# emilemathieu/RiemannHamiltonianMonteCarlo

Hardware: AMD Instinct MI355X
Metric: leapfrog-steps/sec (whole node) (higher is better)
Workload: dtype f64 (the two O(M D^2) contractions as exact int8-sliced integer GEMMs)

## Files before the change

### riemannhamiltonianmontecarlo_amd/csrc/kernels.hip.h

```cpp
#pragma once
#include <hip/hip_runtime.h>
#include <stdint.h>

typedef double d4 __attribute__((ext_vector_type(4)));

#define RM_LD 66
#define RM_PI2 6.283185307179586476925286766559
#define RM_PK_DOUBLES (2688 + 64)
template <bool PK>
__device__ __forceinline__ int rm_row(int i) {
  if (!PK) return i * RM_LD;
  const int I = i >> 4;
  return (128 * I + 160) * I + (i & 15) * (16 * I + 18);
}
template <bool PK>
__device__ __forceinline__ int rm_len(int i) { return PK ? 16 * ((i >> 4) + 1) : 64; }

struct DevData {
  const double* Xr;
  const double* Xt;
  const double* t;
  int M, Mp, D, DP, nblk;
  double inv_alpha;
  double log_prior_const;
// ... 1082 lines not shown
        for (int I = kb + 1; I < NB; ++I) op[I] = A[rm_row<PK>(16 * I + ii) + c0 + k0 + kk];
#pragma unroll
        for (int I = kb + 1; I < NB; ++I)
#pragma unroll
          for (int J = kb + 1; J <= I; ++J) acc[I][J] = __builtin_amdgcn_mfma_f64_16x16x4f64(op[I], op[J], acc[I][J], 0, 0, 0);
      }
#pragma unroll
      for (int I = kb + 1; I < NB; ++I)
#pragma unroll
        for (int J = kb + 1; J <= I; ++J)
#pragma unroll
          for (int r = 0; r < 4; ++r) A[rm_row<PK>(16 * I + kk + 4 * r) + 16 * J + ii] -= acc[I][J][r];
      __builtin_amdgcn_wave_barrier();
    }
  }
  if (lane >= D) rdiag = 1.0;
  return bad;
}
template <bool PK = false>
__device__ __forceinline__ double cholsolve_lds(const double* L, int D, int lane, double b, double rdiag) {
  const double* rowp = L + rm_row<PK>(lane);
  int k = 0;
  for (; k + 4 <= D; k += 4) {
    const double2 l01 = lds2(rowp + k), l23 = lds2(rowp + k + 2);
    const double lk[4] = {l01.x, l01.y, l23.x, l23.y};
#pragma unroll
    for (int q = 0; q < 4; ++q) {
      const double yk = rdlane(b, k + q) * rdlane(rdiag, k + q);
      if (lane == k + q) b = yk;
      else if (lane > k + q) b = fma(-lk[q], yk, b);
    }
  }
  for (; k < D; ++k) {
    const double yk = rdlane(b, k) * rdlane(rdiag, k);
    if (lane == k) b = yk;
    else if (lane > k) b = fma(-rowp[k], yk, b);
  }
  k = D - 1;
  for (; k >= 3; k -= 4) {
    const double lk[4] = {L[rm_row<PK>(k) + lane], L[rm_row<PK>(k - 1) + lane], L[rm_row<PK>(k - 2) + lane], L[rm_row<PK>(k - 3) + lane]};
#pragma unroll
    for (int q = 0; q < 4; ++q) {
      const double xk = rdlane(b, k - q) * rdlane(rdiag, k - q);
      if (lane == k - q) b = xk;
      else if (lane < k - q) b = fma(-lk[q], xk, b);
    }
  }
  for (; k >= 0; --k) {
    const double xk = rdlane(b, k) * rdlane(rdiag, k);
    if (lane == k) b = xk;
    else if (lane < k) b = fma(-L[rm_row<PK>(k) + lane], xk, b);
  }
  return b;
}

template <bool PK = false>
__device__ __forceinline__ void load_mat_lds(double* A, const double* __restrict__ G, int D, int DP, int lane) {
  const int l = lane < D ? lane : 0;
  int i = 0;
  for (; i + 16 <= D; i += 16) {
    double v[16];
    const bool in = lane < rm_len<PK>(i);
    if (in) {
#pragma unroll
      for (int q = 0; q < 16; ++q) v[q] = G[(i + q) * DP + l];
#pragma unroll
      for (int q = 0; q < 16; ++q) A[rm_row<PK>(i + q) + lane] = v[q];
    }
  }
  for (; i + 8 <= D; i += 8) {
    double v[8];
    if (lane < rm_len<PK>(i)) {
#pragma unroll
      for (int q = 0; q < 8; ++q) v[q] = G[(i + q) * DP + l];
#pragma unroll
      for (int q = 0; q < 8; ++q) A[rm_row<PK>(i + q) + lane] = v[q];
    }
  }
  for (; i < D; ++i)
    if (lane < rm_len<PK>(i)) A[rm_row<PK>(i) + lane] = G[i * DP + l];
  __builtin_amdgcn_wave_barrier();
}

__global__ __launch_bounds__(64) void k_pos_first(int D, int DP, Chains ch, double eps, int upd_nsplit = 0) {
  __shared__ double A[64];
  const int c = blockIdx.x, lane = threadIdx.x;
  if (c == 0 && lane == 0 && ch.stale_list) *ch.stale_count = 0;
  if (ch.phase[c] != 1) return;
  const double* __restrict__ Gi = ch.trj.Ginv + (size_t)c * DP * DP;
  const bool in = lane < D;
  double g[16];
#pragma unroll
  for (int q = 0; q < 16; ++q) g[q] = (in && q < D) ? Gi[q * DP + lane] : 0.0;
  double pb = in ? ch.p[(size_t)c * DP + lane] : 0.0;
  if (upd_nsplit > 0 && in) {
    const size_t o = (size_t)c * DP + lane;
    double q = 0.0;
    for (int s0 = 0; s0 < upd_nsplit; s0 += 16) {
      double t[16];
#pragma unroll
      for (int k = 0; k < 16; ++k) t[k] = (s0 + k < upd_nsplit) ? ch.qpart[((size_t)(s0 + k) * ch.n + c) * DP + lane] : 0.0;
#pragma unroll
      for (int k = 0; k < 16; ++k)
        if (s0 + k < upd_nsplit) q += t[k];
    }
    pb = pb + (ch.tau[c] * eps * 0.5) * (ch.trj.grad[o] - 0.5 * ch.trj.tr[o] + 0.5 * q);
    ch.p[o] = pb;
  }
  double u0 = 0.0;
  A[lane] = pb;
  __builtin_amdgcn_wave_barrier();
  for (int j0 = 0; j0 < D; j0 += 16) {
    double gn[16];
#pragma unroll
    for (int q = 0; q < 16; ++q) gn[q] = (in && j0 + 16 + q < D) ? Gi[(j0 + 16 + q) * DP + lane] : 0.0;
#pragma unroll
    for (int q = 0; q < 16; ++q)
      if (in && j0 + q < D) u0 = fma(g[q], A[j0 + q], u0);
#pragma unroll
    for (int q = 0; q < 16; ++q) g[q] = gn[q];
  }
  if (lane < D) {
    ch.u0[(size_t)c * DP + lane] = u0;
    ch.wq[(size_t)c * DP + lane] = ch.trj.w[(size_t)c * DP + lane] + ch.tau[c] * eps * u0;
  }
}

template <int NB>
__global__ __launch_bounds__(64) void k_factor_solve(int D, int DP, Chains ch, double eps, int last = -1) {
  __shared__ __attribute__((aligned(16))) double A[RM_PK_DOUBLES];
  const int c = blockIdx.x, lane = threadIdx.x;
  if (c == 0 && lane == 0 && ch.i8_dmax) *ch.i8_dmax = 0ull;
  if (ch.phase[c] != 1) return;
  if (lane == 0 && ch.i8_vbad) ch.i8_vbad[c] = 0;
  load_mat_lds<true>(A, ch.Gq + (size_t)c * DP * DP, D, DP, lane);
  double rdiag;
  const int bad = chol_lds_blk<NB, true>(A, D, lane, rdiag);
  const double pb = (lane < D) ? ch.p[(size_t)c * DP + lane] : 0.0;
  const double u = cholsolve_lds<true>(A, D, lane, pb, rdiag);
  double wn = 0.0;
  if (lane < D) wn = ch.trj.w[(size_t)c * DP + lane] + ch.tau[c] * (eps * 0.5) * (ch.u0[(size_t)c * DP + lane] + u);
  int st = bad ? 1 : 0;
  if (last >= 0) {
    const double nw = sqrt(wave_sum(wn * wn));
    if (last && nw > 10.0) { wn /= nw * 3.0; st |= 8; }
    if (lane < D) ch.trj.w[(size_t)c * DP + lane] = wn;
  }
  if (lane < D) ch.wq[(size_t)c * DP + lane] = wn;
  if (st && lane == 0) ch.status[c] |= st;
}

#define RM_DMAX 256
#define RM_DCH 4

__global__ __launch_bounds__(64) void k_pos_final(int D, int DP, Chains ch, int guards) {
  const int c = blockIdx.x, lane = threadIdx.x;
  if (ch.phase[c] != 1) return;
  const size_t o = (size_t)c * DP;
  double ss = 0.0;
  for (int d = lane; d < D; d += 64) { const double w = ch.wq[o + d]; ss = fma(w, w, ss); }
  const double nw = sqrt(wave_sum(ss));
  const bool fire = guards && nw > 10.0;
  for (int d = lane; d < D; d += 64) {
    double w = ch.wq[o + d];
    if (fire) w /= nw * 3.0;
    ch.trj.w[o + d] = w;
    ch.wq[o + d] = w;
  }
  if (fire && lane == 0) ch.status[c] |= 8;
}

template <int NB, bool PK = false>
__device__ __forceinline__ void spd_inverse_lds(double* A, int D, int lane, double rdiag) {
  constexpr int DPc = 16 * NB;
  {
    const bool act = lane < DPc;
    const int row = act ? lane : DPc - 1;
    double* rowp = A + rm_row<PK>(row);
    const int rlen = min(DPc, rm_len<PK>(row));
    const int il = row & 15, cb0 = row & ~15;
    if (act) {
      rowp[row] = rdiag;
      for (int m = row + 1; m < rlen; ++m) rowp[m] = 0.0;
    }
    __builtin_amdgcn_wave_barrier();
    for (int jl = 14; jl >= 0; --jl) {
      double s0 = 0.0, s1 = 0.0;
#pragma unroll
      for (int ml = 1; ml < 16; ++ml) {
        const double t = (ml > jl) ? rowp[cb0 + ml] * A[rm_row<PK>(cb0 + ml) + cb0 + jl] : 0.0;
        if (ml & 1) s0 += t; else s1 += t;
      }
      const double rj = A[rm_row<PK>(cb0 + jl) + cb0 + jl];
      __builtin_amdgcn_wave_barrier();
      if (act && il > jl) rowp[cb0 + jl] = -(s0 + s1) * rj;
      __builtin_amdgcn_wave_barrier();
    }
    const int kk = lane >> 4, ii = lane & 15;
#pragma unroll
    for (int J = 0; J + 1 < NB; ++J) {
#pragma unroll
      for (int I = J + 1; I < NB; ++I) {
        d4 T = (d4){0.0, 0.0, 0.0, 0.0};
#pragma unroll
        for (int K = J; K < I; ++K)
#pragma unroll
          for (int k0 = 0; k0 < 16; k0 += 4)
            T = __builtin_amdgcn_mfma_f64_16x16x4f64(A[rm_row<PK>(16 * I + ii) + 16 * K + k0 + kk], A[rm_row<PK>(16 * K + k0 + kk) + 16 * J + ii], T, 0, 0,
                                                     0);
        d4 R = (d4){0.0, 0.0, 0.0, 0.0};
#pragma unroll
        for (int r = 0; r < 4; ++r) R = __builtin_amdgcn_mfma_f64_16x16x4f64(A[rm_row<PK>(16 * I + ii) + 16 * I + 4 * r + kk], T[r], R, 0, 0, 0);
        __builtin_amdgcn_wave_barrier();
#pragma unroll
        for (int r = 0; r < 4; ++r) A[rm_row<PK>(16 * I + kk + 4 * r) + 16 * J + ii] = -R[r];
        __builtin_amdgcn_wave_barrier();
      }
    }
    if (D < DPc) {
      if (lane >= D && lane < DPc)
        for (int m = 0; m < rlen; ++m) rowp[m] = 0.0;
      __builtin_amdgcn_wave_barrier();
    }
  }
  constexpr int NT = NB * (NB + 1) / 2;
  d4 acc[NT];
#pragma unroll
  for (int q = 0; q < NT; ++q) acc[q] = (d4){0.0, 0.0, 0.0, 0.0};
  {
    const int kk = lane >> 4, ii = lane & 15;
    for (int m0 = 0; m0 < DPc; m0 += 4) {
      double op[NB];
#pragma unroll
      for (int I = 0; I < NB; ++I) op[I] = A[rm_row<PK>(m0 + kk) + 16 * I + ii];
      int q = 0;
#pragma unroll
      for (int I = 0; I < NB; ++I)
#pragma unroll
        for (int J = 0; J <= I; ++J) {
          if (m0 + 3 >= 16 * I) acc[q] = __builtin_amdgcn_mfma_f64_16x16x4f64(op[I], op[J], acc[q], 0, 0, 0);
          ++q;
        }
    }
  }
  __builtin_amdgcn_wave_barrier();
  {
    int q = 0;
#pragma unroll
    for (int I = 0; I < NB; ++I)
#pragma unroll
      for (int J = 0; J <= I; ++J) {
#pragma unroll
        for (int r = 0; r < 4; ++r) A[rm_row<PK>(16 * I + (lane >> 4) + 4 * r) + 16 * J + (lane & 15)] = acc[q][r];
        ++q;
      }
  }
  __builtin_amdgcn_wave_barrier();
}

template <int NB>
__global__ __launch_bounds__(64) void k_factor_full(DevData dd, Chains ch, int nsplit) {
  __shared__ __attribute__((aligned(16))) double A[RM_PK_DOUBLES];
  constexpr int DPc = 16 * NB;
  const int D = dd.D, DP = dd.DP;
  const int c = blockIdx.x, lane = threadIdx.x;
  if (c == 0 && lane == 0 && ch.i8_dmax) *ch.i8_dmax = 0ull;
  if (ch.phase[c] != 1) return;
  if (lane == 0 && ch.i8_vbad) ch.i8_vbad[c] = 0;
  load_mat_lds<true>(A, ch.Gq + (size_t)c * DP * DP, D, DP, lane);
  double rdiag;
  const int bad = chol_lds_blk<NB, true>(A, D, lane, rdiag);
  const double hld = -wave_sum((lane < D) ? log(rdiag) : 0.0);
  double* __restrict__ Lg = ch.trj.L + (size_t)c * DP * DP;
  for (int i = 0; i < D; ++i)
    if (lane <= i) Lg[i * DP + lane] = A[rm_row<true>(i) + lane];
  __builtin_amdgcn_wave_barrier();
  spd_inverse_lds<NB, true>(A, D, lane, rdiag);
  double* __restrict__ Gi = ch.trj.Ginv + (size_t)c * DP * DP;
  const double pl = (lane < D) ? ch.p[(size_t)c * DP + lane] : 0.0;
  double u = 0.0;
  for (int i = 0; i < D; ++i) {
    const double gi = (lane <= i) ? A[rm_row<true>(i) + lane] : A[rm_row<true>(min(lane, DPc - 1)) + i];
    if (lane < D) Gi[i * DP + lane] = gi;
    u = fma((lane < D) ? gi : 0.0, rdlane(pl, i), u);
  }
  if (lane < D) ch.uq[(size_t)c * DP + lane] = u;
  double part = 0.0;
  for (int b = lane; b < nsplit; b += 64) part += ch.ljl_part[(size_t)c * nsplit + b];
  const double wl = (lane < D) ? ch.trj.w[(size_t)c * DP + lane] : 0.0;
  if (lane < D) {
    double g = 0.0;
    for (int sp = 0; sp < nsplit; ++sp) g += ch.gpart[((size_t)sp * ch.n + c) * DP + lane];
    ch.trj.grad[(size_t)c * DP + lane] = g - wl * dd.inv_alpha;
  }
  part += (lane < D) ? (dd.log_prior_const - wl * wl * 0.5 * dd.inv_alpha) : 0.0;
  const double ljl = wave_sum(part);
  if (lane == 0) {
    ch.trj.hld[c] = hld;
    ch.trj.ljl[c] = ljl;
    if (bad) ch.status[c] |= 1;
  }
}

__global__ __launch_bounds__(64) void k_ginv_matvec(int D, int DP, Chains ch, const double* __restrict__ src) {
  const int c = blockIdx.x, lane = threadIdx.x;
  if (ch.phase[c] != 1) return;
  const double* __restrict__ Gi = ch.trj.Ginv + (size_t)c * DP * DP;
  if (D <= 64) {
    const bool in = lane < D;
    const double sv = in ? src[(size_t)c * DP + lane] : 0.0;
    double u0 = 0.0;
    for (int j0 = 0; j0 < D; j0 += 16) {
      double g[16];
#pragma unroll
      for (int q = 0; q < 16; ++q) g[q] = (in && j0 + q < D) ? Gi[(j0 + q) * DP + lane] : 0.0;
#pragma unroll
      for (int q = 0; q < 16; ++q)
        if (in && j0 + q < D) u0 = fma(g[q], rdlane(sv, j0 + q), u0);
    }
    if (in) ch.uq[(size_t)c * DP + lane] = u0;
    return;
  }
  double u[RM_DCH] = {0.0, 0.0, 0.0, 0.0};
  for (int j = 0; j < D; ++j) {
    const double sj = src[(size_t)c * DP + j];
#pragma unroll
    for (int k = 0; k < RM_DCH; ++k) {
      const int d = lane + 64 * k;
      if (d < D) u[k] = fma(Gi[j * DP + d], sj, u[k]);
    }
  }
#pragma unroll
  for (int k = 0; k < RM_DCH; ++k)
    if (lane + 64 * k < D) ch.uq[(size_t)c * DP + lane + 64 * k] = u[k];
}

__global__ __launch_bounds__(64) void k_mom_update(int D, int DP, Chains ch, double eps, int final, int nsplit) {
  const int c = blockIdx.x, lane = threadIdx.x;
  if (ch.phase[c] != 1) return;
  const double h = ch.tau[c] * eps * 0.5;
  for (int d = lane; d < D; d += 64) {
    const size_t o = (size_t)c * DP + d;
    double q = 0.0;
    for (int s = 0; s < nsplit; ++s) q += ch.qpart[((size_t)s * ch.n + c) * DP + d];
    const double pm = ch.p[o] + h * (ch.trj.grad[o] - 0.5 * ch.trj.tr[o] + 0.5 * q);
    if (final) ch.p[o] = pm;
    else ch.PM[o] = pm;
  }
}

__global__ __launch_bounds__(64) void k_mom_update_matvec(int D, int DP, Chains ch, double eps, int nsplit) {
  const int c = blockIdx.x, lane = threadIdx.x;
  if (ch.phase[c] != 1) return;
  const size_t o = (size_t)c * DP + lane;
  const double* __restrict__ Gi = ch.trj.Ginv + (size_t)c * DP * DP;
  const bool in = lane < D;
  double g[16];
#pragma unroll
  for (int q = 0; q < 16; ++q) g[q] = (in && q < D) ? Gi[q * DP + lane] : 0.0;
  double pm = 0.0;
  if (in) {
    double q = 0.0;
    for (int s0 = 0; s0 < nsplit; s0 += 16) {
      double t[16];
#pragma unroll
      for (int k = 0; k < 16; ++k) t[k] = (s0 + k < nsplit) ? ch.qpart[((size_t)(s0 + k) * ch.n + c) * DP + lane] : 0.0;
#pragma unroll
      for (int k = 0; k < 16; ++k)
        if (s0 + k < nsplit) q += t[k];
    }
    pm = ch.p[o] + (ch.tau[c] * eps * 0.5) * (ch.trj.grad[o] - 0.5 * ch.trj.tr[o] + 0.5 * q);
    ch.PM[o] = pm;
  }
  double u = 0.0;
  for (int j0 = 0; j0 < D; j0 += 16) {
    double gn[16];
#pragma unroll
    for (int q = 0; q < 16; ++q) gn[q] = (in && j0 + 16 + q < D) ? Gi[(j0 + 16 + q) * DP + lane] : 0.0;
#pragma unroll
    for (int q = 0; q < 16; ++q)
      if (j0 + q < D) u = fma(g[q], rdlane(pm, j0 + q), u);
#pragma unroll
    for (int q = 0; q < 16; ++q) g[q] = gn[q];
  }
  if (in) ch.uq[o] = u;
}

__global__ __launch_bounds__(64) void k_mom_final(int D, int DP, Chains ch, double eps, int advance, int nsplit, const double* __restrict__ trpart = nullptr) {
  const int c = blockIdx.x, lane = threadIdx.x;
  if (ch.phase[c] != 1) return;
  const double h = ch.tau[c] * eps * 0.5;
  int nonfinite = 0;
  for (int d = lane; d < D; d += 64) {
    const size_t o = (size_t)c * DP + d;
    if (trpart) {
      double s = 0.0;
      for (int sp = 0; sp < nsplit; ++sp) s += trpart[((size_t)sp * ch.n + c) * DP + d];
      ch.trj.tr[o] = s;
    }
    double q = 0.0;
    for (int s = 0; s < nsplit; ++s) q += ch.qpart[((size_t)s * ch.n + c) * DP + d];
    ch.last[o] = q;
    const double pn = advance ? ch.p[o] + h * (ch.trj.grad[o] - 0.5 * ch.trj.tr[o] + 0.5 * q) : ch.p[o];
    if (advance) ch.p[o] = pn;
    nonfinite |= !(isfinite(pn) && isfinite(ch.trj.w[o]));
  }
  const unsigned long long any = __ballot(nonfinite);
  if (lane == 0) {
    if (any) ch.status[c] |= 2;
    if (advance) {
      ch.steps_left[c] -= 1;
      ch.steps_done[c] += 1;
    }
  }
}

struct IterParams {
  unsigned flags;
  int L;
  unsigned long long seed;
  long long chain_offset;
  long long iter_limit;
  long long burn_in;
  long long S;
  double* samples;
  const double *z_in, *ulen_in, *gdir_in, *uacc_in;
  int* done_count;
  const int* orig;
  int lower_L;
};

__device__ __forceinline__ void copy_rec(const Rec& dst, const Rec& src, int c, int D, int DP, int lane, bool lowerL = false) {
  const size_t o = (size_t)c * DP;
  for (int d = lane; d < D; d += 64) {
    dst.w[o + d] = src.w[o + d];
    dst.grad[o + d] = src.grad[o + d];
    dst.tr[o + d] = src.tr[o + d];
  }
  const size_t m = (size_t)c * DP * DP;
  for (int d = lane; d < D; d += 64) {
    int i = 0;
    for (; i + 16 <= D; i += 16) {
      double a[16], b[16];
#pragma unroll
      for (int q = 0; q < 16; ++q) { a[q] = lowerL && d > i + 15 ? 0.0 : src.L[m + (i + q) * DP + d]; b[q] = src.Ginv[m + (i + q) * DP + d]; }
#pragma unroll
      for (int q = 0; q < 16; ++q) {
        if (!(lowerL && d > i + 15)) dst.L[m + (i + q) * DP + d] = a[q];
        dst.Ginv[m + (i + q) * DP + d] = b[q];
      }
    }
    for (; i + 8 <= D; i += 8) {
      double a[8], b[8];
#pragma unroll
      for (int q = 0; q < 8; ++q) { a[q] = lowerL && d > i + 7 ? 0.0 : src.L[m + (i + q) * DP + d]; b[q] = src.Ginv[m + (i + q) * DP + d]; }
#pragma unroll
      for (int q = 0; q < 8; ++q) {
        if (!(lowerL && d > i + 7)) dst.L[m + (i + q) * DP + d] = a[q];
        dst.Ginv[m + (i + q) * DP + d] = b[q];
      }
    }
    for (; i < D; ++i) {
      if (!(lowerL && d > i)) dst.L[m + i * DP + d] = src.L[m + i * DP + d];
      dst.Ginv[m + i * DP + d] = src.Ginv[m + i * DP + d];
    }
  }
  if (lane == 0) {
    dst.ljl[c] = src.ljl[c];
    dst.hld[c] = src.hld[c];
  }
}

__device__ __forceinline__ double half_quadform(const double* __restrict__ Gi, int D, int DP, int lane, const double* ps) {
  if (D <= 64) {
    const bool in = lane < D;
    double y = 0.0;
    for (int j0 = 0; j0 < D; j0 += 16) {
      double g[16];
#pragma unroll
      for (int q = 0; q < 16; ++q) g[q] = (in && j0 + q < D) ? Gi[(size_t)(j0 + q) * DP + lane] : 0.0;
#pragma unroll
      for (int q = 0; q < 16; ++q)
        if (in && j0 + q < D) y = fma(g[q], ps[j0 + q], y);
    }
    return 0.5 * wave_sum(in ? fma(y, ps[lane], 0.0) : 0.0);
  }
  double y[RM_DCH] = {0.0, 0.0, 0.0, 0.0};
  for (int j = 0; j < D; ++j) {
    const double pj = ps[j];
#pragma unroll
    for (int k = 0; k < RM_DCH; ++k) {
      const int d = lane + 64 * k;
      if (d < D) y[k] = fma(Gi[j * DP + d], pj, y[k]);
    }
  }
  double s = 0.0;
#pragma unroll
  for (int k = 0; k < RM_DCH; ++k)
    if (lane + 64 * k < D) s = fma(y[k], ps[lane + 64 * k], s);
  return 0.5 * wave_sum(s);
}

__device__ __forceinline__ void draw_normals(const IterParams& ip, int c, long long it, int D, int lane, double* zs, long long oc = -1) {
  const long long id = oc >= 0 ? oc : c;
  for (int d = lane; d < D; d += 64) {
    if (ip.z_in) {
      zs[d] = ip.z_in[(size_t)c * D + d];
    } else {
      double U0, U1;
      rng_block(ip.seed, (unsigned long long)(ip.chain_offset + id), (uint32_t)it, (uint32_t)(d >> 1), U0, U1);
      const double R = sqrt(-2.0 * log(U0));
      double sn, cs;
      sincos(RM_PI2 * U1, &sn, &cs);
      zs[d] = (d & 1) ? R * sn : R * cs;
    }
  }
  __builtin_amdgcn_wave_barrier();
}

__device__ __forceinline__ void iter_begin_dev(int D, int DP, const Chains& ch, const IterParams& ip, int c, int lane, double* zs, double* ps) {
  if (ch.phase[c] != 0) return;
  const long long it = ch.iter[c];
  if (it >= ip.iter_limit) return;
  if (!ch.cstale || ch.cstale[c]) copy_rec(ch.trj, ch.cur, c, D, DP, lane, ip.lower_L != 0);
  const long long oc = ip.orig ? ip.orig[c] : c;
  draw_normals(ip, c, it, D, lane, zs, oc);
  double u_len, g_dir;
  if (ip.z_in) {
    u_len = ip.ulen_in[c];
    g_dir = ip.gdir_in[c];
  } else {
    const unsigned long long gid = (unsigned long long)(ip.chain_offset + oc);
    double U0, U1, Ua;
    rng_block(ip.seed, gid, (uint32_t)it, 0x40000000u, u_len, Ua);
    rng_block(ip.seed, gid, (uint32_t)it, 0x40000001u, U0, U1);
    g_dir = sqrt(-2.0 * log(U0)) * cos(RM_PI2 * U1);
  }
  const double* __restrict__ Lc = ch.cur.L + (size_t)c * DP * DP;
  double p[RM_DCH] = {0.0, 0.0, 0.0, 0.0};
  if (D <= 64) {
    const int d = lane;
    double acc = 0.0;
    for (int j0 = 0; j0 < D; j0 += 16) {
      double l[16];
      if (ip.flags & 1u) {
#pragma unroll
        for (int q = 0; q < 16; ++q) l[q] = (j0 + q < D && d <= j0 + q) ? Lc[(size_t)(j0 + q) * DP + d] : 0.0;
#pragma unroll
        for (int q = 0; q < 16; ++q)
          if (j0 + q < D && d <= j0 + q) acc = fma(l[q], zs[j0 + q], acc);
      } else {
#pragma unroll
        for (int q = 0; q < 16; ++q) l[q] = (d < D && j0 + q <= d) ? Lc[(size_t)d * DP + j0 + q] : 0.0;
#pragma unroll
        for (int q = 0; q < 16; ++q)
          if (d < D && j0 + q <= d) acc = fma(l[q], zs[j0 + q], acc);
      }
    }
    p[0] = acc;
  } else if (ip.flags & 1u) {
    for (int i = 0; i < D; ++i) {
      const double zi = zs[i];
#pragma unroll
      for (int k = 0; k < RM_DCH; ++k) {
        const int d = lane + 64 * k;
        if (d <= i) p[k] = fma(Lc[i * DP + d], zi, p[k]);
      }
    }
  } else {
    for (int j = 0; j < D; ++j) {
      const double zj = zs[j];
#pragma unroll
      for (int k = 0; k < RM_DCH; ++k) {
        const int d = lane + 64 * k;
        if (d >= j && d < D) p[k] = fma(Lc[d * DP + j], zj, p[k]);
      }
    }
  }
  int st = 0;
  if (ip.flags & 2u) {
    double ss = 0.0;
#pragma unroll
    for (int k = 0; k < RM_DCH; ++k) ss = fma(p[k], p[k], ss);
    const double np_ = sqrt(wave_sum(ss));
    if (np_ > 100.0) {
#pragma unroll
      for (int k = 0; k < RM_DCH; ++k) p[k] /= np_ * 25.0;
      st = 4;
    }
  }
#pragma unroll
  for (int k = 0; k < RM_DCH; ++k) {
    const int d = lane + 64 * k;
    if (d < D) {
      ps[d] = p[k];
      ch.p[(size_t)c * DP + d] = p[k];
      ch.p0[(size_t)c * DP + d] = p[k];
    }
  }
  __builtin_amdgcn_wave_barrier();
  const double quad = half_quadform(ch.cur.Ginv + (size_t)c * DP * DP, D, DP, lane, ps);
  if (lane == 0) {
    const int ns = (int)ceil(u_len * (double)ip.L);
    ch.steps_left[c] = ns;
    ch.nsteps_last[c] = ns;
    ch.tau[c] = (g_dir > 0.5) ? 1.0 : -1.0;
    ch.Hcur[c] = -ch.cur.ljl[c] + ch.cur.hld[c] + quad;
    ch.status[c] = st;
    ch.phase[c] = (ns > 0) ? 1 : 2;
  }
}

__global__ __launch_bounds__(64) void k_iter_begin(int D, int DP, Chains ch, IterParams ip) {
  __shared__ double zs[RM_DMAX];
  __shared__ double ps[RM_DMAX];
  iter_begin_dev(D, DP, ch, ip, blockIdx.x, threadIdx.x, zs, ps);
}

__device__ __forceinline__ void iter_end_dev(int D, int DP, const Chains& ch, const IterParams& ip, int c, int lane, double* ps) {
  const int ph = ch.phase[c];
  if (!(ph == 2 || (ph == 1 && ch.steps_left[c] == 0))) return;
  const long long it = ch.iter[c];
  const long long oc = ip.orig ? ip.orig[c] : c;
  for (int d = lane; d < D; d += 64) ps[d] = ch.p[(size_t)c * DP + d];
  __builtin_amdgcn_wave_barrier();
  const double quad = half_quadform(ch.trj.Ginv + (size_t)c * DP * DP, D, DP, lane, ps);
  const double Hp = -ch.trj.ljl[c] + ch.trj.hld[c] + quad;
  const double ratio = -Hp + ch.Hcur[c];
  double u_acc;
  if (ip.z_in) {
    u_acc = ip.uacc_in[c];
  } else {
    double U0;
    rng_block(ip.seed, (unsigned long long)(ip.chain_offset + oc), (uint32_t)it, 0x40000000u, U0, u_acc);
  }
  const bool accept = (ratio > 0.0) || (ratio > log(u_acc));
  if (accept) copy_rec(ch.cur, ch.trj, c, D, DP, lane, ip.lower_L != 0);
  __builtin_amdgcn_wave_barrier();
  if (ip.samples && it >= ip.burn_in && it - ip.burn_in < ip.S)
    for (int d = lane; d < D; d += 64)
      ip.samples[((size_t)oc * ip.S + (size_t)(it - ip.burn_in)) * D + d] = ch.cur.w[(size_t)c * DP + d];
  if (lane == 0) {
    ch.Hprop[c] = Hp;
    if (accept) ch.accepted[c] += 1;
    else if (ch.cstale) {
      ch.cstale[c] = 1;
      if (ch.stale_list) ch.stale_list[atomicAdd(ch.stale_count, 1)] = c;
    }
    ch.iter[c] = it + 1;
    ch.phase[c] = 0;
    if (it + 1 == ip.iter_limit && ip.done_count) atomicAdd(ip.done_count, 1);
  }
}

__global__ __launch_bounds__(64) void k_iter_end(int D, int DP, Chains ch, IterParams ip) {
  __shared__ double ps[RM_DMAX];
  iter_end_dev(D, DP, ch, ip, blockIdx.x, threadIdx.x, ps);
}

__global__ __launch_bounds__(64) void k_commit_all(int D, int DP, Chains ch) {
  copy_rec(ch.cur, ch.trj, blockIdx.x, D, DP, threadIdx.x);
}

__device__ __forceinline__ void hmc_finish_eval(const DevData& dd, const Chains& ch, int c, int lane, int nsplit) {
  const int D = dd.D, DP = dd.DP;
  double part = 0.0;
  for (int d = lane; d < D; d += 64) {
    const double wl = ch.trj.w[(size_t)c * DP + d];
    double g = 0.0;
    for (int sp = 0; sp < nsplit; ++sp) g += ch.gpart[((size_t)sp * ch.n + c) * DP + d];
    ch.trj.grad[(size_t)c * DP + d] = g - wl * dd.inv_alpha;
    part += dd.log_prior_const - wl * wl * 0.5 * dd.inv_alpha;
  }
  for (int b = lane; b < nsplit; b += 64) part += ch.ljl_part[(size_t)c * nsplit + b];
  const double ljl = wave_sum(part);
  if (lane == 0) ch.trj.ljl[c] = ljl;
}
__device__ __forceinline__ void hmc_copy(const Rec& dst, const Rec& src, int c, int D, int DP, int lane) {
  for (int d = lane; d < D; d += 64) {
    dst.w[(size_t)c * DP + d] = src.w[(size_t)c * DP + d];
    dst.grad[(size_t)c * DP + d] = src.grad[(size_t)c * DP + d];
  }
  if (lane == 0) dst.ljl[c] = src.ljl[c];
}
__global__ __launch_bounds__(64) void k_hmc_init(DevData dd, Chains ch, int nsplit) {
  const int c = blockIdx.x, lane = threadIdx.x;
  hmc_finish_eval(dd, ch, c, lane, nsplit);
  __syncthreads();
  hmc_copy(ch.cur, ch.trj, c, dd.D, dd.DP, lane);
}
__global__ __launch_bounds__(64) void k_hmc_begin(int D, int DP, Chains ch, IterParams ip) {
  __shared__ double zs[RM_DMAX];
  const int c = blockIdx.x, lane = threadIdx.x;
  if (ch.phase[c] != 0) return;
  const long long it = ch.iter[c];
  if (it >= ip.iter_limit) return;
  hmc_copy(ch.trj, ch.cur, c, D, DP, lane);
  draw_normals(ip, c, it, D, lane, zs);
  double u_len;
  if (ip.z_in) {
    u_len = ip.ulen_in[c];
  } else {
    double Ua;
    rng_block(ip.seed, (unsigned long long)(ip.chain_offset + c), (uint32_t)it, 0x40000000u, u_len, Ua);
  }
  double kin = 0.0;
  for (int d = lane; d < D; d += 64) {
    const double z = zs[d];
    kin = fma(z, z, kin);
    ch.p[(size_t)c * DP + d] = z;
  }
  kin = 0.5 * wave_sum(kin);
  if (lane == 0) {
    const int ns = (int)ceil(u_len * (double)ip.L);
    ch.steps_left[c] = ns;
    ch.nsteps_last[c] = ns;
    ch.Hcur[c] = -ch.cur.ljl[c] + kin;
    ch.status[c] = 0;
    ch.phase[c] = (ns > 0) ? 1 : 2;
  }
}
__global__ __launch_bounds__(64) void k_hmc_pre(int D, int DP, Chains ch, double eps) {
  const int c = blockIdx.x, lane = threadIdx.x;
  if (ch.phase[c] != 1) return;
  int isnan_ = 0;
  for (int d = lane; d < D; d += 64) {
    const size_t o = (size_t)c * DP + d;
    const double p = ch.p[o] + eps * 0.5 * ch.trj.grad[o];
    ch.p[o] = p;
    isnan_ |= (p != p);
  }
  const unsigned long long nan = __ballot(isnan_);
  if (!nan)
    for (int d = lane; d < D; d += 64) ch.trj.w[(size_t)c * DP + d] += eps * ch.p[(size_t)c * DP + d];
  if (nan && lane == 0) { ch.status[c] |= 2; ch.steps_left[c] = 1; }
}
__global__ __launch_bounds__(64) void k_hmc_post(DevData dd, Chains ch, double eps, int nsplit) {
  const int c = blockIdx.x, lane = threadIdx.x;
  if (ch.phase[c] != 1) return;
  hmc_finish_eval(dd, ch, c, lane, nsplit);
  __syncthreads();
  if (!(ch.status[c] & 2))
    for (int d = lane; d < dd.D; d += 64) ch.p[(size_t)c * dd.DP + d] += eps * 0.5 * ch.trj.grad[(size_t)c * dd.DP + d];
  if (lane == 0) { ch.steps_left[c] -= 1; ch.steps_done[c] += 1; }
}
__global__ __launch_bounds__(64) void k_hmc_end(int D, int DP, Chains ch, IterParams ip) {
  const int c = blockIdx.x, lane = threadIdx.x;
  const int ph = ch.phase[c];
  if (!(ph == 2 || (ph == 1 && ch.steps_left[c] == 0))) return;
  const long long it = ch.iter[c];
  double kin = 0.0;
  for (int d = lane; d < D; d += 64) { const double pl = ch.p[(size_t)c * DP + d]; kin = fma(pl, pl, kin); }
  const double Hp = -ch.trj.ljl[c] + 0.5 * wave_sum(kin);
  const double ratio = -Hp + ch.Hcur[c];
  double u_acc;
  if (ip.z_in) {
    u_acc = ip.uacc_in[c];
  } else {
    double U0;
    rng_block(ip.seed, (unsigned long long)(ip.chain_offset + c), (uint32_t)it, 0x40000000u, U0, u_acc);
  }
  const bool accept = (ratio > 0.0) || (ratio > log(u_acc));
  if (accept) hmc_copy(ch.cur, ch.trj, c, D, DP, lane);
  __syncthreads();
  if (ip.samples && it >= ip.burn_in && it - ip.burn_in < ip.S)
    for (int d = lane; d < D; d += 64)
      ip.samples[((size_t)c * ip.S + (size_t)(it - ip.burn_in)) * D + d] = ch.cur.w[(size_t)c * DP + d];
  if (lane == 0) {
    ch.Hprop[c] = Hp;
    if (accept) ch.accepted[c] += 1;
    ch.iter[c] = it + 1;
    ch.phase[c] = 0;
    if (it + 1 == ip.iter_limit && ip.done_count) atomicAdd(ip.done_count, 1);
  }
}

template <int NB>
__global__ __launch_bounds__(256) void k_trvec(DevData dd, int n_chains, int nsplit, const double* __restrict__ R, double* __restrict__ trpart,
                                               const d4* __restrict__ ctile = nullptr) {
  constexpr int DP = 16 * NB;
  const int lane = threadIdx.x & 63;
  const int c0 = (blockIdx.x * 4 + (threadIdx.x >> 6)) * 16;
  if (c0 >= n_chains) return;
  const int split = blockIdx.y;
  const int rr = lane >> 4, ci = lane & 15;
  const int cj = min(c0 + ci, n_chains - 1);
  const int nb32 = dd.Mp / 32;
  const int per = (nb32 + nsplit - 1) / nsplit;
  const int B0 = split * per, B1 = min(nb32, B0 + per);
  const double* __restrict__ xr_p = dd.Xr + (size_t)(8 * rr) * DP + NB * ci;
  const double* __restrict__ rp = R + (size_t)cj * dd.Mp + 8 * rr;
  d4 T[NB];
#pragma unroll
  for (int I = 0; I < NB; ++I) T[I] = (d4){0.0, 0.0, 0.0, 0.0};
  for (int B = B0; B < B1; ++B) {
    const int n0 = 32 * B;
    d4 r0 = *(const d4*)(rp + n0), r1 = *(const d4*)(rp + n0 + 4);
    if (ctile) {
      const d4 cA = ctile[((size_t)(c0 >> 4) * (dd.Mp / 16) + 2 * B) * 64 + lane], cB = ctile[((size_t)(c0 >> 4) * (dd.Mp / 16) + 2 * B + 1) * 64 + lane];
      r0 *= (d4){cA[0], cB[0], cA[1], cB[1]};
      r1 *= (d4){cA[2], cB[2], cA[3], cB[3]};
    }
#pragma unroll
    for (int k = 0; k < 8; ++k) {
      double xb[NB];
#pragma unroll
      for (int I = 0; I < NB; ++I) xb[I] = xr_p[(size_t)(n0 + k) * DP + I];
      const double rv = k < 4 ? r0[k & 3] : r1[k & 3];
#pragma unroll
      for (int I = 0; I < NB; ++I) T[I] = __builtin_amdgcn_mfma_f64_16x16x4f64(xb[I], rv, T[I], 0, 0, 0);
    }
  }
  if (c0 + ci < n_chains) {
    double* __restrict__ out = trpart + ((size_t)split * n_chains + c0 + ci) * DP;
#pragma unroll
    for (int I = 0; I < NB; ++I)
#pragma unroll
      for (int r = 0; r < 4; ++r) {
        const int d = NB * (rr + 4 * r) + I;
        if (d < dd.D) out[d] = T[I][r];
      }
  }
}

__global__ __launch_bounds__(64) void k_mmala_begin(int D, int DP, Chains ch, IterParams ip, double eps, int full) {
  __shared__ double zs[RM_DMAX];
  __shared__ double ts[RM_DMAX];
  const int c = blockIdx.x, lane = threadIdx.x;
  const long long it = ch.iter[c];
  if (it >= ip.iter_limit) { if (lane == 0) ch.phase[c] = 0; return; }
  draw_normals(ip, c, it, D, lane, zs);
  const double* __restrict__ Lc = ch.cur.L + (size_t)c * DP * DP;
  const double* __restrict__ Gi = ch.cur.Ginv + (size_t)c * DP * DP;
  double zz = 0.0;
  for (int d = lane; d < D; d += 64) {
    double s = 0.0;
    for (int j = 0; j <= d; ++j) s = fma(Lc[(size_t)d * DP + j], zs[j], s);
    const double dv = ch.cur.grad[(size_t)c * DP + d] - (full ? ch.cur.tr[(size_t)c * DP + d] : 0.0);
    ts[d] = sqrt(eps) * s + 0.5 * eps * dv;
    zz = fma(zs[d], zs[d], zz);
  }
  zz = wave_sum(zz);
  __syncthreads();
  double u[RM_DCH] = {0.0, 0.0, 0.0, 0.0};
  for (int j = 0; j < D; ++j) {
    const double tj = ts[j];
#pragma unroll
    for (int k = 0; k < RM_DCH; ++k) {
      const int d = lane + 64 * k;
      if (d < D) u[k] = fma(Gi[(size_t)j * DP + d], tj, u[k]);
    }
  }
#pragma unroll
  for (int k = 0; k < RM_DCH; ++k) {
    const int d = lane + 64 * k;
    if (d < D) ch.trj.w[(size_t)c * DP + d] = ch.cur.w[(size_t)c * DP + d] + u[k];
  }
  if (lane == 0) {
    ch.Hcur[c] = ch.cur.ljl[c] + ch.cur.hld[c] - 0.5 * zz;
    ch.status[c] = 0;
    ch.phase[c] = 1;
  }
}
__global__ __launch_bounds__(64) void k_mmala_end(int D, int DP, Chains ch, IterParams ip, double eps, int full) {
  __shared__ double ds[RM_DMAX];
  const int c = blockIdx.x, lane = threadIdx.x;
  if (ch.phase[c] != 1) return;
  const long long it = ch.iter[c];
  const double* __restrict__ Lp = ch.trj.L + (size_t)c * DP * DP;
  const double* __restrict__ Gi = ch.trj.Ginv + (size_t)c * DP * DP;
  double u[RM_DCH] = {0.0, 0.0, 0.0, 0.0};
  for (int j = 0; j < D; ++j) {
    const double gj = ch.trj.grad[(size_t)c * DP + j] - (full ? ch.trj.tr[(size_t)c * DP + j] : 0.0);
#pragma unroll
    for (int k = 0; k < RM_DCH; ++k) {
      const int d = lane + 64 * k;
      if (d < D) u[k] = fma(Gi[(size_t)j * DP + d], gj, u[k]);
    }
  }
#pragma unroll
  for (int k = 0; k < RM_DCH; ++k) {
    const int d = lane + 64 * k;
    if (d < D) ds[d] = ch.trj.w[(size_t)c * DP + d] + 0.5 * eps * u[k] - ch.cur.w[(size_t)c * DP + d];
  }
  __syncthreads();
  double yy = 0.0;
  for (int j = lane; j < D; j += 64) {
    double s = 0.0;
    for (int i = j; i < D; ++i) s = fma(Lp[(size_t)i * DP + j], ds[i], s);
    yy = fma(s, s, yy);
  }
  yy = wave_sum(yy);
  const double q_rev = ch.trj.hld[c] - yy / (2.0 * eps);
  const double ratio = ch.trj.ljl[c] + q_rev - ch.Hcur[c];
  double u_acc;
  if (ip.z_in) {
    u_acc = ip.uacc_in[c];
  } else {
    double U0;
    rng_block(ip.seed, (unsigned long long)(ip.chain_offset + c), (uint32_t)it, 0x40000000u, U0, u_acc);
  }
  const bool accept = (ratio > 0.0) || (ratio > log(u_acc));
  __syncthreads();
  if (accept) copy_rec(ch.cur, ch.trj, c, D, DP, lane);
  __syncthreads();
  if (ip.samples && it >= ip.burn_in && it - ip.burn_in < ip.S)
    for (int d = lane; d < D; d += 64)
      ip.samples[((size_t)c * ip.S + (size_t)(it - ip.burn_in)) * D + d] = ch.cur.w[(size_t)c * DP + d];
  if (lane == 0) {
    ch.Hprop[c] = ratio;
    if (accept) ch.accepted[c] += 1;
    ch.iter[c] = it + 1;
    ch.phase[c] = 0;
  }
}

__global__ __launch_bounds__(64) void k_ess(const double* __restrict__ samples, long long S, int P, double* __restrict__ ess_out,
                                            double* __restrict__ mean_out, double* __restrict__ var_out, long long nfft) {
  extern __shared__ __attribute__((aligned(16))) double ess_x[];
  const long long idx = blockIdx.x;
  const long long c = idx / P;
  const int d = (int)(idx % P);
  const int lane = threadIdx.x;
  const double* __restrict__ x = samples + (size_t)c * S * P + d;
  double m = 0.0;
  for (long long s = lane; s < S; s += 64) m += x[(size_t)s * P];
  m = wave_sum(m) / (double)S;
  double c0 = 0.0;
  for (long long s = lane; s < S; s += 64) {
    const double v = x[(size_t)s * P] - m;
    ess_x[s] = v;
    c0 = fma(v, v, c0);
  }
  c0 = wave_sum(c0);
  __syncthreads();
  double prev = INFINITY, sum = 0.0;
  const long long half = S / 2;
  for (long long j = 0; j < half; ++j) {
    const long long l0 = 2 * j, l1 = 2 * j + 1;
    double a = 0.0, b = 0.0;
    for (long long s = lane; s + l0 < S; s += 64) a = fma(ess_x[s], ess_x[s + l0], a);
    for (long long s = lane; s + l1 < S; s += 64) b = fma(ess_x[s], ess_x[s + l1], b);
    if (nfft > 0) {
      const long long w0 = nfft - l0, w1 = nfft - l1;
      if (l0 > 0) for (long long s = lane; s + w0 < S; s += 64) a = fma(ess_x[s], ess_x[s + w0], a);
      for (long long s = lane; s + w1 < S; s += 64) b = fma(ess_x[s], ess_x[s + w1], b);
    }
    double g = wave_sum(a + b) / c0;
    if (g > prev) g = prev;
    if (!(g > 0.0)) break;
    sum += g;
    prev = g;
  }
  double mono = -1.0 + 2.0 * sum;
  if (mono < 1.0) mono = 1.0;
  if (lane == 0) {
    if (ess_out) ess_out[idx] = (c0 > 0.0) ? (double)S / mono : NAN;
    if (mean_out) mean_out[idx] = m;
    if (var_out) var_out[idx] = c0 / (double)S;
  }
}

__global__ void k_fill_int(int* p, int v, size_t n) {
  size_t i = blockIdx.x * (size_t)blockDim.x + threadIdx.x;
  if (i < n) p[i] = v;
}
__global__ void k_fill_ll(long long* p, long long v, size_t n) {
  size_t i = blockIdx.x * (size_t)blockDim.x + threadIdx.x;
  if (i < n) p[i] = v;
}
__global__ void k_min_iter(const long long* __restrict__ iter, size_t n, unsigned long long* __restrict__ out) {
  size_t i = blockIdx.x * (size_t)blockDim.x + threadIdx.x;
  unsigned long long m = i < n ? (unsigned long long)iter[i] : ~0ull;
  for (int o = 32; o > 0; o >>= 1) {
    const unsigned long long x = __shfl_xor(m, o);
    m = x < m ? x : m;
  }
  if ((threadIdx.x & 63) == 0) atomicMin(out, m);
}
__global__ void k_traj_steps(unsigned long long seed, long long chain_offset, int L, long long it0, long long it1, size_t n,
                             long long* __restrict__ T) {
  size_t c = blockIdx.x * (size_t)blockDim.x + threadIdx.x;
  if (c >= n) return;
  long long t = 0;
  for (long long it = it0; it < it1; ++it) {
    double u_len, ua;
    rng_block(seed, (unsigned long long)(chain_offset + (long long)c), (uint32_t)it, 0x40000000u, u_len, ua);
    t += (long long)ceil(u_len * (double)L);
  }
  T[c] = t;
}
__global__ void k_scatter_ll(long long* __restrict__ dst, const long long* __restrict__ src, const int* __restrict__ orig, size_t n) {
  size_t i = blockIdx.x * (size_t)blockDim.x + threadIdx.x;
  if (i < n) dst[orig[i]] = src[i];
}
__global__ void k_sub_ll(long long* __restrict__ a, const long long* __restrict__ b, size_t n) {
  size_t i = blockIdx.x * (size_t)blockDim.x + threadIdx.x;
  if (i < n) a[i] = b[i] - a[i];
}
__global__ void k_set_leapfrog(int n, const int* __restrict__ nsteps, const int* __restrict__ dir, Chains ch) {
  int c = blockIdx.x * blockDim.x + threadIdx.x;
  if (c >= n) return;
  ch.steps_left[c] = nsteps[c];
  ch.tau[c] = (double)dir[c];
  ch.phase[c] = nsteps[c] > 0 ? 1 : 3;
}
__global__ void k_park_finished(int n, Chains ch) {
  int c = blockIdx.x * blockDim.x + threadIdx.x;
  if (c >= n) return;
  if (ch.phase[c] == 1 && ch.steps_left[c] <= 0) ch.phase[c] = 3;
}
```

### riemannhamiltonianmontecarlo_amd/csrc/rmhmc_hip.hip

```cpp
#include "../../include/rmhmc.h"
#include "../../include/rmhmc_amh.h"
#include "../../include/rmhmc_iwls.h"
#include "../../include/rmhmc_gibbs.h"
#include "kernels.hip.h"
#include "fused_small.hip.h"
#include "large_d.hip.h"
#include "metric_i8.hip.h"
#include "medium_step.hip.h"
#include "amh.hip.h"
#include "iwls.hip.h"
#include "gibbs.hip.h"

#include <algorithm>
#include <chrono>
#include <cmath>
#include <cstdio>
#include <cstdlib>
#include <cstring>
#include <map>
#include <string>
#include <vector>

namespace {

thread_local char g_err[512] = "";
constexpr int MAX_LDS = 160 * 1024;

struct EvPair { hipEvent_t a, b; };

struct Group {
  Chains ch{};
  int n = 0;
  int nsplit = 1;
  int8_t* Vs = nullptr;
  int8_t* Qs = nullptr;
  double* qscale = nullptr;
  double *Gpart = nullptr, *Rpart = nullptr;
  int* Tq = nullptr;
  int tail_pieces = 1;
  int ksplit_a = 1, ksplit_l = 1;
  int fsplit = 1;
  int* vbad = nullptr;
  int* vexp = nullptr;
  int* vexp_d = nullptr; int* rebase = nullptr; unsigned long long* dmax = nullptr;
  unsigned long long* dcount = nullptr;
  double* Gbase = nullptr;
  d4* ctile = nullptr;
  int nCp = 0;
};

struct Options {
  int64_t graph = 1, sorted = 1, inflight = 32, cdyn = 1, crestore = 1, i8_force_rebase = 0;
  int64_t ccache = 1, medium = 1, fused = 1, hmc_traj_maxn = -1, fsplit = 0, nsplit_max = 64, nsplit_waves = -1, i8_tail = -1,
          i8_delta = 1, i8_delta_inner = 1;
};
struct OptionDesc { const char* key; int64_t Options::*slot; bool create_only; int64_t lo, hi; };
const OptionDesc kOptions[] = {
    {"graph", &Options::graph, false, 0, 1},
    {"sorted", &Options::sorted, false, 0, 1},
    {"inflight", &Options::inflight, false, 0, 1 << 20},
    {"cdyn", &Options::cdyn, false, 0, 1},
    {"crestore", &Options::crestore, false, 0, 1},
    {"i8_force_rebase", &Options::i8_force_rebase, false, 0, 1},
    {"ccache", &Options::ccache, true, 0, 1},
    {"medium", &Options::medium, true, 0, 1},
    {"fused", &Options::fused, true, 0, 1},
    {"hmc_traj_maxn", &Options::hmc_traj_maxn, true, -1, (int64_t)1 << 40},
    {"fsplit", &Options::fsplit, true, 0, 64},
    {"nsplit_max", &Options::nsplit_max, true, 1, 1 << 20},
    {"nsplit_waves", &Options::nsplit_waves, true, -1, 1 << 20},
    {"i8_tail", &Options::i8_tail, true, -1, 1},
    {"i8_delta", &Options::i8_delta, true, 0, 1},
    {"i8_delta_inner", &Options::i8_delta_inner, true, 0, 1},
};
const OptionDesc* find_option(const char* key) {
  if (!key) return nullptr;
  for (const OptionDesc& d : kOptions)
    if (!strcmp(d.key, key)) return &d;
  return nullptr;
}

}

struct rmhmc_ctx {
  int device = 0;
  int64_t M = 0, n = 0;
  int D = 0, DP = 0, NB = 0, Mp = 0, nblk = 0;
  uint32_t flags = 0;
  double alpha = 100.0;
  hipStream_t stream = nullptr;
  Options opt{};
  std::vector<hipEvent_t> flow;
  long long flow_steps = 0, flow_ticks = 0;
  int* stale_list_alloc = nullptr;
  DevData dd{};
  Group batch;
  std::vector<void*> allocs;
  bool have_data = false, chains_ready = false;
  int sampler = 0;
  bool big = false;
  int nbk = 1, npairs = 1;
  double *d_Wd = nullptr, *d_hpart = nullptr, *d_Gcopy = nullptr;
  bool want_G = false;
  bool fused = false;
  size_t fused_lds = 0;
  bool medium = false;
  size_t medium_lds = 0;
  bool hmc_traj = false;
  bool i8 = false;
  int i8S = 0, i8_nks = 0, i8_bn = 128, i8_chunk = 1;
  int i8_inner_drop = 1;
  int8_t* d_Zs = nullptr;
  int* d_ze = nullptr;
  int8_t* d_Zt = nullptr;
  int* d_zre = nullptr;
  double *d_cmin = nullptr, *d_cmax = nullptr;
  double* d_zscale = nullptr;
  int i8_nkp = 0, i8_NRp = 0;
  I8Pairs pairs{};
  bool i8_requested = false;
  double i8_bound = 0.0;
  int L = 6, K = 4;
  double eps = 0.5;
  uint64_t seed = 0;
  int64_t chain_offset = 0;
  double *d_z = nullptr, *d_ulen = nullptr, *d_gdir = nullptr, *d_uacc = nullptr;
  int *d_nsteps = nullptr, *d_dir = nullptr, *d_done = nullptr;
  long long* d_steps0 = nullptr;
  unsigned long long* d_miniter = nullptr;
  int* d_orig = nullptr;
  long long* d_T = nullptr;
  bool sorted = false;
  bool counters_sorted = false;
  rmhmc_progress_fn progress_fn = nullptr;
  void* progress_user = nullptr;
  long long progress_first = 0, progress_every = 0, progress_next = 0;
  bool timing = false;
  std::map<std::string, std::vector<EvPair>> events;
  std::vector<EvPair> pool;
  char err[512] = "";
};

namespace {

int fail(rmhmc_ctx* ctx, int code, const std::string& msg) {
  snprintf(ctx ? ctx->err : g_err, 512, "%s", msg.c_str());
  return code;
}

#define HIPCK(call)                                                                                        \
  do {                                                                                                     \
    hipError_t e_ = (call);                                                                                \
    if (e_ != hipSuccess)                                                                                  \
      return fail(ctx, RMHMC_ERR_RUNTIME, std::string(hipGetErrorString(e_)) + " in " #call " (" __FILE__ ":" + std::to_string(__LINE__) + ")"); \
  } while (0)

template <typename T>
int dalloc(rmhmc_ctx* ctx, T** p, size_t count) {
  void* q = nullptr;
  size_t bytes = (count ? count : 1) * sizeof(T);
  HIPCK(hipMalloc(&q, bytes));
  HIPCK(hipMemsetAsync(q, 0, bytes, ctx->stream));
  ctx->allocs.push_back(q);
  *p = (T*)q;
  return RMHMC_OK;
}

struct Timed {
  rmhmc_ctx* ctx;
  hipStream_t st;
  EvPair ev{};
  bool on;
  Timed(rmhmc_ctx* c, const char* name, hipStream_t s) : ctx(c), st(s), on(c->timing) {
    if (!on) return;
    if (!ctx->pool.empty()) { ev = ctx->pool.back(); ctx->pool.pop_back(); }
    else { (void)hipEventCreate(&ev.a); (void)hipEventCreate(&ev.b); }
    (void)hipEventRecord(ev.a, st);
    ctx->events[name].push_back(ev);
  }
  ~Timed() { if (on) (void)hipEventRecord(ev.b, st); }
};

template <typename F>
void launch(rmhmc_ctx* ctx, const char* name, F&& fn) {
  Timed t(ctx, name, ctx->stream);
  fn(ctx->stream);
}

void flow_tick(rmhmc_ctx* ctx, long long steps = 1) {
  const long long w = ctx->opt.inflight;
  if (w <= 0) return;
  ctx->flow_steps += steps;
  const long long stride = std::max<long long>(1, w / 4);
  if (ctx->flow_steps < stride) return;
  ctx->flow_steps = 0;
  if (ctx->flow.empty()) return;
  hipEvent_t e = ctx->flow[ctx->flow_ticks % 4];
  if (ctx->flow_ticks >= 4) (void)hipEventSynchronize(e);
  (void)hipEventRecord(e, ctx->stream);
  ctx->flow_ticks++;
}

#define NB_SWITCH(ctx, ...)                                               \
  switch ((ctx)->NB) {                                                    \
    case 1: { constexpr int NB_ = 1; __VA_ARGS__; } break;                \
    case 2: { constexpr int NB_ = 2; __VA_ARGS__; } break;                \
    case 3: { constexpr int NB_ = 3; __VA_ARGS__; } break;                \
    default: { constexpr int NB_ = 4; __VA_ARGS__; } break;               \
  }

#define I8_SWITCH(ctx, ...) I8_SWITCH_S((ctx)->i8S, __VA_ARGS__)
#define I8_SWITCH_S(sval, ...)                                                     \
  switch (sval) {                                                                  \
    case 4: { constexpr int S_ = 4, WN_ = 4, TN_ = 1; __VA_ARGS__; } break;        \
    case 5: { constexpr int S_ = 5, WN_ = 4, TN_ = 1; __VA_ARGS__; } break;        \
    case 6: { constexpr int S_ = 6, WN_ = 4, TN_ = 1; __VA_ARGS__; } break;        \
    default: { constexpr int S_ = 7, WN_ = 2, TN_ = 1; __VA_ARGS__; } break;       \
  }

static bool use_delta(const rmhmc_ctx* ctx, const Group& g) {
  return ctx->i8 && ctx->opt.i8_delta && (!ctx->big || g.Gbase) && ctx->i8S == 6 && g.ctile && g.ksplit_a <= 1 && ctx->K >= 2 && g.dmax;
}
static bool use_delta_inner(const rmhmc_ctx* ctx, const Group& g, int it) {
  return use_delta(ctx, g) && ctx->opt.i8_delta_inner && ctx->i8_inner_drop && it == 2 && it < ctx->K - 1;
}
template <int MODE>
void launch_rowpass(rmhmc_ctx* ctx, Group& g, const double* w, double* out0, double* out2 = nullptr, bool delta = false) {
  launch(ctx, "rowpass", [&](hipStream_t st) {
    if (ctx->big) {
      dim3 grid((unsigned)((g.n + 15) / 16), g.nsplit);
      hipLaunchKernelGGL((k_rowpass_big<MODE>), grid, dim3(256), 0, st, ctx->dd, g.n, g.nsplit, ctx->nbk, g.ch.phase, w, out0, out2,
                         g.ch.gpart, g.ch.ljl_part, g.ctile);
      return;
    }
    dim3 grid((unsigned)((g.n + 63) / 64), g.nsplit);
    if (ctx->i8 && MODE != RP_G) {
      const VSlice vs{g.Vs, g.vbad, ctx->i8_nks, g.nCp, ctx->i8S, g.vexp, ctx->d_cmin, ctx->d_cmax};
      if (MODE != RP_G && delta) {
        VSlice vd = vs;
        vd.vexp_d = g.vexp_d; vd.rebase = g.rebase; vd.dmax = g.dmax; vd.force_rebase = (int)ctx->opt.i8_force_rebase;
        if (MODE == RP_F) {
          NB_SWITCH(ctx, hipLaunchKernelGGL((k_rowpass<NB_, RP_F, 6, false, true>), grid, dim3(256), 0, st, ctx->dd, g.n, g.nsplit, g.ch.phase, w,
                                            out0, nullptr, g.ch.gpart, g.ch.ljl_part, vd, g.ctile, g.ch.cstale));
        } else {
          NB_SWITCH(ctx, hipLaunchKernelGGL((k_rowpass<NB_, RP_V, 6, true, true>), grid, dim3(256), 0, st, ctx->dd, g.n, g.nsplit, g.ch.phase, w,
                                            out0, out2, g.ch.gpart, g.ch.ljl_part, vd, g.ctile, g.ch.cstale));
        }
      } else if (g.ctile && MODE == RP_F) {
        I8_SWITCH(ctx, NB_SWITCH(ctx, hipLaunchKernelGGL((k_rowpass<NB_, MODE, S_, false>), grid, dim3(256), 0, st, ctx->dd, g.n, g.nsplit, g.ch.phase, w,
                                                        out0, nullptr, g.ch.gpart, g.ch.ljl_part, vs, g.ctile, g.ch.cstale)));
      } else {
        I8_SWITCH(ctx, NB_SWITCH(ctx, hipLaunchKernelGGL((k_rowpass<NB_, MODE, S_>), grid, dim3(256), 0, st, ctx->dd, g.n, g.nsplit, g.ch.phase, w, out0,
                                                        out2, g.ch.gpart, g.ch.ljl_part, vs, g.ctile, g.ch.cstale)));
      }
      return;
    }
    NB_SWITCH(ctx, hipLaunchKernelGGL((k_rowpass<NB_, MODE>), grid, dim3(256), 0, st, ctx->dd, g.n, g.nsplit, g.ch.phase, w, out0,
                                      out2, g.ch.gpart, g.ch.ljl_part, VSlice{}, g.ctile, g.ch.cstale));
  });
}

template <int S, int WN, int TN>
void launch_assemble_i8_t(rmhmc_ctx* ctx, Group& g, const double* v, hipStream_t st, int part, bool delta = false, int seff = 6, int need_lo = 0,
                          int need_hi = 0) {
  const size_t vplane = (size_t)ctx->i8_nks * g.nCp * 32;
  const int8_t* const Vs = g.Vs + (delta ? (size_t)(seff - S) * vplane : 0);
  const I8Delta dl{delta ? g.dmax : nullptr, delta ? g.rebase : nullptr, delta ? std::ldexp(1.0, -8 * (seff - S)) : 1.0, need_lo, need_hi,
                   (delta && ctx->big) ? g.Gbase : nullptr};
  const int* const vexp = delta ? g.vexp_d : g.vexp;
  const int acc0 = delta ? 2 : 0;
  if (part == 0) {
    if (delta) {
      (void)hipMemsetAsync(g.dmax, 0, sizeof(unsigned long long), st);
      hipLaunchKernelGGL((k_vsplit<S, true>), dim3((unsigned)((g.n + 7) / 8)), dim3(256), 0, st, v, ctx->Mp, g.n, g.ch.phase, ctx->i8_nks, g.nCp, g.Vs,
                         g.vbad, ctx->D, ctx->DP, ctx->dd.inv_alpha, g.ch.Gq, g.vexp, VDelta{g.vexp_d, g.rebase, g.dmax, (int)ctx->opt.i8_force_rebase});
      return;
    }
    hipLaunchKernelGGL((k_vsplit<S>), dim3((unsigned)((g.n + 7) / 8)), dim3(256), 0, st, v, ctx->Mp, g.n, g.ch.phase, ctx->i8_nks, g.nCp, g.Vs, g.vbad,
                       ctx->D, ctx->DP, ctx->dd.inv_alpha, g.ch.Gq, g.vexp, VDelta{});
    return;
  }
  const int nCB = g.nCp / I8_BM, nPB = ctx->pairs.NPp / (32 * TN * WN);
  constexpr int lds = i8_lds_bytes<S, WN, TN>();
  const unsigned nblk = (unsigned)(nCB < 8 ? nCB * nPB : (nCB + 7) / 8 * 8 * nPB);
  if (g.ksplit_a > 1) {
    const size_t plane = (size_t)g.n * ctx->DP * ctx->DP;
    hipLaunchKernelGGL((k_assemble_i8<S, WN, TN>), dim3(nblk, (unsigned)g.ksplit_a), dim3(128 * WN), lds, st, g.Vs, ctx->d_Zs, g.nCp, ctx->i8_nks,
                       0, ctx->i8_nks, 0, ctx->pairs, g.n, g.ch.phase, g.vbad, ctx->DP, ctx->dd.inv_alpha, g.Gpart, plane, g.vexp, nPB,
                       I8Delta{nullptr, nullptr, 1.0, 0, 0, nullptr});
    hipLaunchKernelGGL(k_sum_planes, dim3((unsigned)((plane + 255) / 256)), dim3(256), 0, st, g.ch.Gq, g.Gpart, g.ksplit_a, plane, plane);
    return;
  }
  const int nPBfull = ctx->pairs.NP / (32 * TN * WN);
  const bool tail = WN == 4 && g.Tq && nPBfull < nPB && (ctx->opt.i8_tail == 1 || (ctx->opt.i8_tail < 0 && (long long)nCB * nPBfull >= 256));
  const int npb = tail ? nPBfull : nPB;
  const unsigned nblk_main = (unsigned)(nCB < 8 ? nCB * npb : (nCB + 7) / 8 * 8 * npb);
  const int pb32_0 = nPBfull * TN * WN, ntail = (ctx->pairs.NP - pb32_0 * 32 + 31) / 32;
  for (int ks0 = 0; ks0 < ctx->i8_nks; ks0 += ctx->i8_chunk) {
    const int nk = std::min(ctx->i8_chunk, ctx->i8_nks - ks0);
    if (nblk_main)
      hipLaunchKernelGGL((k_assemble_i8<S, WN, TN>), dim3(nblk_main), dim3(128 * WN), lds, st, Vs, ctx->d_Zs, g.nCp,
                         ctx->i8_nks, ks0, nk, (ks0 > 0 ? 1 : 0) | acc0, ctx->pairs, g.n, g.ch.phase, g.vbad, ctx->DP, ctx->dd.inv_alpha, g.ch.Gq, (size_t)0, vexp, npb, dl);
    if (tail) {
      const int pieces = std::max(1, std::min({g.tail_pieces, nk / 8, (int)(256 / std::max(1, nCB * ntail))}));
      hipLaunchKernelGGL((k_assemble_i8_tail<S>), dim3((unsigned)(nCB * ntail), (unsigned)pieces), dim3(128), (i8_lds_bytes<S, 1, 1>()), st, Vs, ctx->d_Zs,
                         g.nCp, ctx->pairs.NPp, ctx->pairs.NP, ctx->i8_nks, ks0, nk, g.n, pb32_0, ntail, g.Tq, dl);
      hipLaunchKernelGGL((k_assemble_i8_tailsum<S>), dim3((unsigned)(((size_t)g.n * 32 * ntail + 255) / 256)), dim3(256), 0, st, g.Tq, pieces, g.nCp, ntail,
                         pb32_0, (ks0 > 0 ? 1 : 0) | acc0, ctx->pairs, g.n, g.ch.phase, g.vbad, ctx->DP, ctx->dd.inv_alpha, g.ch.Gq, vexp, dl);
    }
  }
}
void launch_assemble_i8_delta(rmhmc_ctx* ctx, Group& g, hipStream_t st, int seff) {
  constexpr int WN = 4, TN = 1;
  const size_t vplane = (size_t)ctx->i8_nks * g.nCp * 32;
  const I8Delta dl{g.dmax, g.rebase, 1.0, 0, 0, ctx->big ? g.Gbase : nullptr};
  const int nCB = g.nCp / I8_BM, nPB = ctx->pairs.NPp / (32 * TN * WN);
  constexpr int lds = i8_lds_bytes<6, WN, TN>() > i8_lds_bytes<4, WN, TN>() ? i8_lds_bytes<6, WN, TN>() : i8_lds_bytes<4, WN, TN>();
  static_assert(lds >= (i8_lds_bytes<5, WN, TN>()), "dynamic LDS of the widest instantiation");
  const int nPBfull = ctx->pairs.NP / (32 * TN * WN);
  const bool tail = g.Tq && nPBfull < nPB && (ctx->opt.i8_tail == 1 || (ctx->opt.i8_tail < 0 && (long long)nCB * nPBfull >= 256));
  const int npb = tail ? nPBfull : nPB;
  const unsigned nblk_main = (unsigned)(nCB < 8 ? nCB * npb : (nCB + 7) / 8 * 8 * npb);
  const int pb32_0 = nPBfull * TN * WN, ntail = (ctx->pairs.NP - pb32_0 * 32 + 31) / 32;
  constexpr int lds_t = i8_lds_bytes<6, 1, 1>() > i8_lds_bytes<4, 1, 1>() ? i8_lds_bytes<6, 1, 1>() : i8_lds_bytes<4, 1, 1>();
  static_assert(lds_t >= (i8_lds_bytes<5, 1, 1>()), "dynamic LDS of the widest tail instantiation");
  I8Delta dlc = dl;
  dlc.count = g.dcount;
  for (int ks0 = 0; ks0 < ctx->i8_nks; ks0 += ctx->i8_chunk) {
    const int nk = std::min(ctx->i8_chunk, ctx->i8_nks - ks0);
    if (nblk_main)
      hipLaunchKernelGGL((k_assemble_i8_sel<WN, TN>), dim3(nblk_main), dim3(128 * WN), lds, st, g.Vs, vplane, seff, ctx->d_Zs, g.nCp, ctx->i8_nks, ks0, nk,
                         (ks0 > 0 ? 1 : 0) | 2, ctx->pairs, g.n, g.ch.phase, g.vbad, ctx->DP, ctx->dd.inv_alpha, g.ch.Gq, (size_t)0, g.vexp_d, npb,
                         ks0 == 0 ? dlc : dl);
    if (tail) {
      const int pieces = std::max(1, std::min({g.tail_pieces, nk / 8, (int)(256 / std::max(1, nCB * ntail))}));
      hipLaunchKernelGGL(k_assemble_i8_tail_sel, dim3((unsigned)(nCB * ntail), (unsigned)pieces), dim3(128), lds_t, st, g.Vs, vplane, seff, ctx->d_Zs,
                         g.nCp, ctx->pairs.NPp, ctx->pairs.NP, ctx->i8_nks, ks0, nk, g.n, pb32_0, ntail, g.Tq, (ks0 == 0 && !nblk_main) ? dlc : dl);
      hipLaunchKernelGGL(k_assemble_i8_tailsum_sel, dim3((unsigned)(((size_t)g.n * 32 * ntail + 255) / 256)), dim3(256), 0, st, seff, g.Tq, pieces, g.nCp, ntail,
                         pb32_0, (ks0 > 0 ? 1 : 0) | 2, ctx->pairs, g.n, g.ch.phase, g.vbad, ctx->DP, ctx->dd.inv_alpha, g.ch.Gq, g.vexp_d, dl);
    }
  }
}
template <int S, int WN, int TN>
void launch_leverage_i8_t(rmhmc_ctx* ctx, Group& g, hipStream_t st, int part) {
  if (part == 0) {
    hipLaunchKernelGGL((k_qsplit<S>), dim3((unsigned)g.n), dim3(256), 0, st, g.ch.trj.Ginv, ctx->DP, ctx->pairs, g.ch.phase, ctx->i8_nkp, g.nCp,
                       g.Qs, g.qscale);
    return;
  }
  const int nCB = g.nCp / I8_BM, nRB = ctx->i8_NRp / (32 * TN * WN);
  constexpr int lds = i8_lds_bytes<S, WN, TN>();
  const unsigned nblk = (unsigned)(nCB < 8 ? nCB * nRB : (nCB + 7) / 8 * 8 * nRB);
  if (g.ksplit_l > 1) {
    const size_t plane = (size_t)g.n * ctx->Mp;
    hipLaunchKernelGGL((k_leverage_i8<S, WN, TN>), dim3(nblk, (unsigned)g.ksplit_l), dim3(128 * WN), lds, st, g.Qs, ctx->d_Zt, g.nCp, ctx->i8_NRp,
                       ctx->i8_nkp, 0, ctx->i8_nkp, 0, (ctx->big || g.ctile) ? 0 : 1, g.n, ctx->Mp, g.ch.phase, g.qscale, ctx->d_zscale, g.ch.rv2, g.Rpart, plane);
    hipLaunchKernelGGL(k_sum_planes, dim3((unsigned)((plane + 255) / 256)), dim3(256), 0, st, g.ch.rv0, g.Rpart, g.ksplit_l, plane, plane);
    return;
  }
  for (int kp0 = 0; kp0 < ctx->i8_nkp; kp0 += ctx->i8_chunk) {
    const int nk = std::min(ctx->i8_chunk, ctx->i8_nkp - kp0);
    hipLaunchKernelGGL((k_leverage_i8<S, WN, TN>), dim3(nblk), dim3(128 * WN), lds, st, g.Qs, ctx->d_Zt, g.nCp,
                       ctx->i8_NRp, ctx->i8_nkp, kp0, nk, kp0 > 0 ? 1 : 0, (ctx->big || g.ctile) ? 0 : 1, g.n, ctx->Mp, g.ch.phase, g.qscale, ctx->d_zscale,
                       g.ch.rv2, g.ch.rv0, (size_t)0);
  }
}
void launch_assemble(rmhmc_ctx* ctx, Group& g, const double* v, bool inner = false, bool delta = false, bool keep_base = false) {
  if (ctx->i8 && delta && ctx->big)
    launch(ctx, "vsplit", [&](hipStream_t st) { launch_assemble_i8_t<6, 4, 1>(ctx, g, v, st, 0, true); });
  if (ctx->i8 && delta && inner) {
    launch(ctx, "assemble_i8_inner_delta", [&](hipStream_t st) { launch_assemble_i8_delta(ctx, g, st, 5); });
    return;
  }
  if (ctx->i8 && delta) {
    launch(ctx, "assemble_i8_delta", [&](hipStream_t st) { launch_assemble_i8_delta(ctx, g, st, 6); });
    return;
  }
  if (ctx->i8) {
    if (ctx->big)
      launch(ctx, "vsplit", [&](hipStream_t st) { I8_SWITCH(ctx, (launch_assemble_i8_t<S_, WN_, TN_>(ctx, g, v, st, 0))); });
    const int suse = (inner && ctx->i8_inner_drop && ctx->i8S == 6) ? 5 : ctx->i8S;
    launch(ctx, suse == ctx->i8S ? "assemble_i8" : "assemble_i8_inner", [&](hipStream_t st) {
      I8_SWITCH_S(suse, (launch_assemble_i8_t<S_, WN_, TN_>(ctx, g, v, st, 1)));
      if (keep_base && ctx->big && g.Gbase)
        (void)hipMemcpyAsync(g.Gbase, g.ch.Gq, sizeof(double) * (size_t)g.n * ctx->DP * ctx->DP, hipMemcpyDeviceToDevice, st);
    });
    return;
  }
  launch(ctx, "assemble", [&](hipStream_t st) {
    if (ctx->flags & RMHMC_FLAG_FP32_METRIC) {
      if (ctx->big) {
        hipLaunchKernelGGL((k_assemble_f32<4>), dim3((unsigned)((g.n + 3) / 4), ctx->npairs), dim3(256), 0, st, ctx->dd, g.n, g.ch.phase, v,
                           g.ch.Gq, ctx->nbk);
      } else {
        NB_SWITCH(ctx, hipLaunchKernelGGL((k_assemble_f32<NB_>), dim3((unsigned)((g.n + 3) / 4)), dim3(256), 0, st, ctx->dd, g.n,
                                          g.ch.phase, v, g.ch.Gq, 1));
      }
      return;
    }
    if (ctx->big) {
      hipLaunchKernelGGL(k_assemble_pair<false>, dim3((unsigned)((g.n + 3) / 4), ctx->npairs - ctx->nbk), dim3(256), 0, st, ctx->dd, g.n,
                         g.ch.phase, v, g.ch.Gq);
      hipLaunchKernelGGL(k_assemble_pair<true>, dim3((unsigned)((g.n + 3) / 4), ctx->nbk), dim3(256), 0, st, ctx->dd, g.n, g.ch.phase, v,
                         g.ch.Gq);
      return;
    }
    if (g.fsplit > 1) {
      const size_t plane = (size_t)g.n * ctx->DP * ctx->DP;
      dim3 grid((unsigned)((g.n + 3) / 4), (unsigned)g.fsplit);
      NB_SWITCH(ctx, hipLaunchKernelGGL((k_assemble<NB_>), grid, dim3(256), 0, st, ctx->dd, g.n, g.ch.phase, v, g.Gpart, plane));
      hipLaunchKernelGGL(k_sum_planes, dim3((unsigned)((plane + 255) / 256)), dim3(256), 0, st, g.ch.Gq, g.Gpart, g.fsplit, plane, plane);
      return;
    }
    dim3 grid((unsigned)((g.n + 3) / 4));
    NB_SWITCH(ctx, hipLaunchKernelGGL((k_assemble<NB_>), grid, dim3(256), 0, st, ctx->dd, g.n, g.ch.phase, v, g.ch.Gq, (size_t)0));
  });
}

void launch_mompass(rmhmc_ctx* ctx, Group& g, const double* w, int cmode) {
  launch(ctx, "mompass", [&](hipStream_t st) {
    if (!ctx->opt.ccache) cmode = 0;
    if (ctx->big) {
      dim3 grid((unsigned)((g.n + 15) / 16), g.nsplit);
      switch (cmode) {
        case 1: hipLaunchKernelGGL(k_mompass_big<1>, grid, dim3(256), 0, st, ctx->dd, g.n, g.nsplit, ctx->nbk, w, g.ch.uq, g.ch.qpart, g.ctile); break;
        case 2: hipLaunchKernelGGL(k_mompass_big<2>, grid, dim3(256), 0, st, ctx->dd, g.n, g.nsplit, ctx->nbk, w, g.ch.uq, g.ch.qpart, g.ctile); break;
        default: hipLaunchKernelGGL(k_mompass_big<0>, grid, dim3(256), 0, st, ctx->dd, g.n, g.nsplit, ctx->nbk, w, g.ch.uq, g.ch.qpart, g.ctile); break;
      }
      return;
    }
    dim3 grid((unsigned)((g.n + 63) / 64), g.nsplit);
    switch (cmode) {
      case 1:
        if (ctx->opt.cdyn) { NB_SWITCH(ctx, hipLaunchKernelGGL((k_mompass<NB_, 3>), grid, dim3(256), 0, st, ctx->dd, g.n, g.nsplit, w, g.ch.uq, g.ch.qpart, g.ctile, g.ch.cstale)); }
        else { NB_SWITCH(ctx, hipLaunchKernelGGL((k_mompass<NB_, 1>), grid, dim3(256), 0, st, ctx->dd, g.n, g.nsplit, w, g.ch.uq, g.ch.qpart, g.ctile)); }
        break;
      case 2: NB_SWITCH(ctx, hipLaunchKernelGGL((k_mompass<NB_, 2>), grid, dim3(256), 0, st, ctx->dd, g.n, g.nsplit, w, g.ch.uq, g.ch.qpart, g.ctile)); break;
      default: NB_SWITCH(ctx, hipLaunchKernelGGL((k_mompass<NB_, 0>), grid, dim3(256), 0, st, ctx->dd, g.n, g.nsplit, w, g.ch.uq, g.ch.qpart, g.ctile)); break;
    }
  });
}

static bool fused_trace(const rmhmc_ctx* ctx, const Group& g) { return ctx->i8 && !ctx->big && g.ctile != nullptr && ctx->opt.ccache; }

void launch_leverage(rmhmc_ctx* ctx, Group& g, int part = 0) {
  if (ctx->i8 && part == 2) {
    launch(ctx, "small", [&](hipStream_t st) {
      hipLaunchKernelGGL(k_reduce_tr, dim3((unsigned)g.n), dim3(64), 0, st, ctx->D, ctx->DP, g.ch, g.ch.gpart, g.nsplit);
    });
    return;
  }
  if (ctx->i8) {
    launch(ctx, "qsplit", [&](hipStream_t st) { I8_SWITCH(ctx, (launch_leverage_i8_t<S_, WN_, TN_>(ctx, g, st, 0))); });
    const int suse = (ctx->i8_inner_drop && ctx->i8S == 6) ? 5 : ctx->i8S;
    launch(ctx, "leverage_i8", [&](hipStream_t st) { I8_SWITCH_S(suse, (launch_leverage_i8_t<S_, WN_, TN_>(ctx, g, st, 1))); });
    if (part == 1) return;
    launch(ctx, "trvec", [&](hipStream_t st) {
      if (ctx->big) {
        dim3 grid((unsigned)((g.n + 15) / 16), g.nsplit);
        hipLaunchKernelGGL(k_trace_big, grid, dim3(256), 0, st, ctx->dd, g.n, g.nsplit, ctx->nbk, 1, g.ch.rv2, g.ch.rv0, g.ch.gpart);
        return;
      }
      dim3 grid((unsigned)((g.n + 63) / 64), g.nsplit);
      NB_SWITCH(ctx, hipLaunchKernelGGL((k_trvec<NB_>), grid, dim3(256), 0, st, ctx->dd, g.n, g.nsplit, g.ch.rv0, g.ch.gpart, (const d4*)g.ctile));
    });
    launch(ctx, "small", [&](hipStream_t st) {
      hipLaunchKernelGGL(k_reduce_tr, dim3((unsigned)g.n), dim3(64), 0, st, ctx->D, ctx->DP, g.ch, g.ch.gpart, g.nsplit);
    });
    return;
  }
  if (ctx->big) {
    double* hpart = ctx->d_hpart;
    launch(ctx, "leverage", [&](hipStream_t st) {
      hipLaunchKernelGGL(k_leverage_pair<false>, dim3((unsigned)((g.n + 3) / 4), ctx->npairs - ctx->nbk), dim3(256), 0, st, ctx->dd, g.n,
                         ctx->nbk, g.ch.phase, g.ch.trj.Ginv, hpart);
      hipLaunchKernelGGL(k_leverage_pair<true>, dim3((unsigned)((g.n + 3) / 4), ctx->nbk), dim3(256), 0, st, ctx->dd, g.n, ctx->nbk,
                         g.ch.phase, g.ch.trj.Ginv, hpart);
    });
    launch(ctx, "leverage", [&](hipStream_t st) {
      dim3 grid((unsigned)((g.n + 15) / 16), g.nsplit);
      hipLaunchKernelGGL(k_trace_big, grid, dim3(256), 0, st, ctx->dd, g.n, g.nsplit, ctx->nbk, ctx->npairs, g.ch.rv2, hpart, g.ch.gpart);
    });
    launch(ctx, "small", [&](hipStream_t st) {
      hipLaunchKernelGGL(k_reduce_tr, dim3((unsigned)g.n), dim3(64), 0, st, ctx->D, ctx->DP, g.ch, g.ch.gpart, g.nsplit);
    });
    return;
  }
  const int fs = std::min(g.fsplit, g.nsplit);
  launch(ctx, "leverage", [&](hipStream_t st) {
    dim3 grid((unsigned)((g.n + 3) / 4), (unsigned)fs);
    NB_SWITCH(ctx, hipLaunchKernelGGL((k_leverage<NB_>), grid, dim3(256), 0, st, ctx->dd, g.n, g.ch.phase, g.ch.trj.Ginv, g.ch.rv2,
                                      g.ch.trj.tr, g.ch.gpart));
  });
  if (fs > 1)
    launch(ctx, "small", [&](hipStream_t st) {
      hipLaunchKernelGGL(k_reduce_tr, dim3((unsigned)g.n), dim3(64), 0, st, ctx->D, ctx->DP, g.ch, g.ch.gpart, fs);
    });
}

#define SMALL(ctx, g, name, kern, ...)                                                                     \
  launch(ctx, name, [&](hipStream_t st_) { hipLaunchKernelGGL(kern, dim3((unsigned)(g).n), dim3(64), 0, st_, __VA_ARGS__); })

#define BIG(ctx, g, name, kern, ...)                                                                       \
  launch(ctx, name, [&](hipStream_t st_) { hipLaunchKernelGGL(kern, dim3((unsigned)(g).n), dim3(256), 0, st_, __VA_ARGS__); })

void eval_point_phases(rmhmc_ctx* ctx, Group& g, bool advance, int mode = 0) {
  const bool delta = advance && use_delta(ctx, g);
  launch_rowpass<RP_F>(ctx, g, g.ch.trj.w, g.ch.rv0, g.ch.rv2, delta);
  if (ctx->big) SMALL(ctx, g, "small", k_finish_big, ctx->dd, g.ch, g.nsplit);
  launch_assemble(ctx, g, g.ch.rv0, false, delta);
  if (ctx->big) {
    if (ctx->want_G)
      (void)hipMemcpyAsync(ctx->d_Gcopy, g.ch.Gq, sizeof(double) * (size_t)g.n * ctx->DP * ctx->DP, hipMemcpyDeviceToDevice, ctx->stream);
    BIG(ctx, g, "factor", k_chol_big<1>, ctx->dd, g.ch, ctx->nbk, ctx->d_Wd, ctx->eps);
    BIG(ctx, g, "factor", k_inverse_big, ctx->dd, g.ch, ctx->nbk, ctx->d_Wd);
    SMALL(ctx, g, "small", k_ginv_matvec, ctx->D, ctx->DP, g.ch, g.ch.p);
  } else {
    launch(ctx, "factor", [&](hipStream_t st) {
      NB_SWITCH(ctx, hipLaunchKernelGGL((k_factor_full<NB_>), dim3((unsigned)g.n), dim3(64), 0, st, ctx->dd, g.ch, g.nsplit));
    });
  }
  if (mode == 1) return;
  if (mode == 2) {
    launch_leverage(ctx, g);
    return;
  }
  if (fused_trace(ctx, g)) {
    launch_leverage(ctx, g, 1);
    launch(ctx, "mompass", [&](hipStream_t st) {
      dim3 grid((unsigned)((g.n + 63) / 64), g.nsplit);
      NB_SWITCH(ctx, hipLaunchKernelGGL((k_mompass_trv<NB_>), grid, dim3(256), 0, st, ctx->dd, g.n, g.nsplit, g.ch.uq, g.ch.qpart, g.ctile, g.ch.rv0, g.ch.gpart));
    });
  } else {
    launch_mompass(ctx, g, g.ch.trj.w, 2);
    launch_leverage(ctx, g);
  }
  SMALL(ctx, g, "small", k_mom_final, ctx->D, ctx->DP, g.ch, ctx->eps, advance ? 1 : 0, g.nsplit, fused_trace(ctx, g) ? g.ch.gpart : (const double*)nullptr);
}

template <int NB>
void launch_step_medium_nb(rmhmc_ctx* ctx, Group& g, hipStream_t st, int guards, int eval_only, int fold, const IterParams& ip) {
  const int rpt = (ctx->Mp + 255) / 256;
  const dim3 grid((unsigned)g.n), block(256);
  const size_t lds = ctx->medium_lds;
  switch (rpt * 16 * NB <= 64 ? rpt : 0) {
    case 1: hipLaunchKernelGGL((k_step_medium<NB, 1>), grid, block, lds, st, ctx->dd, g.ch, ctx->eps, ctx->K, guards, eval_only, fold, ip); break;
    case 2: hipLaunchKernelGGL((k_step_medium<NB, 2>), grid, block, lds, st, ctx->dd, g.ch, ctx->eps, ctx->K, guards, eval_only, fold, ip); break;
    case 3: hipLaunchKernelGGL((k_step_medium<NB, (NB == 1 ? 3 : 0)>), grid, block, lds, st, ctx->dd, g.ch, ctx->eps, ctx->K, guards, eval_only, fold, ip); break;
    case 4: hipLaunchKernelGGL((k_step_medium<NB, (NB == 1 ? 4 : 0)>), grid, block, lds, st, ctx->dd, g.ch, ctx->eps, ctx->K, guards, eval_only, fold, ip); break;
    default: hipLaunchKernelGGL((k_step_medium<NB, 0>), grid, block, lds, st, ctx->dd, g.ch, ctx->eps, ctx->K, guards, eval_only, fold, ip); break;
  }
}
void launch_step_medium(rmhmc_ctx* ctx, Group& g, hipStream_t st, int guards, int eval_only, int fold, const IterParams& ip) {
  if (ctx->NB == 1) launch_step_medium_nb<1>(ctx, g, st, guards, eval_only, fold, ip);
  else launch_step_medium_nb<2>(ctx, g, st, guards, eval_only, fold, ip);
}

void step_phases(rmhmc_ctx* ctx, Group& g) {
  const int D = ctx->D, DP = ctx->DP, K = ctx->K;
  const double eps = ctx->eps;
  const int guards = (ctx->flags & RMHMC_FLAG_GUARDS) ? 1 : 0;
  if (ctx->medium) {
    launch(ctx, "medium", [&](hipStream_t st) { launch_step_medium(ctx, g, st, guards, 0, 0, IterParams{}); });
    return;
  }
  if (!ctx->big && ctx->opt.cdyn && g.ctile && g.ch.stale_list)
    launch(ctx, "mompass", [&](hipStream_t st) {
      const int rsplit = std::max(1, std::min(32, ctx->Mp / 32 / 4));
      dim3 grid((unsigned)std::min((g.n + 63) / 64, 8), (unsigned)rsplit);
      NB_SWITCH(ctx, hipLaunchKernelGGL((k_crestore<NB_>), grid, dim3(256), 0, st, ctx->dd, g.n, g.ch.phase, g.ch.trj.w, g.ctile, g.ch.cstale,
                                        g.ch.stale_list, g.ch.stale_count));
    });
  const bool fuse = !ctx->big;
  for (int it = 0; it < K; ++it) {
    if (it == 0 || !fuse) SMALL(ctx, g, "small", k_ginv_matvec, D, DP, g.ch, it == 0 ? g.ch.p : g.ch.PM);
    launch_mompass(ctx, g, g.ch.trj.w, it == 0 ? 1 : 2);
    if (!fuse) SMALL(ctx, g, "small", k_mom_update, D, DP, g.ch, eps, it == K - 1 ? 1 : 0, g.nsplit);
    else if (it < K - 1) SMALL(ctx, g, "small", k_mom_update_matvec, D, DP, g.ch, eps, g.nsplit);
  }
  if (ctx->big) {
    SMALL(ctx, g, "small", k_ginv_matvec, D, DP, g.ch, g.ch.p);
    SMALL(ctx, g, "small", k_pos_first_big, D, DP, g.ch, eps);
  } else {
    SMALL(ctx, g, "factor", k_pos_first, D, DP, g.ch, eps, g.nsplit);
  }
  for (int it = 1; it < K; ++it) {
    launch_rowpass<RP_V>(ctx, g, g.ch.wq, g.ch.rv0, nullptr, use_delta_inner(ctx, g, it));
    const bool base = (it == 1 && use_delta_inner(ctx, g, 2)) || (it == K - 1 && use_delta(ctx, g));
    launch_assemble(ctx, g, g.ch.rv0, it < K - 1, use_delta_inner(ctx, g, it), base);
    if (ctx->big)
      BIG(ctx, g, "factor", k_chol_big<0>, ctx->dd, g.ch, ctx->nbk, ctx->d_Wd, eps);
    else
      launch(ctx, "factor", [&](hipStream_t st) {
        NB_SWITCH(ctx, hipLaunchKernelGGL((k_factor_solve<NB_>), dim3((unsigned)g.n), dim3(64), 0, st, D, DP, g.ch, eps, it == K - 1 ? guards : -1));
      });
  }
  if (ctx->big || K < 2) SMALL(ctx, g, "small", k_pos_final, D, DP, g.ch, guards);
  eval_point_phases(ctx, g, true);
}

struct IterBase {
  long long limit, burn_in, S;
  double* samples;
  bool explicit_rng;
  bool count_done;
};

IterParams iter_params(rmhmc_ctx* ctx, const IterBase& b) {
  IterParams ip{};
  ip.flags = ctx->flags;
  ip.L = ctx->L;
  ip.seed = ctx->seed;
  ip.chain_offset = ctx->chain_offset;
  ip.iter_limit = b.limit;
  ip.burn_in = b.burn_in;
  ip.S = b.S;
  ip.samples = b.samples;
  if (ctx->sorted) ip.orig = ctx->d_orig;
  if (b.explicit_rng) {
    ip.z_in = ctx->d_z; ip.ulen_in = ctx->d_ulen; ip.gdir_in = ctx->d_gdir; ip.uacc_in = ctx->d_uacc;
  }
  ip.done_count = b.count_done ? ctx->d_done : nullptr;
  ip.lower_L = (!ctx->big && !ctx->medium && !ctx->fused && ctx->sampler == 0) ? 1 : 0;
  return ip;
}

void launch_iter_begin(rmhmc_ctx* ctx, Group& g, const IterBase& b) {
  const IterParams ip = iter_params(ctx, b);
  SMALL(ctx, g, "small", k_iter_begin, ctx->D, ctx->DP, g.ch, ip);
}
void launch_iter_end(rmhmc_ctx* ctx, Group& g, const IterBase& b) {
  const IterParams ip = iter_params(ctx, b);
  SMALL(ctx, g, "small", k_iter_end, ctx->D, ctx->DP, g.ch, ip);
}

template <int NB>
void launch_hmc_traj_nb(rmhmc_ctx* ctx, Group& g, int eval_only, hipStream_t st) {
  const int rpt = (ctx->Mp + 255) / 256;
  const dim3 grid((unsigned)g.n), block(256);
  switch (rpt <= 4 ? rpt : 0) {
    case 1: hipLaunchKernelGGL((k_hmc_traj<NB, 1>), grid, block, 0, st, ctx->dd, g.ch, ctx->eps, eval_only); break;
    case 2: hipLaunchKernelGGL((k_hmc_traj<NB, 2>), grid, block, 0, st, ctx->dd, g.ch, ctx->eps, eval_only); break;
    case 3: hipLaunchKernelGGL((k_hmc_traj<NB, 3>), grid, block, 0, st, ctx->dd, g.ch, ctx->eps, eval_only); break;
    case 4: hipLaunchKernelGGL((k_hmc_traj<NB, 4>), grid, block, 0, st, ctx->dd, g.ch, ctx->eps, eval_only); break;
    default: hipLaunchKernelGGL((k_hmc_traj<NB, 0>), grid, block, 0, st, ctx->dd, g.ch, ctx->eps, eval_only); break;
  }
}
void launch_hmc_traj(rmhmc_ctx* ctx, Group& g, int eval_only) {
  launch(ctx, "medium", [&](hipStream_t st) {
    if (ctx->NB == 1) launch_hmc_traj_nb<1>(ctx, g, eval_only, st);
    else launch_hmc_traj_nb<2>(ctx, g, eval_only, st);
  });
}

void launch_hmc_global_step(rmhmc_ctx* ctx, Group& g, const IterBase& b) {
  const double eps = ctx->eps;
  const IterParams ip = iter_params(ctx, b);
  SMALL(ctx, g, "small", k_hmc_begin, ctx->D, ctx->DP, g.ch, ip);
  if (ctx->hmc_traj) {
    launch_hmc_traj(ctx, g, 0);
  } else {
    SMALL(ctx, g, "small", k_hmc_pre, ctx->D, ctx->DP, g.ch, eps);
    launch_rowpass<RP_G>(ctx, g, g.ch.trj.w, nullptr);
    SMALL(ctx, g, "small", k_hmc_post, ctx->dd, g.ch, eps, g.nsplit);
  }
  SMALL(ctx, g, "small", k_hmc_end, ctx->D, ctx->DP, g.ch, ip);
}

void launch_global_step(rmhmc_ctx* ctx, Group& g, const IterBase& b) {
  if (ctx->sampler == 1) { launch_hmc_global_step(ctx, g, b); return; }
  if (ctx->medium) {
    const int guards = (ctx->flags & RMHMC_FLAG_GUARDS) ? 1 : 0;
    const IterParams ip = iter_params(ctx, b);
    launch(ctx, "medium", [&](hipStream_t st) { launch_step_medium(ctx, g, st, guards, 0, 1, ip); });
    return;
  }
  launch_iter_begin(ctx, g, b);
  step_phases(ctx, g);
  launch_iter_end(ctx, g, b);
}

void launch_fused(rmhmc_ctx* ctx, const IterBase& b, long long nsteps) {
  Group& g = ctx->batch;
  while (nsteps > 0) {
    const int chunk = (int)std::min<long long>(nsteps, 4096);
    FusedParams fp{};
    fp.ip = iter_params(ctx, b);
    fp.eps = ctx->eps; fp.K = ctx->K; fp.nsteps = chunk; fp.DPs = ctx->DP; fp.init_eval = 0;
    launch(ctx, "fused", [&](hipStream_t st) {
      hipLaunchKernelGGL(k_fused_small, dim3((unsigned)((g.n + FS_WAVES - 1) / FS_WAVES)), dim3(64 * FS_WAVES), ctx->fused_lds, st,
                         ctx->dd, g.ch, fp);
    });
    nsteps -= chunk;
    if (nsteps > 0) flow_tick(ctx, ctx->opt.inflight);
  }
}

void fill_int(rmhmc_ctx* ctx, int* p, int v, size_t n) {
  hipLaunchKernelGGL(k_fill_int, dim3((unsigned)((n + 255) / 256)), dim3(256), 0, ctx->stream, p, v, n);
}
void fill_ll(rmhmc_ctx* ctx, long long* p, long long v, size_t n) {
  hipLaunchKernelGGL(k_fill_ll, dim3((unsigned)((n + 255) / 256)), dim3(256), 0, ctx->stream, p, v, n);
}

int upload_vec(rmhmc_ctx* ctx, double* dst, const double* src) {
  HIPCK(hipMemcpy2DAsync(dst, ctx->DP * sizeof(double), src, ctx->D * sizeof(double), ctx->D * sizeof(double), ctx->n,
                         hipMemcpyHostToDevice, ctx->stream));
  return RMHMC_OK;
}
int download_vec(rmhmc_ctx* ctx, double* dst, const double* src) {
  HIPCK(hipMemcpy2DAsync(dst, ctx->D * sizeof(double), src, ctx->DP * sizeof(double), ctx->D * sizeof(double), ctx->n,
                         hipMemcpyDeviceToHost, ctx->stream));
  return RMHMC_OK;
}
template <typename T>
int download(rmhmc_ctx* ctx, T* dst, const T* src, size_t count) {
  HIPCK(hipMemcpyAsync(dst, src, count * sizeof(T), hipMemcpyDeviceToHost, ctx->stream));
  return RMHMC_OK;
}
template <typename T>
int upload(rmhmc_ctx* ctx, T* dst, const T* src, size_t count) {
  HIPCK(hipMemcpyAsync(dst, src, count * sizeof(T), hipMemcpyHostToDevice, ctx->stream));
  return RMHMC_OK;
}

int sync(rmhmc_ctx* ctx) {
  HIPCK(hipStreamSynchronize(ctx->stream));
  HIPCK(hipGetLastError());
  return RMHMC_OK;
}

#define RC(x) do { int rc_ = (x); if (rc_ != RMHMC_OK) return rc_; } while (0)
#define NEED_DATA(ctx)                                                              \
  do {                                                                              \
    if (!(ctx)) return fail(nullptr, RMHMC_ERR_INVALID, "null context");            \
    if (!(ctx)->have_data) return fail(ctx, RMHMC_ERR_INVALID, "rmhmc_set_data has not been called"); \
    HIPCK(hipSetDevice((ctx)->device));                                             \
  } while (0)

int eval_at(rmhmc_ctx* ctx, const double* w, const double* p, bool one_launch = false) {
  Group& g = ctx->batch;
  Chains& ch = g.ch;
  RC(upload_vec(ctx, ch.trj.w, w));
  if (p) RC(upload_vec(ctx, ch.p, p));
  else HIPCK(hipMemsetAsync(ch.p, 0, sizeof(double) * ctx->n * ctx->DP, ctx->stream));
  fill_int(ctx, ch.phase, 1, ctx->n);
  fill_int(ctx, ch.status, 0, ctx->n);
  if (one_launch && ctx->medium) {
    launch(ctx, "medium", [&](hipStream_t st) { launch_step_medium(ctx, g, st, 0, 1, 0, IterParams{}); });
    return RMHMC_OK;
  }
  eval_point_phases(ctx, g, false);
  return RMHMC_OK;
}

void apply_runtime_options(rmhmc_ctx* ctx) {
  Group& g = ctx->batch;
  const bool ok = !ctx->big && !ctx->medium && !ctx->fused && g.ctile && ctx->opt.cdyn && ctx->opt.crestore;
  g.ch.stale_list = ok ? ctx->stale_list_alloc : nullptr;
}

}

extern "C" {

const char* rmhmc_version(void) { return "rmhmc-hip 0.1 (gfx950, fp64 MFMA)"; }
const char* rmhmc_last_error(const rmhmc_ctx* ctx) { return ctx ? ctx->err : g_err; }

int rmhmc_create(rmhmc_ctx** out, int32_t device_id, int64_t M, int32_t D, int64_t n_chains, int32_t dtype, uint32_t flags) {
  return rmhmc_create_opts(out, device_id, M, D, n_chains, dtype, flags, nullptr, 0);
}

int rmhmc_create_opts(rmhmc_ctx** out, int32_t device_id, int64_t M, int32_t D, int64_t n_chains, int32_t dtype, uint32_t flags,
                      const rmhmc_option* opts, int32_t n_opts) {
  rmhmc_ctx* ctx = nullptr;
  Options opt{};
  if (n_opts < 0 || (n_opts > 0 && !opts)) return fail(nullptr, RMHMC_ERR_INVALID, "rmhmc_create_opts: bad option array");
  for (int i = 0; i < n_opts; ++i) {
    const OptionDesc* d = find_option(opts[i].key);
    if (!d) return fail(nullptr, RMHMC_ERR_INVALID, std::string("rmhmc_create_opts: unknown option '") + (opts[i].key ? opts[i].key : "(null)") + "'");
    if (opts[i].value < d->lo || opts[i].value > d->hi)
      return fail(nullptr, RMHMC_ERR_INVALID, std::string("rmhmc_create_opts: value out of range for option '") + d->key + "'");
    opt.*(d->slot) = opts[i].value;
  }
  if (!out || M <= 0 || D <= 0 || n_chains <= 0) return fail(nullptr, RMHMC_ERR_INVALID, "rmhmc_create: bad shape");
  if (dtype != RMHMC_F64) return fail(nullptr, RMHMC_ERR_UNSUPPORTED, "rmhmc_create: only float64 is built (the reference is float64)");
  if (D > 256) return fail(nullptr, RMHMC_ERR_UNSUPPORTED, "rmhmc_create: D > 256 is not supported (64 < D <= 256 uses the blocked large-D path)");
  if (flags & RMHMC_FLAG_ORACLE_LITERAL) return fail(nullptr, RMHMC_ERR_UNSUPPORTED, "rmhmc_create: the literal variant exists only in the CPU oracle");
  if (M > (int64_t)1 << 30 || n_chains > (int64_t)1 << 30) return fail(nullptr, RMHMC_ERR_UNSUPPORTED, "rmhmc_create: M or n_chains too large");
  if (D <= 64 && (M + 63) / 64 * 64 * (int64_t)(16 * ((D + 15) / 16)) * 8 >= (int64_t)1 << 32)
    return fail(nullptr, RMHMC_ERR_UNSUPPORTED, "rmhmc_create: the data matrix of the D <= 64 path must stay below 4 GB");
  int ndev = 0;
  if (hipGetDeviceCount(&ndev) != hipSuccess || ndev <= 0)
    return fail(nullptr, RMHMC_ERR_NO_DEVICE, "rmhmc_create: no HIP device available (this library has no CPU fallback)");
  if (device_id < 0 || device_id >= ndev) return fail(nullptr, RMHMC_ERR_NO_DEVICE, "rmhmc_create: device ordinal out of range");
  HIPCK(hipSetDevice(device_id));
  hipDeviceProp_t prop;
  HIPCK(hipGetDeviceProperties(&prop, device_id));
  if (std::string(prop.gcnArchName).find("gfx950") == std::string::npos)
    return fail(nullptr, RMHMC_ERR_NO_DEVICE, std::string("rmhmc_create: kernels are built for gfx950 only, device is ") + prop.gcnArchName);
  ctx = new rmhmc_ctx();
  ctx->device = device_id;
  ctx->M = M; ctx->D = D; ctx->n = n_chains; ctx->flags = flags; ctx->opt = opt;
  ctx->NB = (D + 15) / 16; ctx->DP = 16 * ctx->NB;
  if (D > 64) {
    ctx->big = true;
    ctx->nbk = (D + 63) / 64;
    ctx->npairs = ctx->nbk * (ctx->nbk + 1) / 2;
    ctx->DP = 64 * ctx->nbk;
    ctx->NB = 4;
  }
  ctx->Mp = (int)((M + 63) / 64 * 64); ctx->nblk = ctx->Mp / 64;
  if (flags & RMHMC_FLAG_INT8_INNER_FULL) ctx->i8_inner_drop = 0;
  int rc = RMHMC_OK;
  auto body = [&]() -> int {
    HIPCK(hipStreamCreateWithFlags(&ctx->stream, hipStreamNonBlocking));
    ctx->flow.resize(4);
    for (auto& e : ctx->flow) { e = nullptr; HIPCK(hipEventCreateWithFlags(&e, hipEventDisableTiming)); }
    const size_t n = n_chains, DP = ctx->DP, Mp = ctx->Mp;
    double *Xr, *Xt, *t;
    RC(dalloc(ctx, &Xr, Mp * DP)); RC(dalloc(ctx, &Xt, DP * Mp)); RC(dalloc(ctx, &t, Mp));
    ctx->dd.Xr = Xr; ctx->dd.Xt = Xt; ctx->dd.t = t;
    ctx->dd.M = (int)M; ctx->dd.Mp = ctx->Mp; ctx->dd.D = D; ctx->dd.DP = ctx->DP; ctx->dd.nblk = ctx->nblk;
    Chains& ch = ctx->batch.ch;
    ch.n = (int)n;
    for (Rec* r : {&ch.cur, &ch.trj}) {
      RC(dalloc(ctx, &r->w, n * DP)); RC(dalloc(ctx, &r->grad, n * DP)); RC(dalloc(ctx, &r->tr, n * DP));
      RC(dalloc(ctx, &r->L, n * DP * DP)); RC(dalloc(ctx, &r->Ginv, n * DP * DP));
      RC(dalloc(ctx, &r->ljl, n)); RC(dalloc(ctx, &r->hld, n));
    }
    RC(dalloc(ctx, &ch.p, n * DP)); RC(dalloc(ctx, &ch.p0, n * DP)); RC(dalloc(ctx, &ch.Hcur, n)); RC(dalloc(ctx, &ch.Hprop, n));
    RC(dalloc(ctx, &ch.tau, n)); RC(dalloc(ctx, &ch.steps_left, n)); RC(dalloc(ctx, &ch.phase, n)); RC(dalloc(ctx, &ch.status, n)); RC(dalloc(ctx, &ch.cstale, n));
    RC(dalloc(ctx, &ch.stale_list, n)); RC(dalloc(ctx, &ch.stale_count, (size_t)1));
    ctx->stale_list_alloc = ch.stale_list;
    RC(dalloc(ctx, &ch.nsteps_last, n)); RC(dalloc(ctx, &ch.iter, n)); RC(dalloc(ctx, &ch.accepted, n)); RC(dalloc(ctx, &ch.steps_done, n));
    RC(dalloc(ctx, &ch.wq, n * DP)); RC(dalloc(ctx, &ch.uq, n * DP)); RC(dalloc(ctx, &ch.PM, n * DP)); RC(dalloc(ctx, &ch.u0, n * DP));
    RC(dalloc(ctx, &ch.q, n * DP)); RC(dalloc(ctx, &ch.last, n * DP)); RC(dalloc(ctx, &ch.Gq, n * DP * DP));
    RC(dalloc(ctx, &ch.rv0, n * Mp)); RC(dalloc(ctx, &ch.rv2, n * Mp));
    Group& g = ctx->batch;
    {
      g.n = (int)n_chains;
      const long long cgroups = (g.n + 15) / 16, nb16 = ctx->Mp / 16;
      const long long target = ctx->opt.nsplit_waves > 0 ? ctx->opt.nsplit_waves : (ctx->big ? 6144 : 2048);
      long long ns = (target + cgroups - 1) / cgroups;
      if (ns < 1) ns = 1;
      if (ns > nb16) ns = nb16;
      if (ns > ctx->opt.nsplit_max) ns = ctx->opt.nsplit_max;
      g.nsplit = (int)ns;
      RC(dalloc(ctx, &g.ch.qpart, (size_t)g.nsplit * g.n * DP));
      RC(dalloc(ctx, &g.ch.gpart, (size_t)g.nsplit * g.n * DP));
      RC(dalloc(ctx, &g.ch.ljl_part, (size_t)g.n * g.nsplit));
      if (ctx->opt.ccache) RC(dalloc(ctx, &g.ctile, (size_t)((g.n + 15) / 16) * (ctx->Mp / 16) * 64));
      if (!ctx->big) {
        const long long waves = g.n;
        long long fs = waves >= 1024 ? 1 : std::min<long long>(16, (2048 + waves - 1) / waves);
        fs = std::min<long long>(fs, std::max(1, ctx->Mp / 256));
        if (ctx->opt.fsplit >= 1) fs = ctx->opt.fsplit;
        g.fsplit = (int)fs;
      }
    }
    int i8_slices = (int)((flags >> 12) & 7u);
    if (i8_slices == 0) i8_slices = 6;
    if (i8_slices < 4) i8_slices = 4;
    if (flags & RMHMC_FLAG_INT8_METRIC) {
      const int S = i8_slices;
      ctx->i8_chunk = std::max(1, (int)(2147483647.0 / (S * 16384.0)) / 32);
      ctx->i8 = true;
      ctx->i8_requested = true;
      ctx->i8S = S;
      ctx->i8_bn = S <= 6 ? 128 : 64;
      ctx->i8_nks = (int)((M + 31) / 32);
      const int NP = D * (D + 1) / 2, NPp = (NP + ctx->i8_bn - 1) / ctx->i8_bn * ctx->i8_bn;
      std::vector<short> pa(NPp, 0), pb(NPp, 0);
      for (int a = 0, q = 0; a < D; ++a)
        for (int b = 0; b <= a; ++b, ++q) { pa[q] = (short)a; pb[q] = (short)b; }
      short *d_pa, *d_pb; double* d_scale;
      RC(dalloc(ctx, &d_pa, (size_t)NPp)); RC(dalloc(ctx, &d_pb, (size_t)NPp)); RC(dalloc(ctx, &d_scale, (size_t)NPp));
      RC(dalloc(ctx, &ctx->d_ze, (size_t)NPp));
      HIPCK(hipMemcpyAsync(d_pa, pa.data(), NPp * sizeof(short), hipMemcpyHostToDevice, ctx->stream));
      HIPCK(hipMemcpyAsync(d_pb, pb.data(), NPp * sizeof(short), hipMemcpyHostToDevice, ctx->stream));
      RC(sync(ctx));
      int* d_cexp;
      RC(dalloc(ctx, &d_cexp, (size_t)ctx->DP));
      RC(dalloc(ctx, &ctx->d_cmin, (size_t)ctx->DP)); RC(dalloc(ctx, &ctx->d_cmax, (size_t)ctx->DP));
      ctx->pairs = I8Pairs{d_pa, d_pb, d_scale, NP, NPp, d_cexp};
      RC(dalloc(ctx, &ctx->d_Zs, (size_t)S * ctx->i8_nks * NPp * 32));
      ctx->i8_nkp = (NP + 31) / 32;
      ctx->i8_NRp = (ctx->Mp + ctx->i8_bn - 1) / ctx->i8_bn * ctx->i8_bn;
      RC(dalloc(ctx, &ctx->d_Zt, (size_t)S * ctx->i8_nkp * ctx->i8_NRp * 32));
      RC(dalloc(ctx, &ctx->d_zre, (size_t)ctx->i8_NRp)); RC(dalloc(ctx, &ctx->d_zscale, (size_t)ctx->i8_NRp));
      {
        g.nCp = (g.n + I8_BM - 1) / I8_BM * I8_BM;
        RC(dalloc(ctx, &g.Vs, (size_t)S * ctx->i8_nks * g.nCp * 32));
        RC(dalloc(ctx, &g.vbad, (size_t)g.nCp));
        RC(dalloc(ctx, &g.vexp, (size_t)g.nCp));
        RC(dalloc(ctx, &g.vexp_d, (size_t)g.nCp)); RC(dalloc(ctx, &g.rebase, (size_t)g.nCp)); RC(dalloc(ctx, &g.dmax, (size_t)1));
        RC(dalloc(ctx, &g.dcount, (size_t)6));
        if (!ctx->big) { g.ch.i8_vbad = g.vbad; g.ch.i8_dmax = g.dmax; }
        if (ctx->big && ctx->opt.i8_delta && S == 6) RC(dalloc(ctx, &g.Gbase, (size_t)g.n * ctx->DP * ctx->DP));
        RC(dalloc(ctx, &g.Qs, (size_t)S * ctx->i8_nkp * g.nCp * 32));
        RC(dalloc(ctx, &g.qscale, (size_t)g.nCp));
        auto pieces = [&](long long tiles, int stages) {
          long long k = std::min<long long>(16, 256 / std::max<long long>(1, tiles));
          k = std::min<long long>(k, stages / 8);
          if (k < 2 || stages > ctx->i8_chunk || ctx->big) return 1;
          const int per = (int)((stages + k - 1) / k);
          return (stages + per - 1) / per;
        };
        g.ksplit_a = pieces((long long)(g.nCp / I8_BM) * (NPp / ctx->i8_bn), ctx->i8_nks);
        g.ksplit_l = pieces((long long)(g.nCp / I8_BM) * (ctx->i8_NRp / ctx->i8_bn), ctx->i8_nkp);
        if (g.ksplit_a > 1) RC(dalloc(ctx, &g.Gpart, (size_t)g.ksplit_a * g.n * ctx->DP * ctx->DP));
        if (g.ksplit_a == 1 && ctx->i8_bn == 128 && NP % 128 != 0 && ctx->opt.i8_tail != 0) {
          const int ntail = (NP % 128 + 31) / 32;
          g.tail_pieces = (int)std::max<long long>(1, std::min<long long>(8, 256 / ((long long)(g.nCp / I8_BM) * ntail)));
          RC(dalloc(ctx, &g.Tq, (size_t)g.tail_pieces * S * g.nCp * 32 * ntail));
        }
        if (g.ksplit_l > 1) RC(dalloc(ctx, &g.Rpart, (size_t)g.ksplit_l * g.n * ctx->Mp));
      }
      I8_SWITCH(ctx, {
        constexpr int lds = i8_lds_bytes<S_, WN_, TN_>();
        auto kfn = k_assemble_i8<S_, WN_, TN_>;
        HIPCK(hipFuncSetAttribute((const void*)kfn, hipFuncAttributeMaxDynamicSharedMemorySize, lds));
        auto kfn2 = k_leverage_i8<S_, WN_, TN_>;
        HIPCK(hipFuncSetAttribute((const void*)kfn2, hipFuncAttributeMaxDynamicSharedMemorySize, lds));
        auto kfn3 = k_assemble_i8_tail<S_>;
        HIPCK(hipFuncSetAttribute((const void*)kfn3, hipFuncAttributeMaxDynamicSharedMemorySize, (i8_lds_bytes<S_, 1, 1>())));
      });
      if (S == 6) {
        constexpr int ld = i8_lds_bytes<6, 4, 1>() > i8_lds_bytes<4, 4, 1>() ? i8_lds_bytes<6, 4, 1>() : i8_lds_bytes<4, 4, 1>();
        constexpr int ldt = i8_lds_bytes<6, 1, 1>() > i8_lds_bytes<4, 1, 1>() ? i8_lds_bytes<6, 1, 1>() : i8_lds_bytes<4, 1, 1>();
        HIPCK(hipFuncSetAttribute((const void*)k_assemble_i8_sel<4, 1>, hipFuncAttributeMaxDynamicSharedMemorySize, ld));
        HIPCK(hipFuncSetAttribute((const void*)k_assemble_i8_tail_sel, hipFuncAttributeMaxDynamicSharedMemorySize, ldt));
      }
      if (S == 6)
        for (int sv = S - 2; sv < S; ++sv)
          I8_SWITCH_S(sv, {
            auto kfn = k_assemble_i8<S_, WN_, TN_>;
            HIPCK(hipFuncSetAttribute((const void*)kfn, hipFuncAttributeMaxDynamicSharedMemorySize, (i8_lds_bytes<S_, WN_, TN_>())));
            auto kfn2 = k_leverage_i8<S_, WN_, TN_>;
            HIPCK(hipFuncSetAttribute((const void*)kfn2, hipFuncAttributeMaxDynamicSharedMemorySize, (i8_lds_bytes<S_, WN_, TN_>())));
            auto kfn3 = k_assemble_i8_tail<S_>;
            HIPCK(hipFuncSetAttribute((const void*)kfn3, hipFuncAttributeMaxDynamicSharedMemorySize, (i8_lds_bytes<S_, 1, 1>())));
          });
    }
    {
      const int need = std::max(g.fsplit, g.ksplit_a);
      if (g.fsplit > 1 && (!g.Gpart || g.fsplit > g.ksplit_a)) RC(dalloc(ctx, &g.Gpart, (size_t)need * g.n * ctx->DP * ctx->DP));
    }
    RC(dalloc(ctx, &ctx->d_z, n * (size_t)D)); RC(dalloc(ctx, &ctx->d_ulen, n)); RC(dalloc(ctx, &ctx->d_gdir, n)); RC(dalloc(ctx, &ctx->d_uacc, n));
    if (ctx->big) {
      RC(dalloc(ctx, &ctx->d_Wd, n * (size_t)ctx->nbk * 4096));
      if (!(flags & RMHMC_FLAG_INT8_METRIC)) RC(dalloc(ctx, &ctx->d_hpart, (size_t)ctx->npairs * n * Mp));
    }
    fill_int(ctx, ch.cstale, 1, n);
    RC(dalloc(ctx, &ctx->d_nsteps, n)); RC(dalloc(ctx, &ctx->d_dir, n)); RC(dalloc(ctx, &ctx->d_done, 1)); RC(dalloc(ctx, &ctx->d_steps0, n));
    RC(dalloc(ctx, &ctx->d_miniter, 1));
    RC(dalloc(ctx, &ctx->d_orig, n)); RC(dalloc(ctx, &ctx->d_T, 2 * n));
    {
      const bool on = ctx->opt.medium && !ctx->big && D > FS_D && D <= 32 && ctx->Mp <= MS_MAXMP && n_chains <= 512;
      if (on) {
        const size_t lds = sizeof(double) * (ctx->NB == 1 ? ms_lds_doubles<1>(ctx->Mp) : ms_lds_doubles<2>(ctx->Mp));
        if (ctx->NB == 1) {
          HIPCK(hipFuncSetAttribute((const void*)k_step_medium<1, 0>, hipFuncAttributeMaxDynamicSharedMemorySize, MAX_LDS));
          HIPCK(hipFuncSetAttribute((const void*)k_step_medium<1, 1>, hipFuncAttributeMaxDynamicSharedMemorySize, MAX_LDS));
          HIPCK(hipFuncSetAttribute((const void*)k_step_medium<1, 2>, hipFuncAttributeMaxDynamicSharedMemorySize, MAX_LDS));
          HIPCK(hipFuncSetAttribute((const void*)k_step_medium<1, 3>, hipFuncAttributeMaxDynamicSharedMemorySize, MAX_LDS));
          HIPCK(hipFuncSetAttribute((const void*)k_step_medium<1, 4>, hipFuncAttributeMaxDynamicSharedMemorySize, MAX_LDS));
        } else {
          HIPCK(hipFuncSetAttribute((const void*)k_step_medium<2, 0>, hipFuncAttributeMaxDynamicSharedMemorySize, MAX_LDS));
          HIPCK(hipFuncSetAttribute((const void*)k_step_medium<2, 1>, hipFuncAttributeMaxDynamicSharedMemorySize, MAX_LDS));
          HIPCK(hipFuncSetAttribute((const void*)k_step_medium<2, 2>, hipFuncAttributeMaxDynamicSharedMemorySize, MAX_LDS));
        }
        ctx->medium = true;
        ctx->medium_lds = lds;
      }
    }
    {
      long long maxn = ctx->Mp <= 1024 ? (1ll << 40) : 512;
      if (ctx->opt.hmc_traj_maxn >= 0) maxn = ctx->opt.hmc_traj_maxn;
      ctx->hmc_traj = ctx->opt.medium && !ctx->big && D <= 32 && n_chains <= maxn;
    }
    {
      const size_t lds = ((size_t)(FS_D + 1 + FS_WAVES) * ctx->Mp + (size_t)FS_WAVES * FS_PT) * sizeof(double);
      if (ctx->opt.fused && D <= FS_D && lds <= 160 * 1024) {
        HIPCK(hipFuncSetAttribute((const void*)k_fused_small, hipFuncAttributeMaxDynamicSharedMemorySize, MAX_LDS));
        ctx->fused = true;
        ctx->fused_lds = lds;
      }
    }
    RC(sync(ctx));
    return RMHMC_OK;
  };
  rc = body();
  if (rc != RMHMC_OK) {
    snprintf(g_err, 512, "%s", ctx->err);
    rmhmc_destroy(ctx);
    return rc;
  }
  apply_runtime_options(ctx);
  *out = ctx;
  return RMHMC_OK;
}

void rmhmc_destroy(rmhmc_ctx* ctx) {
  if (!ctx) return;
  (void)hipSetDevice(ctx->device);
  if (ctx->stream) (void)hipStreamSynchronize(ctx->stream);
  for (auto& e : ctx->flow) if (e) (void)hipEventDestroy(e);
  for (auto& kv : ctx->events) for (auto& e : kv.second) { (void)hipEventDestroy(e.a); (void)hipEventDestroy(e.b); }
  for (auto& e : ctx->pool) { (void)hipEventDestroy(e.a); (void)hipEventDestroy(e.b); }
  for (void* p : ctx->allocs) (void)hipFree(p);
  if (ctx->stream) (void)hipStreamDestroy(ctx->stream);
  delete ctx;
}

int rmhmc_set_option(rmhmc_ctx* ctx, const char* key, int64_t value) {
  if (!ctx) return fail(nullptr, RMHMC_ERR_INVALID, "set_option: null context");
  const OptionDesc* d = find_option(key);
  if (!d) return fail(ctx, RMHMC_ERR_INVALID, std::string("set_option: unknown option '") + (key ? key : "(null)") + "'");
  if (d->create_only) return fail(ctx, RMHMC_ERR_INVALID, std::string("set_option: '") + key + "' shapes the context and can only be given to rmhmc_create_opts");
  if (value < d->lo || value > d->hi) return fail(ctx, RMHMC_ERR_INVALID, std::string("set_option: value out of range for '") + key + "'");
  HIPCK(hipSetDevice(ctx->device));
  HIPCK(hipStreamSynchronize(ctx->stream));
  ctx->opt.*(d->slot) = value;
  apply_runtime_options(ctx);
  if (ctx->stale_list_alloc) {
    HIPCK(hipMemsetAsync(ctx->batch.ch.stale_count, 0, sizeof(int), ctx->stream));
    fill_int(ctx, ctx->batch.ch.cstale, 1, ctx->n);
    HIPCK(hipStreamSynchronize(ctx->stream));
  }
  return RMHMC_OK;
}
int rmhmc_get_option(rmhmc_ctx* ctx, const char* key, int64_t* value_out) {
  if (!ctx || !value_out) return fail(ctx, RMHMC_ERR_INVALID, "get_option: null pointer");
  const OptionDesc* d = find_option(key);
  if (!d) return fail(ctx, RMHMC_ERR_INVALID, std::string("get_option: unknown option '") + (key ? key : "(null)") + "'");
  *value_out = ctx->opt.*(d->slot);
  return RMHMC_OK;
}
int rmhmc_options(rmhmc_ctx* ctx, char* buf, size_t len) {
  if (!ctx || !buf || !len) return fail(ctx, RMHMC_ERR_INVALID, "options: bad argument");
  std::string o;
  for (const OptionDesc& d : kOptions) o += (o.empty() ? "" : " ") + std::string(d.key) + "=" + std::to_string(ctx->opt.*(d.slot));
  snprintf(buf, len, "%s", o.c_str());
  return RMHMC_OK;
}

int rmhmc_device_info(rmhmc_ctx* ctx, char* buf, size_t len) {
  if (!ctx || !buf) return fail(ctx, RMHMC_ERR_INVALID, "device_info: bad argument");
  hipDeviceProp_t prop;
  HIPCK(hipGetDeviceProperties(&prop, ctx->device));
  snprintf(buf, len, "%s %s, %d CUs, %.0f MHz, %.1f GiB; M=%lld (padded %d) D=%d (padded %d, %d MFMA tiles) chains=%lld%s",
           prop.name, prop.gcnArchName, prop.multiProcessorCount, prop.clockRate / 1000.0, prop.totalGlobalMem / 1073741824.0,
           (long long)ctx->M, ctx->Mp, ctx->D, ctx->DP, ctx->NB * (ctx->NB + 1) / 2, (long long)ctx->n,
           ctx->fused ? ", fused small-problem path" : ctx->medium ? ", one-launch step" : ctx->big ? ", blocked large-D path" : "");
  if (ctx->i8_requested) {
    const size_t k = strlen(buf);
    snprintf(buf + k, len > k ? len - k : 0, "; int8 metric path %d slices: %s (certificate %.2e%s)", ctx->i8S,
             ctx->i8 ? "active" : "NOT certified for this data, fp64 matrix cores used", ctx->i8_bound,
             ctx->have_data ? "" : ", no data yet");
  }
  {
    const size_t k = strlen(buf);
    if (len > k + 12) {
      snprintf(buf + k, len - k, "; options: ");
      const size_t k2 = strlen(buf);
      (void)rmhmc_options(ctx, buf + k2, len - k2);
    }
  }
  return RMHMC_OK;
}

int rmhmc_set_data(rmhmc_ctx* ctx, const double* X, const double* t, double alpha) {
  if (!ctx || !X || !t || !(alpha > 0)) return fail(ctx, RMHMC_ERR_INVALID, "set_data: bad argument");
  HIPCK(hipSetDevice(ctx->device));
  const size_t M = ctx->M, D = ctx->D, DP = ctx->DP, Mp = ctx->Mp;
  std::vector<double> xr(Mp * DP, 0.0), xt(DP * Mp, 0.0), tt(Mp, 0.0);
  for (size_t n = 0; n < M; ++n) {
    for (size_t d = 0; d < D; ++d) {
      xr[n * DP + d] = X[n * D + d];
      xt[d * Mp + n] = X[n * D + d];
    }
    tt[n] = t[n];
  }
  HIPCK(hipMemcpyAsync((void*)ctx->dd.Xr, xr.data(), xr.size() * 8, hipMemcpyHostToDevice, ctx->stream));
  HIPCK(hipMemcpyAsync((void*)ctx->dd.Xt, xt.data(), xt.size() * 8, hipMemcpyHostToDevice, ctx->stream));
  HIPCK(hipMemcpyAsync((void*)ctx->dd.t, tt.data(), tt.size() * 8, hipMemcpyHostToDevice, ctx->stream));
  if (ctx->i8_requested) {
    std::vector<int> cexp(DP, 0);
    std::vector<double> cmin(DP, 0.0), cmax(DP, 0.0);
    for (size_t d = 0; d < D; ++d) {
      double m = 0.0, lo = INFINITY;
      for (size_t n = 0; n < M; ++n) { const double a = std::fabs(X[n * D + d]); m = std::max(m, a); lo = std::min(lo, a); }
      if (m > 0.0 && m < 1e300) (void)std::frexp(m, &cexp[d]);
      if (m < 1e300) { cmin[d] = lo; cmax[d] = m; }
    }
    HIPCK(hipMemcpyAsync((void*)ctx->pairs.cexp, cexp.data(), sizeof(int) * DP, hipMemcpyHostToDevice, ctx->stream));
    HIPCK(hipMemcpyAsync(ctx->d_cmin, cmin.data(), sizeof(double) * DP, hipMemcpyHostToDevice, ctx->stream));
    HIPCK(hipMemcpyAsync(ctx->d_cmax, cmax.data(), sizeof(double) * DP, hipMemcpyHostToDevice, ctx->stream));
    RC(sync(ctx));
    hipLaunchKernelGGL(k_zmax, dim3((unsigned)ctx->pairs.NPp), dim3(256), 0, ctx->stream, ctx->dd.Xt, (int)M, (int)Mp, ctx->pairs, ctx->d_ze,
                       (double*)ctx->pairs.scale);
    const dim3 grid((unsigned)((ctx->i8_nks * 8 + 255) / 256), (unsigned)ctx->pairs.NPp);
    I8_SWITCH(ctx, hipLaunchKernelGGL((k_zsplit<S_>), grid, dim3(256), 0, ctx->stream, ctx->dd.Xt, (int)M, (int)Mp, ctx->pairs, ctx->d_ze,
                                      ctx->i8_nks, ctx->d_Zs); (void)WN_; (void)TN_);
    hipLaunchKernelGGL(k_zrowmax, dim3((unsigned)((ctx->i8_NRp + 255) / 256)), dim3(256), 0, ctx->stream, ctx->dd.Xr, (int)M, (int)D, (int)DP,
                       ctx->i8_NRp, ctx->pairs.cexp, ctx->d_zre, ctx->d_zscale);
    const dim3 gridt((unsigned)(ctx->i8_NRp / 32), (unsigned)ctx->i8_nkp);
    I8_SWITCH(ctx, hipLaunchKernelGGL((k_ztsplit<S_>), gridt, dim3(256), 0, ctx->stream, ctx->dd.Xr, (int)M, (int)DP, ctx->pairs, ctx->d_zre,
                                      ctx->i8_nkp, ctx->i8_NRp, ctx->d_Zt); (void)WN_; (void)TN_);
    HIPCK(hipGetLastError());
  }
  RC(sync(ctx));
  if (ctx->i8_requested) {
    std::vector<int> ze(ctx->pairs.NP);
    HIPCK(hipMemcpy(ze.data(), ctx->d_ze, sizeof(int) * ze.size(), hipMemcpyDeviceToHost));
    std::vector<double> g0(D, 1.0 / alpha);
    for (size_t n = 0; n < M; ++n)
      for (size_t d = 0; d < D; ++d) g0[d] += 0.25 * X[n * D + d] * X[n * D + d];
    double bound = 0.0;
    for (size_t a = 0, q = 0; a < D; ++a)
      for (size_t b = 0; b <= a; ++b, ++q)
        bound = std::max(bound, std::ldexp((double)ctx->i8S * (double)M, ze[q] - 8 * ctx->i8S) / std::sqrt(g0[a] * g0[b]));
    if (ctx->opt.i8_delta && ctx->i8S == 6) bound *= (2.0 * ctx->i8S - 1.0) / ctx->i8S;
    ctx->i8_bound = bound;
    const bool ok = !(ctx->flags & RMHMC_FLAG_INT8_CERTIFY) || bound <= RMHMC_INT8_CERTIFY_TOL;
    if (!ok && ctx->big && !ctx->d_hpart) RC(dalloc(ctx, &ctx->d_hpart, (size_t)ctx->npairs * ctx->n * Mp));
    ctx->i8 = ok;
    RC(sync(ctx));
  }
  ctx->alpha = alpha;
  ctx->dd.inv_alpha = 1.0 / alpha;
  ctx->dd.log_prior_const = -0.5 * std::log(2.0 * M_PI * alpha);
  ctx->have_data = true;
  ctx->chains_ready = false;
  return RMHMC_OK;
}

int rmhmc_log_posterior(rmhmc_ctx* ctx, const double* w, double* ljl_out) {
  NEED_DATA(ctx);
  if (!w || !ljl_out) return fail(ctx, RMHMC_ERR_INVALID, "log_posterior: null pointer");
  ctx->chains_ready = false;
  RC(eval_at(ctx, w, nullptr));
  RC(download(ctx, ljl_out, ctx->batch.ch.trj.ljl, ctx->n));
  return sync(ctx);
}

int rmhmc_metric(rmhmc_ctx* ctx, const double* w, double* G_out, double* half_logdet_out, double* grad_out) {
  NEED_DATA(ctx);
  if (!w) return fail(ctx, RMHMC_ERR_INVALID, "metric: null pointer");
  ctx->chains_ready = false;
  if (ctx->big && G_out && !ctx->d_Gcopy) RC(dalloc(ctx, &ctx->d_Gcopy, (size_t)ctx->n * ctx->DP * ctx->DP));
  ctx->want_G = ctx->big && G_out;
  int rc_eval = eval_at(ctx, w, nullptr);
  ctx->want_G = false;
  RC(rc_eval);
  if (G_out)
    for (int64_t c = 0; c < ctx->n; ++c)
      HIPCK(hipMemcpy2DAsync(G_out + c * ctx->D * ctx->D, ctx->D * 8, (ctx->big ? ctx->d_Gcopy : ctx->batch.ch.Gq) + c * ctx->DP * ctx->DP, ctx->DP * 8, ctx->D * 8, ctx->D,
                             hipMemcpyDeviceToHost, ctx->stream));
  if (half_logdet_out) RC(download(ctx, half_logdet_out, ctx->batch.ch.trj.hld, ctx->n));
  if (grad_out) RC(download_vec(ctx, grad_out, ctx->batch.ch.trj.grad));
  RC(sync(ctx));
  if (G_out && ctx->i8) {
    const int64_t D = ctx->D;
    for (int64_t c = 0; c < ctx->n; ++c)
      for (int64_t a = 0; a < D; ++a)
        for (int64_t b = a + 1; b < D; ++b) G_out[(c * D + a) * D + b] = G_out[(c * D + b) * D + a];
  }
  return RMHMC_OK;
}

int rmhmc_metric_terms(rmhmc_ctx* ctx, const double* w, const double* p, double* trace_out, double* quad_out) {
  NEED_DATA(ctx);
  if (!w) return fail(ctx, RMHMC_ERR_INVALID, "metric_terms: null pointer");
  ctx->chains_ready = false;
  RC(eval_at(ctx, w, p));
  if (trace_out) RC(download_vec(ctx, trace_out, ctx->batch.ch.trj.tr));
  if (quad_out && p) RC(download_vec(ctx, quad_out, ctx->batch.ch.last));
  return sync(ctx);
}

int rmhmc_leapfrog(rmhmc_ctx* ctx, double* w, double* p, double eps, const int32_t* dir, const int32_t* nsteps, int32_t K,
                   double* half_logdet_out, int32_t* status_out) {
  NEED_DATA(ctx);
  if (!w || !p || !dir || !nsteps || K < 1) return fail(ctx, RMHMC_ERR_INVALID, "leapfrog: null pointer or K < 1");
  ctx->chains_ready = false;
  int maxs = 0;
  for (int64_t c = 0; c < ctx->n; ++c) {
    if (nsteps[c] < 0 || (dir[c] != 1 && dir[c] != -1)) return fail(ctx, RMHMC_ERR_INVALID, "leapfrog: nsteps >= 0 and dir = +-1 required");
    if (nsteps[c] > maxs) maxs = nsteps[c];
  }
  ctx->eps = eps; ctx->K = K;
  RC(upload(ctx, ctx->d_nsteps, nsteps, ctx->n));
  RC(upload(ctx, ctx->d_dir, dir, ctx->n));
  RC(eval_at(ctx, w, p));
  Group& g = ctx->batch;
  launch(ctx, "small", [&](hipStream_t st) {
    hipLaunchKernelGGL(k_set_leapfrog, dim3((unsigned)((g.n + 255) / 256)), dim3(256), 0, st, g.n, ctx->d_nsteps, ctx->d_dir, g.ch);
  });
  for (int s = 0; s < maxs; ++s) {
    step_phases(ctx, g);
    launch(ctx, "small", [&](hipStream_t st) {
      hipLaunchKernelGGL(k_park_finished, dim3((unsigned)((g.n + 255) / 256)), dim3(256), 0, st, g.n, g.ch);
    });
  }
  RC(download_vec(ctx, w, ctx->batch.ch.trj.w));
  RC(download_vec(ctx, p, ctx->batch.ch.p));
  if (half_logdet_out) RC(download(ctx, half_logdet_out, ctx->batch.ch.trj.hld, ctx->n));
  if (status_out) RC(download(ctx, status_out, ctx->batch.ch.status, ctx->n));
  return sync(ctx);
}

static int init_chains(rmhmc_ctx* ctx, const double* theta0_host , bool allow_fused = true, bool allow_medium = true) {
  Group& g = ctx->batch;
  std::vector<double> th;
  if (!theta0_host) {
    th.assign((size_t)ctx->n * ctx->D, 1e-3);
    theta0_host = th.data();
  }
  if (ctx->fused && allow_fused) {
    RC(upload_vec(ctx, g.ch.cur.w, theta0_host));
    FusedParams fp{};
    fp.ip = iter_params(ctx, IterBase{0, 0, 0, nullptr, false, false});
    fp.eps = ctx->eps; fp.K = ctx->K; fp.nsteps = 0; fp.DPs = ctx->DP; fp.init_eval = 1;
    launch(ctx, "fused", [&](hipStream_t st) {
      hipLaunchKernelGGL(k_fused_small, dim3((unsigned)((g.n + FS_WAVES - 1) / FS_WAVES)), dim3(64 * FS_WAVES), ctx->fused_lds, st,
                         ctx->dd, g.ch, fp);
    });
  } else {
    RC(eval_at(ctx, theta0_host, nullptr, allow_medium));
    SMALL(ctx, g, "small", k_commit_all, ctx->D, ctx->DP, g.ch);
  }
  fill_int(ctx, ctx->batch.ch.phase, 0, ctx->n);
  fill_int(ctx, ctx->batch.ch.steps_left, 0, ctx->n);
  fill_int(ctx, ctx->batch.ch.status, 0, ctx->n);
  fill_ll(ctx, ctx->batch.ch.iter, 0, ctx->n);
  fill_ll(ctx, ctx->batch.ch.accepted, 0, ctx->n);
  fill_ll(ctx, ctx->batch.ch.steps_done, 0, ctx->n);
  HIPCK(hipMemsetAsync(ctx->d_done, 0, sizeof(int), ctx->stream));
  return sync(ctx);
}

int rmhmc_transition(rmhmc_ctx* ctx, double* w, const double* z, const double* u_len, const double* g_dir, const double* u_acc,
                     int32_t L, double eps, int32_t K, int32_t* accepted_out, int32_t* nsteps_out, double* H_cur_out,
                     double* H_prop_out, double* w_prop_out, double* p_prop_out, double* half_logdet_prop_out, int32_t* status_out) {
  NEED_DATA(ctx);
  if (!w || !z || !u_len || !g_dir || !u_acc || L < 1 || K < 1) return fail(ctx, RMHMC_ERR_INVALID, "transition: null pointer, L < 1 or K < 1");
  ctx->chains_ready = false;
  ctx->L = L; ctx->eps = eps; ctx->K = K;
  RC(init_chains(ctx, w));
  RC(upload(ctx, ctx->d_z, z, (size_t)ctx->n * ctx->D));
  RC(upload(ctx, ctx->d_ulen, u_len, ctx->n));
  RC(upload(ctx, ctx->d_gdir, g_dir, ctx->n));
  RC(upload(ctx, ctx->d_uacc, u_acc, ctx->n));
  const IterBase ib{1, 0, 0, nullptr, true, false};
  if (ctx->fused) {
    launch_fused(ctx, ib, L);
  } else {
    Group& g = ctx->batch;
    launch_iter_begin(ctx, g, ib);
    launch_iter_end(ctx, g, ib);
    for (int s = 0; s < L; ++s) {
      step_phases(ctx, g);
      launch_iter_end(ctx, g, ib);
    }
  }
  std::vector<long long> acc(ctx->n);
  RC(download_vec(ctx, w, ctx->batch.ch.cur.w));
  RC(download(ctx, acc.data(), ctx->batch.ch.accepted, ctx->n));
  if (nsteps_out) RC(download(ctx, nsteps_out, ctx->batch.ch.nsteps_last, ctx->n));
  if (H_cur_out) RC(download(ctx, H_cur_out, ctx->batch.ch.Hcur, ctx->n));
  if (H_prop_out) RC(download(ctx, H_prop_out, ctx->batch.ch.Hprop, ctx->n));
  if (w_prop_out) RC(download_vec(ctx, w_prop_out, ctx->batch.ch.trj.w));
  if (p_prop_out) RC(download_vec(ctx, p_prop_out, ctx->batch.ch.p));
  if (half_logdet_prop_out) RC(download(ctx, half_logdet_prop_out, ctx->batch.ch.trj.hld, ctx->n));
  if (status_out) RC(download(ctx, status_out, ctx->batch.ch.status, ctx->n));
  RC(sync(ctx));
  if (accepted_out) for (int64_t c = 0; c < ctx->n; ++c) accepted_out[c] = (int32_t)acc[c];
  return RMHMC_OK;
}

struct StepGraph {
  hipGraph_t graph = nullptr;
  hipGraphExec_t exec = nullptr;
  ~StepGraph() {
    if (exec) (void)hipGraphExecDestroy(exec);
    if (graph) (void)hipGraphDestroy(graph);
  }
};
static bool step_graph_usable(const rmhmc_ctx* ctx, long long nsteps) {
  if (ctx->timing || nsteps < 8) return false;
  if (ctx->fused && ctx->sampler == 0) return false;
  if (ctx->medium && ctx->sampler == 0) return false;
  return ctx->opt.graph != 0;
}
static bool build_step_graph(rmhmc_ctx* ctx, const IterBase& ib, StepGraph& sg) {
  if (hipStreamBeginCapture(ctx->stream, hipStreamCaptureModeThreadLocal) != hipSuccess) return false;
  launch_global_step(ctx, ctx->batch, ib);
  if (hipStreamEndCapture(ctx->stream, &sg.graph) != hipSuccess || !sg.graph) { (void)hipGetLastError(); return false; }
  if (hipGraphInstantiate(&sg.exec, sg.graph, nullptr, nullptr, 0) != hipSuccess) { (void)hipGetLastError(); sg.exec = nullptr; return false; }
  return true;
}
static void run_generic_steps(rmhmc_ctx* ctx, const IterBase& ib, long long nsteps, StepGraph* sg) {
  if (sg && sg->exec) {
    for (long long s = 0; s < nsteps; ++s) { (void)hipGraphLaunch(sg->exec, ctx->stream); flow_tick(ctx); }
  } else {
    for (long long s = 0; s < nsteps; ++s) { launch_global_step(ctx, ctx->batch, ib); flow_tick(ctx); }
  }
}

static int poll_progress(rmhmc_ctx* ctx, int* done, long long* min_iter) {
  HIPCK(hipMemsetAsync(ctx->d_miniter, 0xff, sizeof(unsigned long long), ctx->stream));
  hipLaunchKernelGGL(k_min_iter, dim3((unsigned)((ctx->n + 255) / 256)), dim3(256), 0, ctx->stream, ctx->batch.ch.iter, (size_t)ctx->n, ctx->d_miniter);
  unsigned long long mi = 0;
  HIPCK(hipMemcpyAsync(done, ctx->d_done, sizeof(int), hipMemcpyDeviceToHost, ctx->stream));
  HIPCK(hipMemcpyAsync(&mi, ctx->d_miniter, sizeof(mi), hipMemcpyDeviceToHost, ctx->stream));
  RC(sync(ctx));
  *min_iter = (long long)mi;
  return RMHMC_OK;
}

static int report_progress(rmhmc_ctx* ctx, int event, long long iters) {
  std::vector<long long> acc(ctx->n), it(ctx->n);
  RC(download(ctx, acc.data(), ctx->batch.ch.accepted, ctx->n));
  RC(download(ctx, it.data(), ctx->batch.ch.iter, ctx->n));
  RC(sync(ctx));
  long long tot = 0, tit = 0;
  for (long long a : acc) tot += a;
  for (long long a : it) tit += a;
  ctx->progress_fn(event, iters, tot, tit, ctx->progress_user);
  return RMHMC_OK;
}
static bool progress_ticking(const rmhmc_ctx* ctx) { return ctx->progress_fn && ctx->progress_every > 0 && ctx->n > 1; }
static int progress_fire(rmhmc_ctx* ctx, long long min_iter) {
  if (!progress_ticking(ctx)) return RMHMC_OK;
  long long last = -1;
  while (ctx->progress_next <= min_iter) { last = ctx->progress_next; ctx->progress_next += ctx->progress_every; }
  if (last >= 0) RC(report_progress(ctx, RMHMC_EV_PROGRESS, last));
  return RMHMC_OK;
}

static int run_until_done(rmhmc_ctx* ctx, const IterBase& ib, long long min_steps) {
  int done = 0;
  long long s = min_steps, min_iter = 0;
  const long long poll = 4;
  const bool fused = ctx->fused && ctx->sampler == 0;
  const bool ticking = progress_ticking(ctx);
  const long long chunk = ticking ? std::max<long long>(8, ctx->progress_every * (ctx->L + 1) / 2) : min_steps;
  StepGraph sg;
  if (!fused && step_graph_usable(ctx, std::min(min_steps, chunk))) (void)build_step_graph(ctx, ib, sg);
  for (long long left = min_steps; left > 0;) {
    const long long k = std::min(left, chunk);
    if (fused) launch_fused(ctx, ib, k);
    else run_generic_steps(ctx, ib, k, &sg);
    left -= k;
    if (ticking && left > 0) {
      RC(poll_progress(ctx, &done, &min_iter));
      RC(progress_fire(ctx, min_iter));
    }
  }
  for (;;) {
    RC(poll_progress(ctx, &done, &min_iter));
    RC(progress_fire(ctx, min_iter));
    if (done >= ctx->n) break;
    long long next = std::max(poll, ib.limit - min_iter);
    if (ticking) next = std::min(next, chunk);
    if (fused) launch_fused(ctx, ib, next);
    else run_generic_steps(ctx, ib, next, &sg);
    s += next;
    if (s > min_steps * (long long)ctx->L + 1000000) return fail(ctx, RMHMC_ERR_RUNTIME, "sampler did not terminate");
  }
  return RMHMC_OK;
}

static int run_phase(rmhmc_ctx* ctx, const IterBase& ib, long long from, bool at_from = false, bool at_limit = false) {
  if (ctx->progress_fn && ctx->progress_every > 0 && ctx->n == 1) {
    long long m = ctx->progress_first;
    if (from > m) m += ((from - m + ctx->progress_every - 1) / ctx->progress_every) * ctx->progress_every;
    if (m == from) {
      if (at_from) RC(report_progress(ctx, RMHMC_EV_PROGRESS, m));
      m += ctx->progress_every;
    }
    for (; m < ib.limit || (at_limit && m == ib.limit); m += ctx->progress_every) {
      IterBase seg = ib;
      seg.limit = m;
      HIPCK(hipMemsetAsync(ctx->d_done, 0, sizeof(int), ctx->stream));
      RC(run_until_done(ctx, seg, m - from));
      RC(report_progress(ctx, RMHMC_EV_PROGRESS, m));
      from = m;
    }
    HIPCK(hipMemsetAsync(ctx->d_done, 0, sizeof(int), ctx->stream));
  }
  if (ib.limit > from) RC(run_until_done(ctx, ib, ib.limit - from));
  return RMHMC_OK;
}

static void launch_global_step_prefix(rmhmc_ctx* ctx, const IterBase& ib, int na) {
  Group g = ctx->batch;
  g.n = na; g.ch.n = na;
  if (g.nCp) g.nCp = (na + I8_BM - 1) / I8_BM * I8_BM;
  launch_global_step(ctx, g, ib);
}

static int run_sorted_phase(rmhmc_ctx* ctx, const IterBase& ib, const std::vector<long long>& T ) {
  const int n = (int)ctx->n;
  const long long Tmin = T[n - 1], Tmax = T[0];
  const bool ticking = progress_ticking(ctx);
  const long long chunk = ticking ? std::max<long long>(8, ctx->progress_every * (ctx->L + 1) / 2) : Tmax + 1;
  int done = 0;
  long long mi = 0;
  {
    StepGraph sg;
    if (step_graph_usable(ctx, std::min(Tmin, chunk))) (void)build_step_graph(ctx, ib, sg);
    for (long long left = Tmin; left > 0;) {
      const long long k = std::min(left, chunk);
      run_generic_steps(ctx, ib, k, &sg);
      left -= k;
      if (ticking) { RC(poll_progress(ctx, &done, &mi)); RC(progress_fire(ctx, mi)); }
    }
    HIPCK(hipStreamSynchronize(ctx->stream));
  }
  int na = n;
  for (long long s = Tmin; s < Tmax; ++s) {
    while (na > 0 && T[na - 1] <= s) --na;
    const int nar = std::min(n, (na + 127) / 128 * 128);
    if (nar == n) launch_global_step(ctx, ctx->batch, ib);
    else launch_global_step_prefix(ctx, ib, nar);
    flow_tick(ctx);
    if (ticking && (s - Tmin) % chunk == chunk - 1) { RC(poll_progress(ctx, &done, &mi)); RC(progress_fire(ctx, mi)); }
  }
  RC(poll_progress(ctx, &done, &mi));
  RC(progress_fire(ctx, mi));
  if (done < n) RC(run_until_done(ctx, ib, 1));
  return RMHMC_OK;
}

static int sample_core(rmhmc_ctx* ctx, int64_t n_iter, int64_t burn_in, const double* theta0, double* d_samples, double* seconds_out) {
  const long long S = n_iter - burn_in;
  const int n = (int)ctx->n;
  std::vector<long long> T;
  std::vector<double> th_perm;
  bool sorted = ctx->sampler == 0 && !ctx->fused && n >= 2 && n_iter > burn_in + 1;
  ctx->progress_next = ctx->progress_first;
  sorted = sorted && ctx->opt.sorted;
  if (sorted) {
    hipLaunchKernelGGL(k_traj_steps, dim3((unsigned)((n + 255) / 256)), dim3(256), 0, ctx->stream, (unsigned long long)ctx->seed,
                       (long long)ctx->chain_offset, ctx->L, (long long)burn_in + 1, (long long)n_iter, (size_t)n, ctx->d_T);
    std::vector<long long> t0(n);
    RC(download(ctx, t0.data(), ctx->d_T, (size_t)n));
    RC(sync(ctx));
    std::vector<int> orig(n);
    for (int i = 0; i < n; ++i) orig[i] = i;
    std::stable_sort(orig.begin(), orig.end(), [&](int a, int b) { return t0[a] > t0[b]; });
    T.resize(n);
    for (int i = 0; i < n; ++i) T[i] = t0[orig[i]];
    RC(upload(ctx, ctx->d_orig, orig.data(), (size_t)n));
    RC(sync(ctx));
    th_perm.resize((size_t)n * ctx->D);
    for (int i = 0; i < n; ++i)
      for (int d = 0; d < ctx->D; ++d) th_perm[(size_t)i * ctx->D + d] = theta0 ? theta0[(size_t)orig[i] * ctx->D + d] : 1e-3;
    theta0 = th_perm.data();
  }
  ctx->sorted = sorted;
  int rc = [&]() -> int {
    RC(init_chains(ctx, theta0));
    const IterBase ipA{burn_in + 1, burn_in, S, d_samples, false, true};
    RC(run_phase(ctx, ipA, 0));
    HIPCK(hipMemcpyAsync(ctx->d_steps0, ctx->batch.ch.steps_done, sizeof(long long) * ctx->n, hipMemcpyDeviceToDevice, ctx->stream));
    HIPCK(hipMemsetAsync(ctx->d_done, 0, sizeof(int), ctx->stream));
    RC(sync(ctx));
    if (ctx->progress_fn) RC(report_progress(ctx, RMHMC_EV_BURNIN_DONE, burn_in + 1));
    const auto t0 = std::chrono::steady_clock::now();
    if (n_iter > burn_in + 1) {
      const IterBase ipB{n_iter, burn_in, S, d_samples, false, true};
      if (sorted) RC(run_sorted_phase(ctx, ipB, T));
      else RC(run_phase(ctx, ipB, burn_in + 1, true));
    }
    RC(sync(ctx));
    if (seconds_out) *seconds_out = std::chrono::duration<double>(std::chrono::steady_clock::now() - t0).count();
    hipLaunchKernelGGL(k_sub_ll, dim3((unsigned)((ctx->n + 255) / 256)), dim3(256), 0, ctx->stream, ctx->d_steps0, ctx->batch.ch.steps_done, (size_t)ctx->n);
    if (sorted) {
      const dim3 grid((unsigned)((n + 255) / 256));
      hipLaunchKernelGGL(k_scatter_ll, grid, dim3(256), 0, ctx->stream, ctx->d_T, ctx->batch.ch.accepted, ctx->d_orig, (size_t)n);
      hipLaunchKernelGGL(k_scatter_ll, grid, dim3(256), 0, ctx->stream, ctx->d_T + n, ctx->d_steps0, ctx->d_orig, (size_t)n);
    }
    return RMHMC_OK;
  }();
  ctx->sorted = false;
  ctx->counters_sorted = sorted && rc == RMHMC_OK;
  return rc;
}
static int sample_counters(rmhmc_ctx* ctx, int64_t* accept_out, int64_t* steps_out, hipMemcpyKind kind) {
  static_assert(sizeof(long long) == sizeof(int64_t), "int64");
  const long long* acc = ctx->counters_sorted ? ctx->d_T : ctx->batch.ch.accepted;
  const long long* stp = ctx->counters_sorted ? ctx->d_T + ctx->n : ctx->d_steps0;
  if (accept_out) HIPCK(hipMemcpyAsync(accept_out, acc, sizeof(int64_t) * ctx->n, kind, ctx->stream));
  if (steps_out) HIPCK(hipMemcpyAsync(steps_out, stp, sizeof(int64_t) * ctx->n, kind, ctx->stream));
  return RMHMC_OK;
}

static int sample_impl(rmhmc_ctx* ctx, int64_t n_iter, int64_t burn_in, int32_t L, double eps, int32_t K, uint64_t seed, int64_t chain_offset,
                       const double* theta0, double* samples_out, int64_t* accept_out, int64_t* steps_out, double* seconds_out, bool dev) {
  NEED_DATA(ctx);
  if (!samples_out || burn_in < 0 || burn_in >= n_iter || L < 1 || K < 1)
    return fail(ctx, RMHMC_ERR_INVALID, "sample: need samples_out, 0 <= burn_in < n_iter, L >= 1, K >= 1");
  ctx->chains_ready = false;
  ctx->L = L; ctx->eps = eps; ctx->K = K; ctx->seed = seed; ctx->chain_offset = chain_offset;
  const size_t count = (size_t)ctx->n * (n_iter - burn_in) * ctx->D;
  double* d_samples = dev ? samples_out : nullptr;
  if (!dev) HIPCK(hipMalloc((void**)&d_samples, sizeof(double) * count));
  int rc = [&]() -> int {
    RC(sample_core(ctx, n_iter, burn_in, theta0, d_samples, seconds_out));
    if (!dev) HIPCK(hipMemcpyAsync(samples_out, d_samples, sizeof(double) * count, hipMemcpyDeviceToHost, ctx->stream));
    RC(sample_counters(ctx, accept_out, steps_out, dev ? hipMemcpyDeviceToDevice : hipMemcpyDeviceToHost));
    return sync(ctx);
  }();
  if (!dev && d_samples) (void)hipFree(d_samples);
  return rc;
}

int rmhmc_sample(rmhmc_ctx* ctx, int64_t n_iter, int64_t burn_in, int32_t L, double eps, int32_t K, uint64_t seed,
                 int64_t chain_offset, const double* theta0, double* samples_out, int64_t* accept_out, int64_t* steps_out,
                 double* seconds_out) {
  return sample_impl(ctx, n_iter, burn_in, L, eps, K, seed, chain_offset, theta0, samples_out, accept_out, steps_out, seconds_out, false);
}
int rmhmc_sample_dev(rmhmc_ctx* ctx, int64_t n_iter, int64_t burn_in, int32_t L, double eps, int32_t K, uint64_t seed,
                     int64_t chain_offset, const double* theta0, double* samples_dev, int64_t* accept_dev, int64_t* steps_dev,
                     double* seconds_out) {
  return sample_impl(ctx, n_iter, burn_in, L, eps, K, seed, chain_offset, theta0, samples_dev, accept_dev, steps_dev, seconds_out, true);
}

static int launch_ess(rmhmc_ctx* ctx, const double* d_samples, long long nblocks, long long S, int P, double* d_ess, double* d_mean, double* d_var) {
  if (S < 2 || S > 20000) return fail(ctx, RMHMC_ERR_UNSUPPORTED, "ess: 2 <= S <= 20000 samples per chain (the centred series is held in LDS)");
  HIPCK(hipFuncSetAttribute((const void*)k_ess, hipFuncAttributeMaxDynamicSharedMemorySize, MAX_LDS));
  long long nfft = 0;
  if (ctx->flags & RMHMC_FLAG_ESS_WRAP) { nfft = 1; while (nfft < S) nfft *= 2; nfft += 1; }
  hipLaunchKernelGGL(k_ess, dim3((unsigned)(nblocks * P)), dim3(64), (size_t)S * sizeof(double), ctx->stream, d_samples, S, P, d_ess, d_mean, d_var, nfft);
  return RMHMC_OK;
}

int rmhmc_ess(rmhmc_ctx* ctx, const double* samples, int64_t n, int64_t S, int32_t P, double* ess_out) {
  if (!ctx || !samples || !ess_out || n < 1 || P < 1 || n * (int64_t)P > 0x7fffffffLL) return fail(ctx, RMHMC_ERR_INVALID, "ess: bad argument");
  HIPCK(hipSetDevice(ctx->device));
  double *d_s = nullptr, *d_e = nullptr;
  HIPCK(hipMalloc((void**)&d_s, sizeof(double) * (size_t)n * S * P));
  int rc = [&]() -> int {
    HIPCK(hipMalloc((void**)&d_e, sizeof(double) * (size_t)n * P));
    HIPCK(hipMemcpyAsync(d_s, samples, sizeof(double) * (size_t)n * S * P, hipMemcpyHostToDevice, ctx->stream));
    RC(launch_ess(ctx, d_s, n, S, P, d_e, nullptr, nullptr));
    HIPCK(hipMemcpyAsync(ess_out, d_e, sizeof(double) * (size_t)n * P, hipMemcpyDeviceToHost, ctx->stream));
    return sync(ctx);
  }();
  (void)hipFree(d_s);
  if (d_e) (void)hipFree(d_e);
  return rc;
}

static int sample_stats_impl(rmhmc_ctx* ctx, int64_t n_iter, int64_t burn_in, int32_t L, double eps, int32_t K, uint64_t seed,
                             int64_t chain_offset, const double* theta0, double* mean_out, double* var_out, double* ess_out,
                             int64_t* accept_out, int64_t* steps_out, double* seconds_out, bool dev) {
  NEED_DATA(ctx);
  if (burn_in < 0 || burn_in >= n_iter || L < 1 || K < 1)
    return fail(ctx, RMHMC_ERR_INVALID, "sample_stats: need 0 <= burn_in < n_iter, L >= 1, K >= 1");
  ctx->chains_ready = false;
  ctx->L = L; ctx->eps = eps; ctx->K = K; ctx->seed = seed; ctx->chain_offset = chain_offset;
  const long long S = n_iter - burn_in;
  double* d_samples = nullptr;
  double* d_out = nullptr;
  HIPCK(hipMalloc((void**)&d_samples, sizeof(double) * (size_t)ctx->n * S * ctx->D));
  int rc = [&]() -> int {
    RC(sample_core(ctx, n_iter, burn_in, theta0, d_samples, seconds_out));
    const size_t nd = (size_t)ctx->n * ctx->D;
    HIPCK(hipMalloc((void**)&d_out, sizeof(double) * 3 * nd));
    RC(launch_ess(ctx, d_samples, ctx->n, S, ctx->D, d_out, d_out + nd, d_out + 2 * nd));
    const hipMemcpyKind kind = dev ? hipMemcpyDeviceToDevice : hipMemcpyDeviceToHost;
    if (ess_out) HIPCK(hipMemcpyAsync(ess_out, d_out, sizeof(double) * nd, kind, ctx->stream));
    if (mean_out) HIPCK(hipMemcpyAsync(mean_out, d_out + nd, sizeof(double) * nd, kind, ctx->stream));
    if (var_out) HIPCK(hipMemcpyAsync(var_out, d_out + 2 * nd, sizeof(double) * nd, kind, ctx->stream));
    RC(sample_counters(ctx, accept_out, steps_out, kind));
    return sync(ctx);
  }();
  if (d_samples) (void)hipFree(d_samples);
  if (d_out) (void)hipFree(d_out);
  return rc;
}
int rmhmc_sample_stats(rmhmc_ctx* ctx, int64_t n_iter, int64_t burn_in, int32_t L, double eps, int32_t K, uint64_t seed,
                       int64_t chain_offset, const double* theta0, double* mean_out, double* var_out, double* ess_out,
                       int64_t* accept_out, int64_t* steps_out, double* seconds_out) {
  return sample_stats_impl(ctx, n_iter, burn_in, L, eps, K, seed, chain_offset, theta0, mean_out, var_out, ess_out, accept_out, steps_out,
                           seconds_out, false);
}
int rmhmc_sample_stats_dev(rmhmc_ctx* ctx, int64_t n_iter, int64_t burn_in, int32_t L, double eps, int32_t K, uint64_t seed,
                           int64_t chain_offset, const double* theta0, double* mean_dev, double* var_dev, double* ess_dev,
                           int64_t* accept_dev, int64_t* steps_dev, double* seconds_out) {
  return sample_stats_impl(ctx, n_iter, burn_in, L, eps, K, seed, chain_offset, theta0, mean_dev, var_dev, ess_dev, accept_dev, steps_dev,
                           seconds_out, true);
}

static int hmc_init_chains(rmhmc_ctx* ctx, const double* theta0_host ) {
  std::vector<double> th;
  if (!theta0_host) { th.assign((size_t)ctx->n * ctx->D, 0.0); theta0_host = th.data(); }
  RC(upload_vec(ctx, ctx->batch.ch.trj.w, theta0_host));
  fill_int(ctx, ctx->batch.ch.phase, 1, ctx->n);
  Group& g = ctx->batch;
  if (ctx->hmc_traj) {
    launch_hmc_traj(ctx, g, 1);
  } else {
    launch_rowpass<RP_G>(ctx, g, g.ch.trj.w, nullptr);
    SMALL(ctx, g, "small", k_hmc_init, ctx->dd, g.ch, g.nsplit);
  }
  fill_int(ctx, ctx->batch.ch.phase, 0, ctx->n);
  fill_int(ctx, ctx->batch.ch.steps_left, 0, ctx->n);
  fill_int(ctx, ctx->batch.ch.status, 0, ctx->n);
  fill_ll(ctx, ctx->batch.ch.iter, 0, ctx->n);
  fill_ll(ctx, ctx->batch.ch.accepted, 0, ctx->n);
  fill_ll(ctx, ctx->batch.ch.steps_done, 0, ctx->n);
  HIPCK(hipMemsetAsync(ctx->d_done, 0, sizeof(int), ctx->stream));
  return sync(ctx);
}

int rmhmc_hmc_transition(rmhmc_ctx* ctx, double* w, const double* z, const double* u_len, const double* u_acc, int32_t L, double eps,
                         int32_t* accepted_out, int32_t* nsteps_out, double* H_cur_out, double* H_prop_out, double* w_prop_out,
                         double* p_prop_out) {
  NEED_DATA(ctx);
  if (!w || !z || !u_len || !u_acc || L < 1) return fail(ctx, RMHMC_ERR_INVALID, "hmc_transition: null pointer or L < 1");
  ctx->chains_ready = false;
  ctx->L = L; ctx->eps = eps; ctx->sampler = 1;
  int rc = [&]() -> int {
    RC(hmc_init_chains(ctx, w));
    RC(upload(ctx, ctx->d_z, z, (size_t)ctx->n * ctx->D));
    RC(upload(ctx, ctx->d_ulen, u_len, ctx->n));
    RC(upload(ctx, ctx->d_uacc, u_acc, ctx->n));
    const IterBase ib{1, 0, 0, nullptr, true, false};
    for (int s = 0; s < L; ++s) launch_hmc_global_step(ctx, ctx->batch, ib);
    std::vector<long long> acc(ctx->n);
    RC(download_vec(ctx, w, ctx->batch.ch.cur.w));
    RC(download(ctx, acc.data(), ctx->batch.ch.accepted, ctx->n));
    if (nsteps_out) RC(download(ctx, nsteps_out, ctx->batch.ch.nsteps_last, ctx->n));
    if (H_cur_out) RC(download(ctx, H_cur_out, ctx->batch.ch.Hcur, ctx->n));
    if (H_prop_out) RC(download(ctx, H_prop_out, ctx->batch.ch.Hprop, ctx->n));
    if (w_prop_out) RC(download_vec(ctx, w_prop_out, ctx->batch.ch.trj.w));
    if (p_prop_out) RC(download_vec(ctx, p_prop_out, ctx->batch.ch.p));
    RC(sync(ctx));
    if (accepted_out) for (int64_t c = 0; c < ctx->n; ++c) accepted_out[c] = (int32_t)acc[c];
    return RMHMC_OK;
  }();
  ctx->sampler = 0;
  return rc;
}

int rmhmc_hmc_sample(rmhmc_ctx* ctx, int64_t n_iter, int64_t burn_in, int32_t L, double eps, uint64_t seed, int64_t chain_offset,
                     const double* theta0, double* samples_out, int64_t* accept_out, int64_t* steps_out, double* seconds_out) {
  NEED_DATA(ctx);
  if (!samples_out || burn_in < 0 || burn_in >= n_iter || L < 1)
    return fail(ctx, RMHMC_ERR_INVALID, "hmc_sample: need samples_out, 0 <= burn_in < n_iter, L >= 1");
  ctx->chains_ready = false;
  ctx->L = L; ctx->eps = eps; ctx->seed = seed; ctx->chain_offset = chain_offset;
  const long long S = n_iter - burn_in;
  double* d_samples = nullptr;
  HIPCK(hipMalloc((void**)&d_samples, sizeof(double) * (size_t)ctx->n * S * ctx->D));
  ctx->sampler = 1;
  ctx->progress_next = ctx->progress_first;
  int rc = [&]() -> int {
    RC(hmc_init_chains(ctx, theta0));
    const IterBase ipA{burn_in + 1, burn_in, S, d_samples, false, true};
    RC(run_phase(ctx, ipA, 0, false, true));
    HIPCK(hipMemcpyAsync(ctx->d_steps0, ctx->batch.ch.steps_done, sizeof(long long) * ctx->n, hipMemcpyDeviceToDevice, ctx->stream));
    HIPCK(hipMemsetAsync(ctx->d_done, 0, sizeof(int), ctx->stream));
    RC(sync(ctx));
    if (ctx->progress_fn) RC(report_progress(ctx, RMHMC_EV_BURNIN_DONE, burn_in + 1));
    const auto t0 = std::chrono::steady_clock::now();
    if (n_iter > burn_in + 1) {
      const rmhmc_progress_fn fn = ctx->progress_fn;
      ctx->progress_fn = nullptr;
      const IterBase ipB{n_iter, burn_in, S, d_samples, false, true};
      const int rcB = run_phase(ctx, ipB, burn_in + 1);
      ctx->progress_fn = fn;
      RC(rcB);
    }
    RC(sync(ctx));
    if (seconds_out) *seconds_out = std::chrono::duration<double>(std::chrono::steady_clock::now() - t0).count();
    HIPCK(hipMemcpyAsync(samples_out, d_samples, sizeof(double) * (size_t)ctx->n * S * ctx->D, hipMemcpyDeviceToHost, ctx->stream));
    std::vector<long long> a(ctx->n), s1(ctx->n), s0(ctx->n);
    RC(download(ctx, a.data(), ctx->batch.ch.accepted, ctx->n));
    RC(download(ctx, s1.data(), ctx->batch.ch.steps_done, ctx->n));
    RC(download(ctx, s0.data(), ctx->d_steps0, ctx->n));
    RC(sync(ctx));
    for (int64_t c = 0; c < ctx->n; ++c) {
      if (accept_out) accept_out[c] = a[c];
      if (steps_out) steps_out[c] = s1[c] - s0[c];
    }
    return RMHMC_OK;
  }();
  (void)hipFree(d_samples);
  ctx->sampler = 0;
  return rc;
}

static void launch_mmala_step(rmhmc_ctx* ctx, Group& g, const IterBase& b) {
  const double eps = ctx->eps;
  const int full = (ctx->flags & RMHMC_FLAG_MMALA_FULL) ? 1 : 0;
  const IterParams ip = iter_params(ctx, b);
  SMALL(ctx, g, "small", k_mmala_begin, ctx->D, ctx->DP, g.ch, ip, eps, full);
  eval_point_phases(ctx, g, false, full ? 2 : 1);
  SMALL(ctx, g, "small", k_mmala_end, ctx->D, ctx->DP, g.ch, ip, eps, full);
}
static int mmala_init(rmhmc_ctx* ctx, const double* theta0_host, bool allow_medium = true) {
  std::vector<double> th;
  if (!theta0_host) { th.assign((size_t)ctx->n * ctx->D, 0.0); theta0_host = th.data(); }
  return init_chains(ctx, theta0_host, false, allow_medium);
}

int rmhmc_mmala_transition(rmhmc_ctx* ctx, double* w, const double* z, const double* u_acc, double eps, int32_t* accepted_out,
                           double* ratio_out, double* w_prop_out) {
  NEED_DATA(ctx);
  if (!w || !z || !u_acc || !(eps > 0)) return fail(ctx, RMHMC_ERR_INVALID, "mmala_transition: null pointer or eps <= 0");
  ctx->chains_ready = false;
  ctx->eps = eps;
  RC(mmala_init(ctx, w));
  RC(upload(ctx, ctx->d_z, z, (size_t)ctx->n * ctx->D));
  RC(upload(ctx, ctx->d_uacc, u_acc, ctx->n));
  const IterBase ib{1, 0, 0, nullptr, true, false};
  launch_mmala_step(ctx, ctx->batch, ib);
  std::vector<long long> acc(ctx->n);
  RC(download_vec(ctx, w, ctx->batch.ch.cur.w));
  RC(download(ctx, acc.data(), ctx->batch.ch.accepted, ctx->n));
  if (ratio_out) RC(download(ctx, ratio_out, ctx->batch.ch.Hprop, ctx->n));
  if (w_prop_out) RC(download_vec(ctx, w_prop_out, ctx->batch.ch.trj.w));
  RC(sync(ctx));
  if (accepted_out) for (int64_t c = 0; c < ctx->n; ++c) accepted_out[c] = (int32_t)acc[c];
  return RMHMC_OK;
}

int rmhmc_mmala_sample(rmhmc_ctx* ctx, int64_t n_iter, int64_t burn_in, double eps, uint64_t seed, int64_t chain_offset,
                       const double* theta0, double* samples_out, int64_t* accept_out, double* seconds_out) {
  NEED_DATA(ctx);
  if (!samples_out || burn_in < 0 || burn_in >= n_iter || !(eps > 0))
    return fail(ctx, RMHMC_ERR_INVALID, "mmala_sample: need samples_out, 0 <= burn_in < n_iter, eps > 0");
  ctx->chains_ready = false;
  ctx->eps = eps; ctx->seed = seed; ctx->chain_offset = chain_offset;
  const long long S = n_iter - burn_in;
  double* d_samples = nullptr;
  HIPCK(hipMalloc((void**)&d_samples, sizeof(double) * (size_t)ctx->n * S * ctx->D));
  int rc = [&]() -> int {
    RC(mmala_init(ctx, theta0));
    const IterBase ib{n_iter, burn_in, S, d_samples, false, false};
    for (int64_t it = 0; it <= burn_in; ++it) { launch_mmala_step(ctx, ctx->batch, ib); flow_tick(ctx); }
    RC(sync(ctx));
    const auto t0 = std::chrono::steady_clock::now();
    for (int64_t it = burn_in + 1; it < n_iter; ++it) { launch_mmala_step(ctx, ctx->batch, ib); flow_tick(ctx); }
    RC(sync(ctx));
    if (seconds_out) *seconds_out = std::chrono::duration<double>(std::chrono::steady_clock::now() - t0).count();
    HIPCK(hipMemcpyAsync(samples_out, d_samples, sizeof(double) * (size_t)ctx->n * S * ctx->D, hipMemcpyDeviceToHost, ctx->stream));
    if (accept_out) {
      static_assert(sizeof(long long) == sizeof(int64_t), "int64");
      RC(download(ctx, (long long*)accept_out, ctx->batch.ch.accepted, ctx->n));
    }
    return sync(ctx);
  }();
  (void)hipFree(d_samples);
  return rc;
}

int rmhmc_chains_init(rmhmc_ctx* ctx, const double* theta0, uint64_t seed, int64_t chain_offset, int32_t L, double eps, int32_t K) {
  NEED_DATA(ctx);
  if (L < 1 || K < 1) return fail(ctx, RMHMC_ERR_INVALID, "chains_init: L >= 1 and K >= 1 required");
  ctx->L = L; ctx->eps = eps; ctx->K = K; ctx->seed = seed; ctx->chain_offset = chain_offset;
  RC(init_chains(ctx, theta0));
  if (ctx->batch.dcount) HIPCK(hipMemsetAsync(ctx->batch.dcount, 0, 6 * sizeof(unsigned long long), ctx->stream));
  ctx->chains_ready = true;
  return RMHMC_OK;
}

int rmhmc_chains_run(rmhmc_ctx* ctx, int64_t n_steps) {
  NEED_DATA(ctx);
  if (!ctx->chains_ready) return fail(ctx, RMHMC_ERR_INVALID, "chains_run: rmhmc_chains_init has not been called");
  const IterBase ib{(long long)1 << 62, 0, 0, nullptr, false, false};
  {
    Timed t(ctx, "total", ctx->stream);
    if (ctx->fused) {
      launch_fused(ctx, ib, n_steps);
    } else {
      StepGraph sg;
      if (step_graph_usable(ctx, n_steps)) (void)build_step_graph(ctx, ib, sg);
      run_generic_steps(ctx, ib, n_steps, &sg);
      HIPCK(hipStreamSynchronize(ctx->stream));
    }
  }
  return sync(ctx);
}

static int chains_state_impl(rmhmc_ctx* ctx, double* w_out, int64_t* iters_out, int64_t* accept_out, bool dev) {
  NEED_DATA(ctx);
  if (!ctx->chains_ready) return fail(ctx, RMHMC_ERR_INVALID, "chains_state: rmhmc_chains_init has not been called");
  const hipMemcpyKind kind = dev ? hipMemcpyDeviceToDevice : hipMemcpyDeviceToHost;
  if (w_out)
    HIPCK(hipMemcpy2DAsync(w_out, ctx->D * sizeof(double), ctx->batch.ch.cur.w, ctx->DP * sizeof(double), ctx->D * sizeof(double), ctx->n, kind, ctx->stream));
  static_assert(sizeof(long long) == sizeof(int64_t), "int64");
  if (iters_out) HIPCK(hipMemcpyAsync(iters_out, ctx->batch.ch.iter, sizeof(int64_t) * ctx->n, kind, ctx->stream));
  if (accept_out) HIPCK(hipMemcpyAsync(accept_out, ctx->batch.ch.accepted, sizeof(int64_t) * ctx->n, kind, ctx->stream));
  return sync(ctx);
}
int rmhmc_chains_state(rmhmc_ctx* ctx, double* w_out, int64_t* iters_out, int64_t* accept_out) {
  return chains_state_impl(ctx, w_out, iters_out, accept_out, false);
}
int rmhmc_chains_state_dev(rmhmc_ctx* ctx, double* w_dev, int64_t* iters_dev, int64_t* accept_dev) {
  return chains_state_impl(ctx, w_dev, iters_dev, accept_dev, true);
}

int rmhmc_chains_restore(rmhmc_ctx* ctx, const int64_t* iters, const int64_t* accepted) {
  NEED_DATA(ctx);
  if (!ctx->chains_ready || !iters || !accepted) return fail(ctx, RMHMC_ERR_INVALID, "chains_restore: call rmhmc_chains_init first");
  for (int64_t c = 0; c < ctx->n; ++c)
    if (iters[c] < 0 || accepted[c] < 0) return fail(ctx, RMHMC_ERR_INVALID, "chains_restore: negative counter");
  RC(upload(ctx, ctx->batch.ch.iter, (const long long*)iters, ctx->n));
  RC(upload(ctx, ctx->batch.ch.accepted, (const long long*)accepted, ctx->n));
  return sync(ctx);
}

int rmhmc_set_progress(rmhmc_ctx* ctx, rmhmc_progress_fn fn, int64_t first, int64_t every, void* user) {
  if (!ctx || (fn && (first < 1 || every < 1))) return fail(ctx, RMHMC_ERR_INVALID, "set_progress: first >= 1 and every >= 1 required");
  ctx->progress_fn = fn; ctx->progress_first = first; ctx->progress_every = every; ctx->progress_user = user;
  return RMHMC_OK;
}

int rmhmc_int8_certificate(rmhmc_ctx* ctx, double* bound_out, int32_t* active_out) {
  if (!ctx) return fail(nullptr, RMHMC_ERR_INVALID, "int8_certificate: null context");
  if (bound_out) *bound_out = ctx->i8_bound;
  if (active_out) *active_out = (ctx->i8_requested && ctx->i8) ? 1 : 0;
  return RMHMC_OK;
}

int rmhmc_kernel_time(rmhmc_ctx* ctx, const char* which, double* seconds_out, int64_t* launches_out) {
  if (!ctx || !which) return fail(ctx, RMHMC_ERR_INVALID, "kernel_time: bad argument");
  HIPCK(hipSetDevice(ctx->device));
  const std::string w(which);
  if (seconds_out) *seconds_out = 0.0;
  if (launches_out) *launches_out = 0;
  if (w == "enable") { ctx->timing = true; return RMHMC_OK; }
  if (w == "disable") { ctx->timing = false; return RMHMC_OK; }
  if (w == "reset") {
    RC(sync(ctx));
    for (auto& kv : ctx->events) { for (auto& e : kv.second) ctx->pool.push_back(e); kv.second.clear(); }
    return RMHMC_OK;
  }
  RC(sync(ctx));
  if (w.rfind("i8_delta_", 0) == 0) {
    static const char* const names[5] = {"i8_delta_end_s4", "i8_delta_end_s5", "i8_delta_end_s6", "i8_delta_inner_s4", "i8_delta_inner_s5"};
    const int slot = (int)(std::find_if(names, names + 5, [&](const char* s) { return w == s; }) - names);
    if (slot == 5) return fail(ctx, RMHMC_ERR_INVALID, "kernel_time: unknown delta counter " + w);
    if (ctx->batch.dcount) {
      unsigned long long h = 0;
      HIPCK(hipMemcpy(&h, ctx->batch.dcount + slot, sizeof(h), hipMemcpyDeviceToHost));
      if (launches_out) *launches_out = (int64_t)h;
    }
    return RMHMC_OK;
  }
  auto it = ctx->events.find(w);
  if (it == ctx->events.end()) return RMHMC_OK;
  double ms = 0.0;
  for (auto& e : it->second) {
    float m = 0.f;
    HIPCK(hipEventElapsedTime(&m, e.a, e.b));
    ms += m;
  }
  if (seconds_out) *seconds_out = ms * 1e-3;
  if (launches_out) *launches_out = (int64_t)it->second.size();
  return RMHMC_OK;
}

}

namespace {

void amh_shape(const rmhmc_ctx* ctx, int* nt, int* rows) {
  const long long M = ctx->M;
  const int NT = (M <= 64 * 16 && ctx->n >= 1024) ? 64 : 256;
  *nt = NT;
  *rows = M > AMH_MAX_ONCHIP_ROWS ? 0 : (int)((M + NT - 1) / NT);
}

int amh_run(rmhmc_ctx* ctx, AmhParams p, const double* theta0, double* seconds_out) {
  const size_t n = ctx->n, D = ctx->D, DP = ctx->DP;
  Chains& ch = ctx->batch.ch;
  std::vector<double> h((size_t)n * D, 0.0);
  RC(upload_vec(ctx, ch.cur.w, theta0 ? theta0 : h.data()));
  std::fill(h.begin(), h.end(), 1.0);
  RC(upload_vec(ctx, ch.PM, h.data()));
  HIPCK(hipMemsetAsync(ch.u0, 0, sizeof(double) * n * DP, ctx->stream));
  fill_ll(ctx, ch.accepted, 0, n);
  p.w = ch.cur.w; p.sd = ch.PM; p.accw = ch.u0; p.ljl = ch.cur.ljl; p.accepted = ch.accepted; p.fa = ch.rv0; p.fb = ch.rv2;
  int NT = 256, R = 0;
  amh_shape(ctx, &NT, &R);
  const bool sampling = p.z_in == nullptr;
  const long long N = p.n_iter, B = p.burn_in;
  auto t0 = std::chrono::steady_clock::now();
  for (long long start = 0; start < N;) {
    long long end = std::min(N, start + 1000);
    if (start <= B) {
      end = std::min(end, B + 1);
      const long long rep = (start + 999) / 1000 * 1000;
      if (rep < B) end = std::min(end, rep + 1);
    }
    const long long per_iter = (long long)n * (long long)D * ctx->M;
    const long long step = std::max(1LL, AMH_LAUNCH_ROWS / std::max(1LL, per_iter));
    for (long long a = start; a < end; a += step) {
      p.it0 = a; p.it1 = std::min(end, a + step); p.carry = a > start ? 1 : 0;
      AMH_SWITCH(NT, R, hipLaunchKernelGGL((k_amh<NT_, R_>), dim3((unsigned)n), dim3(NT_), 0, ctx->stream, ctx->dd, p));
      HIPCK(hipGetLastError());
    }
    const long long last = end - 1;
    if (sampling && last <= B) {
      RC(sync(ctx));
      if (ctx->progress_fn && last % 1000 == 0 && last < B) ctx->progress_fn(RMHMC_EV_PROGRESS, last, 0, 0, ctx->progress_user);
      if (last == B) {
        if (ctx->progress_fn) ctx->progress_fn(RMHMC_EV_BURNIN_DONE, B, 0, 0, ctx->progress_user);
        t0 = std::chrono::steady_clock::now();
      }
    }
    start = end;
  }
  RC(sync(ctx));
  if (seconds_out) *seconds_out = std::chrono::duration<double>(std::chrono::steady_clock::now() - t0).count();
  return RMHMC_OK;
}

bool amh_iters_ok(int64_t n_iter, int64_t burn_in) { return burn_in >= 0 && burn_in < n_iter && n_iter <= (int64_t)0xffffffffLL; }

}

extern "C" {

int rmhmc_amh_sample(rmhmc_ctx* ctx, int64_t n_iter, int64_t burn_in, uint64_t seed, int64_t chain_offset, const double* theta0,
                     double* samples_out, int64_t* accepted_out, double* sd_out, double* seconds_out) {
  NEED_DATA(ctx);
  if (!samples_out || !amh_iters_ok(n_iter, burn_in) || chain_offset < 0)
    return fail(ctx, RMHMC_ERR_INVALID, "amh_sample: need samples_out, 0 <= burn_in < n_iter < 2^32, chain_offset >= 0");
  ctx->chains_ready = false;
  const size_t n = ctx->n, D = ctx->D, S = (size_t)(n_iter - burn_in);
  double* d_samples = nullptr;
  HIPCK(hipMalloc((void**)&d_samples, sizeof(double) * n * S * D));
  int rc = [&]() -> int {
    AmhParams p{};
    p.samples = d_samples; p.seed = seed; p.chain_offset = chain_offset; p.n_iter = n_iter; p.burn_in = burn_in;
    RC(amh_run(ctx, p, theta0, seconds_out));
    HIPCK(hipMemcpyAsync(samples_out, d_samples, sizeof(double) * n * S * D, hipMemcpyDeviceToHost, ctx->stream));
    std::vector<long long> a(n);
    RC(download(ctx, a.data(), ctx->batch.ch.accepted, n));
    if (sd_out) RC(download_vec(ctx, sd_out, ctx->batch.ch.PM));
    RC(sync(ctx));
    if (accepted_out) for (size_t c = 0; c < n; ++c) accepted_out[c] = a[c];
    return RMHMC_OK;
  }();
  (void)hipFree(d_samples);
  return rc;
}

int rmhmc_amh_replay(rmhmc_ctx* ctx, int64_t n_iter, int64_t burn_in, const double* z, const double* u, const double* theta0,
                     double* w_out, double* ljl_out, double* sd_out, int8_t* decisions_out) {
  NEED_DATA(ctx);
  if (!z || !u || !w_out || !ljl_out || !decisions_out || !amh_iters_ok(n_iter, burn_in))
    return fail(ctx, RMHMC_ERR_INVALID, "amh_replay: need z, u, w_out, ljl_out, decisions_out and 0 <= burn_in < n_iter < 2^32");
  ctx->chains_ready = false;
  const size_t n = ctx->n, D = ctx->D, T = (size_t)n_iter, vec = n * T * D;
  double *d_z = nullptr, *d_u = nullptr, *d_w = nullptr, *d_l = nullptr;
  int8_t* d_dec = nullptr;
  int rc = [&]() -> int {
    HIPCK(hipMalloc((void**)&d_z, sizeof(double) * vec)); HIPCK(hipMalloc((void**)&d_u, sizeof(double) * vec));
    HIPCK(hipMalloc((void**)&d_w, sizeof(double) * vec)); HIPCK(hipMalloc((void**)&d_l, sizeof(double) * n * T));
    HIPCK(hipMalloc((void**)&d_dec, vec));
    RC(upload(ctx, d_z, z, vec)); RC(upload(ctx, d_u, u, vec));
    AmhParams p{};
    p.z_in = d_z; p.u_in = d_u; p.w_out = d_w; p.ljl_out = d_l; p.dec_out = d_dec; p.n_iter = n_iter; p.burn_in = burn_in;
    RC(amh_run(ctx, p, theta0, nullptr));
    RC(download(ctx, w_out, d_w, vec)); RC(download(ctx, ljl_out, d_l, n * T)); RC(download(ctx, decisions_out, d_dec, vec));
    if (sd_out) RC(download_vec(ctx, sd_out, ctx->batch.ch.PM));
    return sync(ctx);
  }();
  for (void* q : {(void*)d_z, (void*)d_u, (void*)d_w, (void*)d_l, (void*)d_dec}) if (q) (void)hipFree(q);
  return rc;
}

}

namespace {

const char* const kIwlsDMsg = "iwls: D > 64 is not supported (64 < D <= 256 needs a blocked factorisation of G^-1 + 1e-6 I)";

struct IwlsState {
  double* lq = nullptr;
  int* sat = nullptr;
  long long* nsat = nullptr;
  double* mcur = nullptr;
};

int iwls_alloc(rmhmc_ctx* ctx, IwlsState& s, IwlsParams& p, int32_t compat) {
  const size_t n = ctx->n;
  HIPCK(hipMalloc((void**)&s.lq, sizeof(double) * 2 * n));
  HIPCK(hipMalloc((void**)&s.sat, sizeof(int) * n));
  HIPCK(hipMalloc((void**)&s.nsat, sizeof(long long) * n));
  HIPCK(hipMalloc((void**)&s.mcur, sizeof(double) * n * ctx->DP));
  HIPCK(hipMemsetAsync(s.lq, 0, sizeof(double) * 2 * n, ctx->stream));
  HIPCK(hipMemsetAsync(s.nsat, 0, sizeof(long long) * n, ctx->stream));
  p.compat = compat ? 1 : 0;
  p.lq_cur = s.lq; p.lq_trj = s.lq + n; p.sat = s.sat; p.nsat = s.nsat; p.mcur = s.mcur;
  return RMHMC_OK;
}
void iwls_free(IwlsState& s) {
  for (void* q : {(void*)s.lq, (void*)s.sat, (void*)s.nsat, (void*)s.mcur}) if (q) (void)hipFree(q);
}

void launch_iwls_ljit(rmhmc_ctx* ctx, Group& g, const double* Ginv, double* out) {
  launch(ctx, "iwls", [&](hipStream_t st) {
    NB_SWITCH(ctx, hipLaunchKernelGGL((k_iwls_ljit<NB_>), dim3((unsigned)g.n), dim3(64), 0, st, ctx->D, ctx->DP, Ginv, out));
  });
}

void launch_iwls_iter(rmhmc_ctx* ctx, Group& g, const IwlsParams& p) {
  SMALL(ctx, g, "iwls", k_iwls_begin, ctx->D, ctx->DP, g.ch, p);
  eval_point_phases(ctx, g, false, 1);
  if (p.compat) {
    launch_iwls_ljit(ctx, g, g.ch.trj.Ginv, p.lq_trj);
    launch(ctx, "iwls_sat", [&](hipStream_t st) {
      const dim3 grid((unsigned)((ctx->M + IWLS_SAT_ROWS - 1) / IWLS_SAT_ROWS), (unsigned)((g.n + IWLS_SAT_CH - 1) / IWLS_SAT_CH));
      hipLaunchKernelGGL(k_iwls_sat, grid, dim3(IWLS_SAT_ROWS), 0, st, ctx->dd, g.n, (const double*)g.ch.trj.w, p.sat);
    });
  }
  SMALL(ctx, g, "iwls", k_iwls_end, ctx->D, ctx->DP, g.ch, p);
}

int iwls_run(rmhmc_ctx* ctx, IwlsParams p, long long n_iter, bool sampling, const double* theta0, double* seconds_out) {
  Group& g = ctx->batch;
  RC(mmala_init(ctx, theta0, false));
  if (p.compat) launch_iwls_ljit(ctx, g, g.ch.cur.Ginv, p.lq_cur);
  std::vector<long long> acc;
  auto t0 = std::chrono::steady_clock::now();
  for (long long i = 0; i < n_iter; ++i) {
    if (sampling && (i % 1000 == 0 || i == p.burn_in)) {
      if (ctx->progress_fn) {
        acc.resize(ctx->n);
        RC(download(ctx, acc.data(), ctx->batch.ch.accepted, ctx->n));
        RC(sync(ctx));
        long long a = 0;
        for (long long x : acc) a += x;
        if (i % 1000 == 0) ctx->progress_fn(RMHMC_EV_PROGRESS, i, a, i * ctx->n, ctx->progress_user);
        if (i == p.burn_in) ctx->progress_fn(RMHMC_EV_BURNIN_DONE, i, a, i * ctx->n, ctx->progress_user);
      }
      if (i == p.burn_in) {
        RC(sync(ctx));
        t0 = std::chrono::steady_clock::now();
      }
    }
    p.it = i;
    launch_iwls_iter(ctx, g, p);
    HIPCK(hipGetLastError());
    flow_tick(ctx);
  }
  RC(sync(ctx));
  if (seconds_out) *seconds_out = std::chrono::duration<double>(std::chrono::steady_clock::now() - t0).count();
  return RMHMC_OK;
}

}

extern "C" {

int rmhmc_iwls_sample(rmhmc_ctx* ctx, int64_t n_iter, int64_t burn_in, int32_t compat, uint64_t seed, int64_t chain_offset,
                      const double* theta0, double* samples_out, int64_t* accepted_out, int64_t* saturated_out, double* seconds_out) {
  NEED_DATA(ctx);
  if (!samples_out || !amh_iters_ok(n_iter, burn_in) || chain_offset < 0)
    return fail(ctx, RMHMC_ERR_INVALID, "iwls_sample: need samples_out, 0 <= burn_in < n_iter < 2^32, chain_offset >= 0");
  if (ctx->D > 64) return fail(ctx, RMHMC_ERR_UNSUPPORTED, kIwlsDMsg);
  ctx->chains_ready = false;
  const size_t n = ctx->n, D = ctx->D, S = (size_t)(n_iter - burn_in);
  double* d_samples = nullptr;
  IwlsState s;
  int rc = [&]() -> int {
    HIPCK(hipMalloc((void**)&d_samples, sizeof(double) * n * S * D));
    IwlsParams p{};
    RC(iwls_alloc(ctx, s, p, compat));
    p.seed = seed; p.chain_offset = chain_offset; p.burn_in = burn_in; p.S = (long long)S; p.samples = d_samples; p.T = n_iter;
    RC(iwls_run(ctx, p, n_iter, true, theta0, seconds_out));
    HIPCK(hipMemcpyAsync(samples_out, d_samples, sizeof(double) * n * S * D, hipMemcpyDeviceToHost, ctx->stream));
    std::vector<long long> a(n), b(n);
    RC(download(ctx, a.data(), ctx->batch.ch.accepted, n));
    RC(download(ctx, b.data(), s.nsat, n));
    RC(sync(ctx));
    for (size_t c = 0; c < n; ++c) {
      if (accepted_out) accepted_out[c] = a[c];
      if (saturated_out) saturated_out[c] = b[c];
    }
    return RMHMC_OK;
  }();
  if (d_samples) (void)hipFree(d_samples);
  iwls_free(s);
  return rc;
}

int rmhmc_iwls_replay(rmhmc_ctx* ctx, int64_t n_iter, int32_t compat, const double* w_prop, const double* u, const double* theta0,
                      double* w_out, double* mean_out, double* ljl_out, double* ratio_out, int8_t* decisions_out) {
  NEED_DATA(ctx);
  if (!w_prop || !u || !w_out || n_iter < 1 || n_iter > (int64_t)0xffffffffLL)
    return fail(ctx, RMHMC_ERR_INVALID, "iwls_replay: need w_prop, u, w_out and 0 < n_iter < 2^32");
  if (ctx->D > 64) return fail(ctx, RMHMC_ERR_UNSUPPORTED, kIwlsDMsg);
  ctx->chains_ready = false;
  const size_t n = ctx->n, D = ctx->D, T = (size_t)n_iter, vec = n * T * D;
  double *d_wp = nullptr, *d_u = nullptr, *d_w = nullptr, *d_m = nullptr, *d_l = nullptr, *d_r = nullptr;
  int8_t* d_dec = nullptr;
  IwlsState s;
  int rc = [&]() -> int {
    HIPCK(hipMalloc((void**)&d_wp, sizeof(double) * vec)); HIPCK(hipMalloc((void**)&d_u, sizeof(double) * n * T));
    HIPCK(hipMalloc((void**)&d_w, sizeof(double) * vec)); HIPCK(hipMalloc((void**)&d_m, sizeof(double) * vec));
    HIPCK(hipMalloc((void**)&d_l, sizeof(double) * n * T)); HIPCK(hipMalloc((void**)&d_r, sizeof(double) * n * T));
    HIPCK(hipMalloc((void**)&d_dec, n * T));
    RC(upload(ctx, d_wp, w_prop, vec)); RC(upload(ctx, d_u, u, n * T));
    IwlsParams p{};
    RC(iwls_alloc(ctx, s, p, compat));
    p.T = n_iter; p.w_prop = d_wp; p.u_in = d_u; p.w_out = d_w; p.mean_out = d_m; p.ljl_out = d_l; p.ratio_out = d_r; p.dec_out = d_dec;
    RC(iwls_run(ctx, p, n_iter, false, theta0, nullptr));
    RC(download(ctx, w_out, d_w, vec));
    if (mean_out) RC(download(ctx, mean_out, d_m, vec));
    if (ljl_out) RC(download(ctx, ljl_out, d_l, n * T));
    if (ratio_out) RC(download(ctx, ratio_out, d_r, n * T));
    if (decisions_out) RC(download(ctx, decisions_out, d_dec, n * T));
    return sync(ctx);
  }();
  for (void* q : {(void*)d_wp, (void*)d_u, (void*)d_w, (void*)d_m, (void*)d_l, (void*)d_r, (void*)d_dec}) if (q) (void)hipFree(q);
  iwls_free(s);
  return rc;
}

}

namespace {

const char* const kGibbsDMsg = "gibbs: D > 64 is not supported (64 < D <= 256 needs a blocked inverse and sweep)";

struct GibbsState {
  double *Z = nullptr, *lam = nullptr, *ilam = nullptr, *B = nullptr, *beta = nullptr;
  long long *capped = nullptr, *dead = nullptr;
  int* stop = nullptr;
};
// ... 169 lines not shown
```

Measured before the change: 563,100.

## Cache step graph across calls and fuse iter-begin/end into neighbouring kernels

The step graph is now kept in the context and keyed on sampler configuration, so it is not rebuilt on every run call. Iteration parameters are written to a device buffer before each run so one captured graph can serve calls with different limits. Iteration begin is merged with the first Ginv matvec, and momentum-final is merged with iteration end, which removes two small launches per step. This adds cache-invalidation logic that could go stale if a relevant setting is missed, plus an extra parameter-write kernel per run.

```diff
diff --git a/riemannhamiltonianmontecarlo_amd/csrc/kernels.hip.h b/riemannhamiltonianmontecarlo_amd/csrc/kernels.hip.h
--- a/riemannhamiltonianmontecarlo_amd/csrc/kernels.hip.h
+++ b/riemannhamiltonianmontecarlo_amd/csrc/kernels.hip.h
@@ -1408,23 +1408,28 @@
   }
 }
 
+__device__ __forceinline__ void ginv_matvec64_dev(int D, int DP, const double* __restrict__ Gi, const double* __restrict__ src,
+                                                  double* __restrict__ uq, int c, int lane) {
+  const bool in = lane < D;
+  const double sv = in ? src[(size_t)c * DP + lane] : 0.0;
+  double u0 = 0.0;
+  for (int j0 = 0; j0 < D; j0 += 16) {
+    double g[16];
+#pragma unroll
+    for (int q = 0; q < 16; ++q) g[q] = (in && j0 + q < D) ? Gi[(j0 + q) * DP + lane] : 0.0;
+#pragma unroll
+    for (int q = 0; q < 16; ++q)
+      if (in && j0 + q < D) u0 = fma(g[q], rdlane(sv, j0 + q), u0);
+  }
+  if (in) uq[(size_t)c * DP + lane] = u0;
+}
+
 __global__ __launch_bounds__(64) void k_ginv_matvec(int D, int DP, Chains ch, const double* __restrict__ src) {
   const int c = blockIdx.x, lane = threadIdx.x;
   if (ch.phase[c] != 1) return;
   const double* __restrict__ Gi = ch.trj.Ginv + (size_t)c * DP * DP;
   if (D <= 64) {
-    const bool in = lane < D;
-    const double sv = in ? src[(size_t)c * DP + lane] : 0.0;
-    double u0 = 0.0;
-    for (int j0 = 0; j0 < D; j0 += 16) {
-      double g[16];
-#pragma unroll
-      for (int q = 0; q < 16; ++q) g[q] = (in && j0 + q < D) ? Gi[(j0 + q) * DP + lane] : 0.0;
-#pragma unroll
-      for (int q = 0; q < 16; ++q)
-        if (in && j0 + q < D) u0 = fma(g[q], rdlane(sv, j0 + q), u0);
-    }
-    if (in) ch.uq[(size_t)c * DP + lane] = u0;
+    ginv_matvec64_dev(D, DP, Gi, src, ch.uq, c, lane);
     return;
   }
   double u[RM_DCH] = {0.0, 0.0, 0.0, 0.0};
@@ -1492,9 +1497,7 @@
   if (in) ch.uq[o] = u;
 }
 
-__global__ __launch_bounds__(64) void k_mom_final(int D, int DP, Chains ch, double eps, int advance, int nsplit, const double* __restrict__ trpart = nullptr) {
-  const int c = blockIdx.x, lane = threadIdx.x;
-  if (ch.phase[c] != 1) return;
+__device__ __forceinline__ void mom_final_dev(int D, int DP, const Chains& ch, double eps, int advance, int nsplit, const double* __restrict__ trpart, int c, int lane) {
   const double h = ch.tau[c] * eps * 0.5;
   int nonfinite = 0;
   for (int d = lane; d < D; d += 64) {
@@ -1519,6 +1522,11 @@
       ch.steps_done[c] += 1;
     }
   }
+}
+__global__ __launch_bounds__(64) void k_mom_final(int D, int DP, Chains ch, double eps, int advance, int nsplit, const double* __restrict__ trpart = nullptr) {
+  const int c = blockIdx.x, lane = threadIdx.x;
+  if (ch.phase[c] != 1) return;
+  mom_final_dev(D, DP, ch, eps, advance, nsplit, trpart, c, lane);
 }
 
 struct IterParams {
@@ -1624,10 +1632,11 @@
   __builtin_amdgcn_wave_barrier();
 }
 
-__device__ __forceinline__ void iter_begin_dev(int D, int DP, const Chains& ch, const IterParams& ip, int c, int lane, double* zs, double* ps) {
-  if (ch.phase[c] != 0) return;
+__device__ __forceinline__ int iter_begin_dev(int D, int DP, const Chains& ch, const IterParams& ip, int c, int lane, double* zs, double* ps) {
+  const int ph0 = ch.phase[c];
+  if (ph0 != 0) return ph0;
   const long long it = ch.iter[c];
-  if (it >= ip.iter_limit) return;
+  if (it >= ip.iter_limit) return 0;
   if (!ch.cstale || ch.cstale[c]) copy_rec(ch.trj, ch.cur, c, D, DP, lane, ip.lower_L != 0);
   const long long oc = ip.orig ? ip.orig[c] : c;
   draw_normals(ip, c, it, D, lane, zs, oc);
@@ -1706,8 +1715,8 @@
   }
   __builtin_amdgcn_wave_barrier();
   const double quad = half_quadform(ch.cur.Ginv + (size_t)c * DP * DP, D, DP, lane, ps);
+  const int ns = (int)ceil(u_len * (double)ip.L);
   if (lane == 0) {
-    const int ns = (int)ceil(u_len * (double)ip.L);
     ch.steps_left[c] = ns;
     ch.nsteps_last[c] = ns;
     ch.tau[c] = (g_dir > 0.5) ? 1.0 : -1.0;
@@ -1715,17 +1724,32 @@
     ch.status[c] = st;
     ch.phase[c] = (ns > 0) ? 1 : 2;
   }
-}
-
-__global__ __launch_bounds__(64) void k_iter_begin(int D, int DP, Chains ch, IterParams ip) {
+  return (ns > 0) ? 1 : 2;
+}
+
+__global__ void k_set_iter_params(IterParams ip, IterParams* __restrict__ dst) {
+  if (blockIdx.x == 0 && threadIdx.x == 0) *dst = ip;
+}
+
+__global__ __launch_bounds__(64) void k_iter_begin(int D, int DP, Chains ch, IterParams ip, const IterParams* __restrict__ ipd) {
   __shared__ double zs[RM_DMAX];
   __shared__ double ps[RM_DMAX];
-  iter_begin_dev(D, DP, ch, ip, blockIdx.x, threadIdx.x, zs, ps);
-}
-
-__device__ __forceinline__ void iter_end_dev(int D, int DP, const Chains& ch, const IterParams& ip, int c, int lane, double* ps) {
-  const int ph = ch.phase[c];
-  if (!(ph == 2 || (ph == 1 && ch.steps_left[c] == 0))) return;
+  if (ipd) ip = *ipd;
+  (void)iter_begin_dev(D, DP, ch, ip, blockIdx.x, threadIdx.x, zs, ps);
+}
+
+__global__ __launch_bounds__(64) void k_iter_begin_matvec(int D, int DP, Chains ch, IterParams ip, const IterParams* __restrict__ ipd) {
+  __shared__ double zs[RM_DMAX];
+  __shared__ double ps[RM_DMAX];
+  if (ipd) ip = *ipd;
+  const int c = blockIdx.x, lane = threadIdx.x;
+  if (iter_begin_dev(D, DP, ch, ip, c, lane, zs, ps) != 1) return;
+  __threadfence_block();
+  ginv_matvec64_dev(D, DP, ch.trj.Ginv + (size_t)c * DP * DP, ch.p, ch.uq, c, lane);
+}
+
+__device__ __forceinline__ void iter_end_dev(int D, int DP, const Chains& ch, const IterParams& ip, int c, int lane, double* ps, int ph, int steps_left) {
+  if (!(ph == 2 || (ph == 1 && steps_left == 0))) return;
   const long long it = ch.iter[c];
   const long long oc = ip.orig ? ip.orig[c] : c;
   for (int d = lane; d < D; d += 64) ps[d] = ch.p[(size_t)c * DP + d];
@@ -1759,9 +1783,29 @@
   }
 }
 
-__global__ __launch_bounds__(64) void k_iter_end(int D, int DP, Chains ch, IterParams ip) {
+__device__ __forceinline__ void iter_end_dev(int D, int DP, const Chains& ch, const IterParams& ip, int c, int lane, double* ps) {
+  iter_end_dev(D, DP, ch, ip, c, lane, ps, ch.phase[c], ch.steps_left[c]);
+}
+
+__global__ __launch_bounds__(64) void k_iter_end(int D, int DP, Chains ch, IterParams ip, const IterParams* __restrict__ ipd) {
   __shared__ double ps[RM_DMAX];
+  if (ipd) ip = *ipd;
   iter_end_dev(D, DP, ch, ip, blockIdx.x, threadIdx.x, ps);
+}
+
+__global__ __launch_bounds__(64) void k_mom_final_end(int D, int DP, Chains ch, double eps, int nsplit, const double* __restrict__ trpart, IterParams ip,
+                                                      const IterParams* __restrict__ ipd) {
+  __shared__ double ps[RM_DMAX];
+  if (ipd) ip = *ipd;
+  const int c = blockIdx.x, lane = threadIdx.x;
+  const int ph = ch.phase[c];
+  int steps_left = ch.steps_left[c];
+  if (ph == 1) {
+    mom_final_dev(D, DP, ch, eps, 1, nsplit, trpart, c, lane);
+    steps_left -= 1;
+    __threadfence_block();
+  }
+  iter_end_dev(D, DP, ch, ip, c, lane, ps, ph, steps_left);
 }
 
 __global__ __launch_bounds__(64) void k_commit_all(int D, int DP, Chains ch) {
@@ -1795,8 +1839,9 @@
   __syncthreads();
   hmc_copy(ch.cur, ch.trj, c, dd.D, dd.DP, lane);
 }
-__global__ __launch_bounds__(64) void k_hmc_begin(int D, int DP, Chains ch, IterParams ip) {
+__global__ __launch_bounds__(64) void k_hmc_begin(int D, int DP, Chains ch, IterParams ip, const IterParams* __restrict__ ipd) {
   __shared__ double zs[RM_DMAX];
+  if (ipd) ip = *ipd;
   const int c = blockIdx.x, lane = threadIdx.x;
   if (ch.phase[c] != 0) return;
   const long long it = ch.iter[c];
@@ -1850,7 +1895,8 @@
     for (int d = lane; d < dd.D; d += 64) ch.p[(size_t)c * dd.DP + d] += eps * 0.5 * ch.trj.grad[(size_t)c * dd.DP + d];
   if (lane == 0) { ch.steps_left[c] -= 1; ch.steps_done[c] += 1; }
 }
-__global__ __launch_bounds__(64) void k_hmc_end(int D, int DP, Chains ch, IterParams ip) {
+__global__ __launch_bounds__(64) void k_hmc_end(int D, int DP, Chains ch, IterParams ip, const IterParams* __restrict__ ipd) {
+  if (ipd) ip = *ipd;
   const int c = blockIdx.x, lane = threadIdx.x;
   const int ph = ch.phase[c];
   if (!(ph == 2 || (ph == 1 && ch.steps_left[c] == 0))) return;
diff --git a/riemannhamiltonianmontecarlo_amd/csrc/rmhmc_hip.hip b/riemannhamiltonianmontecarlo_amd/csrc/rmhmc_hip.hip
--- a/riemannhamiltonianmontecarlo_amd/csrc/rmhmc_hip.hip
+++ b/riemannhamiltonianmontecarlo_amd/csrc/rmhmc_hip.hip
@@ -50,7 +50,7 @@
 };
 
 struct Options {
-  int64_t graph = 1, sorted = 1, inflight = 32, cdyn = 1, crestore = 1, i8_force_rebase = 0;
+  int64_t graph = 1, sorted = 1, inflight = 32, cdyn = 1, crestore = 1, i8_force_rebase = 0, stepfuse = 3;
   int64_t ccache = 1, medium = 1, fused = 1, hmc_traj_maxn = -1, fsplit = 0, nsplit_max = 64, nsplit_waves = -1, i8_tail = -1,
           i8_delta = 1, i8_delta_inner = 1;
 };
@@ -62,6 +62,7 @@
     {"cdyn", &Options::cdyn, false, 0, 1},
     {"crestore", &Options::crestore, false, 0, 1},
     {"i8_force_rebase", &Options::i8_force_rebase, false, 0, 1},
+    {"stepfuse", &Options::stepfuse, false, 0, 3},
     {"ccache", &Options::ccache, true, 0, 1},
     {"medium", &Options::medium, true, 0, 1},
     {"fused", &Options::fused, true, 0, 1},
@@ -72,6 +73,25 @@
     {"i8_tail", &Options::i8_tail, true, -1, 1},
     {"i8_delta", &Options::i8_delta, true, 0, 1},
     {"i8_delta_inner", &Options::i8_delta_inner, true, 0, 1},
+};
+struct StepGraph {
+  hipGraph_t graph = nullptr;
+  hipGraphExec_t exec = nullptr;
+  void destroy() {
+    if (exec) (void)hipGraphExecDestroy(exec);
+    if (graph) (void)hipGraphDestroy(graph);
+    exec = nullptr; graph = nullptr;
+  }
+};
+struct StepKey {
+  int sampler = -1, L = 0, K = 0;
+  double eps = 0.0;
+  uint32_t flags = 0;
+  long long opt_epoch = -1, data_epoch = -1, n = 0;
+  bool operator==(const StepKey& o) const {
+    return sampler == o.sampler && L == o.L && K == o.K && eps == o.eps && flags == o.flags && opt_epoch == o.opt_epoch &&
+           data_epoch == o.data_epoch && n == o.n;
+  }
 };
 const OptionDesc* find_option(const char* key) {
   if (!key) return nullptr;
@@ -135,6 +155,13 @@
   rmhmc_progress_fn progress_fn = nullptr;
   void* progress_user = nullptr;
   long long progress_first = 0, progress_every = 0, progress_next = 0;
+  StepGraph sgraph;
+  StepKey sgraph_key;
+  bool sgraph_known = false;
+  long long opt_epoch = 0, data_epoch = 0;
+  long long graph_builds = 0, graph_replays = 0;
+  IterParams* d_ip = nullptr;
+  bool ip_from_dev = false;
   bool timing = false;
   std::map<std::string, std::vector<EvPair>> events;
   std::vector<EvPair> pool;
@@ -504,7 +531,35 @@
 #define BIG(ctx, g, name, kern, ...)                                                                       \
   launch(ctx, name, [&](hipStream_t st_) { hipLaunchKernelGGL(kern, dim3((unsigned)(g).n), dim3(256), 0, st_, __VA_ARGS__); })
 
-void eval_point_phases(rmhmc_ctx* ctx, Group& g, bool advance, int mode = 0) {
+struct IterBase {
+  long long limit, burn_in, S;
+  double* samples;
+  bool explicit_rng;
+  bool count_done;
+};
+
+IterParams iter_params(rmhmc_ctx* ctx, const IterBase& b) {
+  IterParams ip{};
+  ip.flags = ctx->flags;
+  ip.L = ctx->L;
+  ip.seed = ctx->seed;
+  ip.chain_offset = ctx->chain_offset;
+  ip.iter_limit = b.limit;
+  ip.burn_in = b.burn_in;
+  ip.S = b.S;
+  ip.samples = b.samples;
+  if (ctx->sorted) ip.orig = ctx->d_orig;
+  if (b.explicit_rng) {
+    ip.z_in = ctx->d_z; ip.ulen_in = ctx->d_ulen; ip.gdir_in = ctx->d_gdir; ip.uacc_in = ctx->d_uacc;
+  }
+  ip.done_count = b.count_done ? ctx->d_done : nullptr;
+  ip.lower_L = (!ctx->big && !ctx->medium && !ctx->fused && ctx->sampler == 0) ? 1 : 0;
+  return ip;
+}
+
+static const IterParams* ip_block(const rmhmc_ctx* ctx) { return ctx->ip_from_dev ? ctx->d_ip : nullptr; }
+
+void eval_point_phases(rmhmc_ctx* ctx, Group& g, bool advance, int mode = 0, const IterBase* end_ib = nullptr) {
   const bool delta = advance && use_delta(ctx, g);
   launch_rowpass<RP_F>(ctx, g, g.ch.trj.w, g.ch.rv0, g.ch.rv2, delta);
   if (ctx->big) SMALL(ctx, g, "small", k_finish_big, ctx->dd, g.ch, g.nsplit);
@@ -535,7 +590,13 @@
     launch_mompass(ctx, g, g.ch.trj.w, 2);
     launch_leverage(ctx, g);
   }
-  SMALL(ctx, g, "small", k_mom_final, ctx->D, ctx->DP, g.ch, ctx->eps, advance ? 1 : 0, g.nsplit, fused_trace(ctx, g) ? g.ch.gpart : (const double*)nullptr);
+  const double* const trpart = fused_trace(ctx, g) ? g.ch.gpart : (const double*)nullptr;
+  if (end_ib && advance && !ctx->big) {
+    const IterParams ip = iter_params(ctx, *end_ib);
+    SMALL(ctx, g, "small", k_mom_final_end, ctx->D, ctx->DP, g.ch, ctx->eps, g.nsplit, trpart, ip, ip_block(ctx));
+    return;
+  }
+  SMALL(ctx, g, "small", k_mom_final, ctx->D, ctx->DP, g.ch, ctx->eps, advance ? 1 : 0, g.nsplit, trpart);
 }
 
 template <int NB>
@@ -556,13 +617,18 @@
   else launch_step_medium_nb<2>(ctx, g, st, guards, eval_only, fold, ip);
 }
 
-void step_phases(rmhmc_ctx* ctx, Group& g) {
+void step_phases(rmhmc_ctx* ctx, Group& g, const IterBase* ib = nullptr, int sf = 0) {
   const int D = ctx->D, DP = ctx->DP, K = ctx->K;
   const double eps = ctx->eps;
   const int guards = (ctx->flags & RMHMC_FLAG_GUARDS) ? 1 : 0;
   if (ctx->medium) {
     launch(ctx, "medium", [&](hipStream_t st) { launch_step_medium(ctx, g, st, guards, 0, 0, IterParams{}); });
     return;
+  }
+  const bool whole = ib && !ctx->big && (sf & 1), whole_end = ib && !ctx->big && (sf & 2);
+  if (whole) {
+    const IterParams ip = iter_params(ctx, *ib);
+    SMALL(ctx, g, "small", k_iter_begin_matvec, D, DP, g.ch, ip, ip_block(ctx));
   }
   if (!ctx->big && ctx->opt.cdyn && g.ctile && g.ch.stale_list)
     launch(ctx, "mompass", [&](hipStream_t st) {
@@ -573,7 +639,7 @@
     });
   const bool fuse = !ctx->big;
   for (int it = 0; it < K; ++it) {
-    if (it == 0 || !fuse) SMALL(ctx, g, "small", k_ginv_matvec, D, DP, g.ch, it == 0 ? g.ch.p : g.ch.PM);
+    if ((it == 0 && !whole) || !fuse) SMALL(ctx, g, "small", k_ginv_matvec, D, DP, g.ch, it == 0 ? g.ch.p : g.ch.PM);
     launch_mompass(ctx, g, g.ch.trj.w, it == 0 ? 1 : 2);
     if (!fuse) SMALL(ctx, g, "small", k_mom_update, D, DP, g.ch, eps, it == K - 1 ? 1 : 0, g.nsplit);
     else if (it < K - 1) SMALL(ctx, g, "small", k_mom_update_matvec, D, DP, g.ch, eps, g.nsplit);
@@ -596,42 +662,16 @@
       });
   }
   if (ctx->big || K < 2) SMALL(ctx, g, "small", k_pos_final, D, DP, g.ch, guards);
-  eval_point_phases(ctx, g, true);
-}
-
-struct IterBase {
-  long long limit, burn_in, S;
-  double* samples;
-  bool explicit_rng;
-  bool count_done;
-};
-
-IterParams iter_params(rmhmc_ctx* ctx, const IterBase& b) {
-  IterParams ip{};
-  ip.flags = ctx->flags;
-  ip.L = ctx->L;
-  ip.seed = ctx->seed;
-  ip.chain_offset = ctx->chain_offset;
-  ip.iter_limit = b.limit;
-  ip.burn_in = b.burn_in;
-  ip.S = b.S;
-  ip.samples = b.samples;
-  if (ctx->sorted) ip.orig = ctx->d_orig;
-  if (b.explicit_rng) {
-    ip.z_in = ctx->d_z; ip.ulen_in = ctx->d_ulen; ip.gdir_in = ctx->d_gdir; ip.uacc_in = ctx->d_uacc;
-  }
-  ip.done_count = b.count_done ? ctx->d_done : nullptr;
-  ip.lower_L = (!ctx->big && !ctx->medium && !ctx->fused && ctx->sampler == 0) ? 1 : 0;
-  return ip;
+  eval_point_phases(ctx, g, true, 0, whole_end ? ib : nullptr);
 }
 
 void launch_iter_begin(rmhmc_ctx* ctx, Group& g, const IterBase& b) {
   const IterParams ip = iter_params(ctx, b);
-  SMALL(ctx, g, "small", k_iter_begin, ctx->D, ctx->DP, g.ch, ip);
+  SMALL(ctx, g, "small", k_iter_begin, ctx->D, ctx->DP, g.ch, ip, ip_block(ctx));
 }
 void launch_iter_end(rmhmc_ctx* ctx, Group& g, const IterBase& b) {
   const IterParams ip = iter_params(ctx, b);
-  SMALL(ctx, g, "small", k_iter_end, ctx->D, ctx->DP, g.ch, ip);
+  SMALL(ctx, g, "small", k_iter_end, ctx->D, ctx->DP, g.ch, ip, ip_block(ctx));
 }
 
 template <int NB>
@@ -656,7 +696,7 @@
 void launch_hmc_global_step(rmhmc_ctx* ctx, Group& g, const IterBase& b) {
   const double eps = ctx->eps;
   const IterParams ip = iter_params(ctx, b);
-  SMALL(ctx, g, "small", k_hmc_begin, ctx->D, ctx->DP, g.ch, ip);
+  SMALL(ctx, g, "small", k_hmc_begin, ctx->D, ctx->DP, g.ch, ip, ip_block(ctx));
   if (ctx->hmc_traj) {
     launch_hmc_traj(ctx, g, 0);
   } else {
@@ -664,7 +704,7 @@
     launch_rowpass<RP_G>(ctx, g, g.ch.trj.w, nullptr);
     SMALL(ctx, g, "small", k_hmc_post, ctx->dd, g.ch, eps, g.nsplit);
   }
-  SMALL(ctx, g, "small", k_hmc_end, ctx->D, ctx->DP, g.ch, ip);
+  SMALL(ctx, g, "small", k_hmc_end, ctx->D, ctx->DP, g.ch, ip, ip_block(ctx));
 }
 
 void launch_global_step(rmhmc_ctx* ctx, Group& g, const IterBase& b) {
@@ -675,9 +715,10 @@
     launch(ctx, "medium", [&](hipStream_t st) { launch_step_medium(ctx, g, st, guards, 0, 1, ip); });
     return;
   }
-  launch_iter_begin(ctx, g, b);
-  step_phases(ctx, g);
-  launch_iter_end(ctx, g, b);
+  const int sf = ctx->big ? 0 : (int)ctx->opt.stepfuse;
+  if (!(sf & 1)) launch_iter_begin(ctx, g, b);
+  step_phases(ctx, g, &b, sf);
+  if (!(sf & 2)) launch_iter_end(ctx, g, b);
 }
 
 void launch_fused(rmhmc_ctx* ctx, const IterBase& b, long long nsteps) {
@@ -955,6 +996,7 @@
     fill_int(ctx, ch.cstale, 1, n);
     RC(dalloc(ctx, &ctx->d_nsteps, n)); RC(dalloc(ctx, &ctx->d_dir, n)); RC(dalloc(ctx, &ctx->d_done, 1)); RC(dalloc(ctx, &ctx->d_steps0, n));
     RC(dalloc(ctx, &ctx->d_miniter, 1));
+    RC(dalloc(ctx, &ctx->d_ip, (size_t)1));
     RC(dalloc(ctx, &ctx->d_orig, n)); RC(dalloc(ctx, &ctx->d_T, 2 * n));
     {
       const bool on = ctx->opt.medium && !ctx->big && D > FS_D && D <= 32 && ctx->Mp <= MS_MAXMP && n_chains <= 512;
@@ -1006,6 +1048,7 @@
   if (!ctx) return;
   (void)hipSetDevice(ctx->device);
   if (ctx->stream) (void)hipStreamSynchronize(ctx->stream);
+  ctx->sgraph.destroy();
   for (auto& e : ctx->flow) if (e) (void)hipEventDestroy(e);
   for (auto& kv : ctx->events) for (auto& e : kv.second) { (void)hipEventDestroy(e.a); (void)hipEventDestroy(e.b); }
   for (auto& e : ctx->pool) { (void)hipEventDestroy(e.a); (void)hipEventDestroy(e.b); }
@@ -1023,6 +1066,7 @@
   HIPCK(hipSetDevice(ctx->device));
   HIPCK(hipStreamSynchronize(ctx->stream));
   ctx->opt.*(d->slot) = value;
+  if (d->slot != &Options::graph && d->slot != &Options::sorted && d->slot != &Options::inflight) ctx->opt_epoch++;
   apply_runtime_options(ctx);
   if (ctx->stale_list_alloc) {
     HIPCK(hipMemsetAsync(ctx->batch.ch.stale_count, 0, sizeof(int), ctx->stream));
@@ -1134,6 +1178,7 @@
   ctx->dd.log_prior_const = -0.5 * std::log(2.0 * M_PI * alpha);
   ctx->have_data = true;
   ctx->chains_ready = false;
+  ctx->data_epoch++;
   return RMHMC_OK;
 }
 
@@ -1281,30 +1326,58 @@
   return RMHMC_OK;
 }
 
-struct StepGraph {
-  hipGraph_t graph = nullptr;
-  hipGraphExec_t exec = nullptr;
-  ~StepGraph() {
-    if (exec) (void)hipGraphExecDestroy(exec);
-    if (graph) (void)hipGraphDestroy(graph);
-  }
-};
-static bool step_graph_usable(const rmhmc_ctx* ctx, long long nsteps) {
-  if (ctx->timing || nsteps < 8) return false;
+static bool step_graph_allowed(const rmhmc_ctx* ctx) {
+  if (ctx->timing || !ctx->d_ip) return false;
   if (ctx->fused && ctx->sampler == 0) return false;
   if (ctx->medium && ctx->sampler == 0) return false;
   return ctx->opt.graph != 0;
 }
-static bool build_step_graph(rmhmc_ctx* ctx, const IterBase& ib, StepGraph& sg) {
-  if (hipStreamBeginCapture(ctx->stream, hipStreamCaptureModeThreadLocal) != hipSuccess) return false;
-  launch_global_step(ctx, ctx->batch, ib);
-  if (hipStreamEndCapture(ctx->stream, &sg.graph) != hipSuccess || !sg.graph) { (void)hipGetLastError(); return false; }
-  if (hipGraphInstantiate(&sg.exec, sg.graph, nullptr, nullptr, 0) != hipSuccess) { (void)hipGetLastError(); sg.exec = nullptr; return false; }
+static StepKey step_key(const rmhmc_ctx* ctx) {
+  StepKey k;
+  k.sampler = ctx->sampler; k.L = ctx->L; k.K = ctx->K; k.eps = ctx->eps; k.flags = ctx->flags;
+  k.opt_epoch = ctx->opt_epoch; k.data_epoch = ctx->data_epoch; k.n = ctx->batch.n;
+  return k;
+}
+static void drop_step_graph(rmhmc_ctx* ctx) {
+  if (ctx->sgraph.exec || ctx->sgraph.graph) {
+    if (ctx->stream) (void)hipStreamSynchronize(ctx->stream);
+    ctx->sgraph.destroy();
+  }
+  ctx->sgraph_known = false;
+}
+static bool build_step_graph(rmhmc_ctx* ctx, StepGraph& sg) {
+  if (hipStreamBeginCapture(ctx->stream, hipStreamCaptureModeThreadLocal) != hipSuccess) { (void)hipGetLastError(); return false; }
+  ctx->ip_from_dev = true;
+  launch_global_step(ctx, ctx->batch, IterBase{0, 0, 0, nullptr, false, false});
+  ctx->ip_from_dev = false;
+  if (hipStreamEndCapture(ctx->stream, &sg.graph) != hipSuccess || !sg.graph) { (void)hipGetLastError(); sg.destroy(); return false; }
+  if (hipGraphInstantiate(&sg.exec, sg.graph, nullptr, nullptr, 0) != hipSuccess) { (void)hipGetLastError(); sg.exec = nullptr; sg.destroy(); return false; }
+  ctx->graph_builds++;
   return true;
 }
-static void run_generic_steps(rmhmc_ctx* ctx, const IterBase& ib, long long nsteps, StepGraph* sg) {
-  if (sg && sg->exec) {
-    for (long long s = 0; s < nsteps; ++s) { (void)hipGraphLaunch(sg->exec, ctx->stream); flow_tick(ctx); }
+static hipGraphExec_t step_graph(rmhmc_ctx* ctx, long long nsteps) {
+  if (!step_graph_allowed(ctx)) return nullptr;
+  const StepKey key = step_key(ctx);
+  if (ctx->sgraph_known && ctx->sgraph_key == key) return ctx->sgraph.exec;
+  if (nsteps < 8) return nullptr;
+  drop_step_graph(ctx);
+  ctx->sgraph_key = key;
+  ctx->sgraph_known = true;
+  (void)build_step_graph(ctx, ctx->sgraph);
+  return ctx->sgraph.exec;
+}
+static void write_iter_params(rmhmc_ctx* ctx, const IterBase& ib) {
+  hipLaunchKernelGGL(k_set_iter_params, dim3(1), dim3(64), 0, ctx->stream, iter_params(ctx, ib), ctx->d_ip);
+}
+static hipGraphExec_t prepare_steps(rmhmc_ctx* ctx, const IterBase& ib, long long nsteps) {
+  const hipGraphExec_t ex = step_graph(ctx, nsteps);
+  if (ex) write_iter_params(ctx, ib);
+  return ex;
+}
+static void run_generic_steps(rmhmc_ctx* ctx, const IterBase& ib, long long nsteps, hipGraphExec_t ex) {
+  if (ex) {
+    for (long long s = 0; s < nsteps; ++s) { (void)hipGraphLaunch(ex, ctx->stream); flow_tick(ctx); }
+    ctx->graph_replays += nsteps;
   } else {
     for (long long s = 0; s < nsteps; ++s) { launch_global_step(ctx, ctx->batch, ib); flow_tick(ctx); }
   }
@@ -1348,12 +1421,11 @@
   const bool fused = ctx->fused && ctx->sampler == 0;
   const bool ticking = progress_ticking(ctx);
   const long long chunk = ticking ? std::max<long long>(8, ctx->progress_every * (ctx->L + 1) / 2) : min_steps;
-  StepGraph sg;
-  if (!fused && step_graph_usable(ctx, std::min(min_steps, chunk))) (void)build_step_graph(ctx, ib, sg);
+  const hipGraphExec_t sg = fused ? nullptr : prepare_steps(ctx, ib, std::min(min_steps, chunk));
   for (long long left = min_steps; left > 0;) {
     const long long k = std::min(left, chunk);
     if (fused) launch_fused(ctx, ib, k);
-    else run_generic_steps(ctx, ib, k, &sg);
+    else run_generic_steps(ctx, ib, k, sg);
     left -= k;
     if (ticking && left > 0) {
       RC(poll_progress(ctx, &done, &min_iter));
@@ -1367,7 +1439,7 @@
     long long next = std::max(poll, ib.limit - min_iter);
     if (ticking) next = std::min(next, chunk);
     if (fused) launch_fused(ctx, ib, next);
-    else run_generic_steps(ctx, ib, next, &sg);
+    else run_generic_steps(ctx, ib, next, sg);
     s += next;
     if (s > min_steps * (long long)ctx->L + 1000000) return fail(ctx, RMHMC_ERR_RUNTIME, "sampler did not terminate");
   }
@@ -1410,24 +1482,19 @@
   const long long chunk = ticking ? std::max<long long>(8, ctx->progress_every * (ctx->L + 1) / 2) : Tmax + 1;
   int done = 0;
   long long mi = 0;
-  {
-    StepGraph sg;
-    if (step_graph_usable(ctx, std::min(Tmin, chunk))) (void)build_step_graph(ctx, ib, sg);
-    for (long long left = Tmin; left > 0;) {
-      const long long k = std::min(left, chunk);
-      run_generic_steps(ctx, ib, k, &sg);
-      left -= k;
-      if (ticking) { RC(poll_progress(ctx, &done, &mi)); RC(progress_fire(ctx, mi)); }
-    }
-    HIPCK(hipStreamSynchronize(ctx->stream));
+  const hipGraphExec_t sg = prepare_steps(ctx, ib, std::min(Tmin, chunk));
+  for (long long left = Tmin; left > 0;) {
+    const long long k = std::min(left, chunk);
+    run_generic_steps(ctx, ib, k, sg);
+    left -= k;
+    if (ticking) { RC(poll_progress(ctx, &done, &mi)); RC(progress_fire(ctx, mi)); }
   }
   int na = n;
   for (long long s = Tmin; s < Tmax; ++s) {
     while (na > 0 && T[na - 1] <= s) --na;
     const int nar = std::min(n, (na + 127) / 128 * 128);
-    if (nar == n) launch_global_step(ctx, ctx->batch, ib);
-    else launch_global_step_prefix(ctx, ib, nar);
-    flow_tick(ctx);
+    if (nar == n) run_generic_steps(ctx, ib, 1, sg);
+    else { launch_global_step_prefix(ctx, ib, nar); flow_tick(ctx); }
     if (ticking && (s - Tmin) % chunk == chunk - 1) { RC(poll_progress(ctx, &done, &mi)); RC(progress_fire(ctx, mi)); }
   }
   RC(poll_progress(ctx, &done, &mi));
@@ -1782,10 +1849,7 @@
     if (ctx->fused) {
       launch_fused(ctx, ib, n_steps);
     } else {
-      StepGraph sg;
-      if (step_graph_usable(ctx, n_steps)) (void)build_step_graph(ctx, ib, sg);
-      run_generic_steps(ctx, ib, n_steps, &sg);
-      HIPCK(hipStreamSynchronize(ctx->stream));
+      run_generic_steps(ctx, ib, n_steps, prepare_steps(ctx, ib, n_steps));
     }
   }
   return sync(ctx);
@@ -1838,7 +1902,13 @@
   const std::string w(which);
   if (seconds_out) *seconds_out = 0.0;
   if (launches_out) *launches_out = 0;
-  if (w == "enable") { ctx->timing = true; return RMHMC_OK; }
+  if (w == "graph_builds") { if (launches_out) *launches_out = ctx->graph_builds; return RMHMC_OK; }
+  if (w == "graph_replays") { if (launches_out) *launches_out = ctx->graph_replays; return RMHMC_OK; }
+  if (w == "enable") {
+    ctx->timing = true;
+    drop_step_graph(ctx);
+    return RMHMC_OK;
+  }
   if (w == "disable") { ctx->timing = false; return RMHMC_OK; }
   if (w == "reset") {
     RC(sync(ctx));
```

Result: no change. 571,100, median of 3 (+1.4%).
